# taylorlu/voicepuppet

Hardware: AMD Instinct MI355X
Metric: PixReferNet G+D step frames/sec @256x256 bs=32 (higher is better)
Workload: dtype bf16; 1 GPU; PixReferNet G+D training step (G + 3xD + VGG16-conv3_3 perceptual + TF-Adam x2), 256x256, ngf=ndf=64, global batch 32 = 32 per GPU; global_batch=32, per_gpu_batch=32, parallelism=dp1

## Files before the change

voicepuppet_amd/csrc/conv_args.h:

```cpp
#pragma once
#include <stddef.h>
#include <stdint.h>

namespace vp {

struct TapTable {
  int8_t dh[16];
  int8_t dw[16];
};

struct PixSrc {
  const void* ptr[2];
  int C[2];
  const float* aff_a[2];
  const float* aff_b[2];
  int act;
  int group_n;
};

enum ConvKernel {
  CK_IGEMM = 0,
  CK_PATCH,
  CK_PATCH2,
  CK_SMALLP,
  CK_S2C64,
  CK_CIN8,
  CK_COUT8,
  CK_DCOUT8,
  CK_COUT4,
  CK_C64,
  CK_PATCH3,
  CK_PATCH4,
  CK_DC256,
  CK_DC64,
};
struct IgemmArgs {
  PixSrc x;
  int N, Hin, Win;
  int Cin, log2Cin;
  int cin_mask;
  int cin_real;
  int Hg, Wg;
  int sh, sw;
  int ntaps, nclass;
  TapTable taps[4];
  const void* Wp;
  int Kpad, CoutPad;
  int wp_rows;
  void* Y;
  int y_f32;
  int Cout, ldY;
  int Hof, Wof, os;
  int o0h[4], o0w[4];
  const float* bias;
  int out_act;
  const void* ref;
  const float* ref_a;
  const float* ref_b;
  int ref_act, ref_group_n, accumulate;
  int split_c;
  void* Y2;
  const void* ref2;
  int accumulate2;
  int y2_f32;
  int splitk;
  float* partial;
  int vec_epi;
  int fastk;
  int rowperm;
  int xcd_remap;
  double* bn_part;
  int bn_tpg, bn_nchunk;
  const void* bst_y;
  const void* bst_y2;
  double* bn_part2;
  double* colsum_part;
  const void* zeros;
  int kern, p_kw, p_dhf, p_dhs, p_dwf, p_dws;
  void* xa_lrelu;
  void* xa_relu;
  void* pool_out;
  int pool_only;
  unsigned char* pool_code;
  int pool_src;
  unsigned* sp_cnt;
  unsigned short sp_mask[4];
  int sp_npt, sp_lcpt;
};

struct WgradArgs {
  PixSrc g;
  int Gc, log2Gc;
  int gc_mask;
  int Hgin, Wgin;
  PixSrc d;
  int Dc;
  int N, Hb, Wb;
  int s, ntaps;
  TapTable taps;
  int Mpad, Dpad;
  int splitk;
  float* partial;
  float* dW;
  int Greal, Dreal, accumulate;
  const void* zeros;
  int lw, lh;
  int fastw;
  int xcd_remap;
  int fast_tr;
};

struct Cout1Args {
  const void* dy;
  int ld_dy;
  const float* w;
  const void* ref;
  int ref_act;
  const void* y;
  double* part;
  void* dx;
  int N, H, W, C, Ho, Wo, ks, pad;
  int groups, rows;
  float* slabs;
  float* dW;
  int pix_per_group, tiles_per_group;
};

}
```

voicepuppet_amd/csrc/conv_ops.h:

```cpp
#pragma once
#include <stdlib.h>
#include <string.h>

#include "launch.h"

namespace vp {

struct ConvGeomX : ConvGeom {
  int CoutT;
};

inline ConvGeomX make_geom(int kind, int ks, int stride, int pad, int N, int Hin, int Win, int Cin, int Cin_real, int Cout) {
  ConvGeomX g;
  g.kind = kind; g.ks = ks; g.stride = stride; g.pad = pad;
  g.N = N; g.Hin = Hin; g.Win = Win;
  if (kind == 0) { g.Hout = (Hin + 2 * pad - ks) / stride + 1; g.Wout = (Win + 2 * pad - ks) / stride + 1; }
  else { g.Hout = 2 * Hin; g.Wout = 2 * Win; }
  g.Cin = Cin; g.Cin_real = Cin_real; g.Cout = Cout;
  g.CoutT = Cout < 8 ? 8 : Cout;
  return g;
}

inline int kc_elems(int is_bf16) { return is_bf16 ? 32 : 16; }

inline int& wgrad_cost_knob(int i) { static int v[3] = {80, 15, 150}; return v[i]; }
inline int& plan_misc_knob(int i) { static int v[4] = {384, 8, 4, 512}; return v[i]; }
inline int& igemm_small_grid_knob() { static int v = 128; return v; }
inline int& thin_blocks_knob(int i) { static int v[4] = {1024, 512, 512, 512}; return v[i]; }

inline int pick_igemm_cfg(int rows, int P, int Kpad = 0) {
  if (P >= 96) {
    if (rows % 128 == 0 && igemm_small_grid_knob() > 0 && (long long)((P + 127) / 128) * (rows / 128) <= igemm_small_grid_knob()) return IG_64x128;
    if (rows % 256 == 0 && P >= 256 * 256 && Kpad >= 4096) return IG_256x256;
    if (rows % 128 == 0 && P >= 256 * 512) return IG_128x256;
    if (rows % 128 == 0) return IG_128x128;
    if (rows % 64 == 0) return IG_64x128;
    if (rows <= 16) return IG_16x128;
    return rows > 64 ? IG_128x128 : IG_64x128;
  }
  if (rows <= 64) return IG_64x32;
  return P > 16 ? IG_128x32 : IG_128x16;
}

constexpr int IGEMM_SPLITK_TARGET_DEFAULT = 64;
inline int& igemm_splitk_target_knob() { static int v = IGEMM_SPLITK_TARGET_DEFAULT; return v; }
inline int pick_igemm_splitk(int blocks, int nchunk) {
  const int target = igemm_splitk_target_knob();
  const int cap = plan_misc_knob(1);
  const int minchunk = plan_misc_knob(2);
  if (blocks >= 256 || blocks >= target) return 1;
  int s = (target + blocks - 1) / blocks;
  if (s > nchunk / minchunk) s = nchunk / minchunk;
  if (s > cap) s = cap;
  return s < 1 ? 1 : s;
}

inline void set_single_src(PixSrc& x, const void* p, int C, const float* a, const float* b, int act, int group_n) {
  x.ptr[0] = p; x.ptr[1] = nullptr; x.C[0] = C; x.C[1] = 0;
  x.aff_a[0] = a; x.aff_b[0] = b; x.aff_a[1] = nullptr; x.aff_b[1] = nullptr;
  x.act = act; x.group_n = group_n > 0 ? group_n : (1 << 30);
}

struct LaunchForm {
  bool bias = false, ref = false, xa_lrelu = false, xa_relu = false, x_affine = false;
  bool stats = false;
  int x_act = 0, ref_act = 0;
};

struct IgemmPlan {
  IgemmArgs a;
  int cfg;
  LaunchForm form;
  PackDesc pack;
  size_t pack_elems;
  size_t partial_bytes;
};

struct IgemmPin { int cfg, splitk; };

inline void finish_igemm(IgemmPlan& p, int rows, int is_bf16, const IgemmPin* pin = nullptr) {
  IgemmArgs& a = p.a;
  const int P = a.N * a.Hg * a.Wg;
  a.Kpad = round_up(a.ntaps * a.Cin, kc_elems(is_bf16));
  p.cfg = pick_igemm_cfg(rows, P, a.Kpad);
  if (!is_bf16 && a.ntaps == 1 && p.cfg == IG_128x128) {
    const long long b128 = (long long)((P + 127) / 128) * (rows / 128), b64 = 2 * b128;
    if (((b64 + 255) / 256) * 64 < ((b128 + 255) / 256) * 128) p.cfg = IG_64x128;
  }
  if (pin) p.cfg = pin->cfg;
  int bc, bp;
  igemm_tile(p.cfg, &bc, &bp);
  a.CoutPad = round_up(rows, bc);
  if (a.ntaps == 1) { a.log2Cin = 30; a.cin_mask = 0x3fffffff; }
  else { a.log2Cin = ilog2(a.Cin); a.cin_mask = a.Cin - 1; }
  const int blocks = ((P + bp - 1) / bp) * (a.CoutPad / bc) * a.nclass;
  a.splitk = pin ? pin->splitk : pick_igemm_splitk(blocks, a.Kpad / kc_elems(is_bf16));
  p.partial_bytes = a.splitk > 1 ? (size_t)a.nclass * a.splitk * P * a.CoutPad * sizeof(float) : 0;
  {
    const bool tc4 = p.cfg == IG_128x128 || p.cfg == IG_64x128 || p.cfg == IG_128x256 || p.cfg == IG_256x256;
    a.rowperm = (tc4 && rows % 64 == 0) ? 1 : 0;
    p.pack.perm = a.rowperm;
  }
  a.wp_rows = round_up(rows, 128);
  p.pack.rows_pad = a.wp_rows;
  p.pack.Kpad = a.Kpad;
  p.pack.kc = kc_elems(is_bf16);
  p.pack_elems = (size_t)a.nclass * a.wp_rows * a.Kpad;
}

inline int& patch_tiles_knob() { static int v = 7; return v; }
inline int& patch_small_knob() { static int v = 3; return v; }
inline int& patch_longk_knob() { static int v = 1; return v; }
inline int& patch3_knob() { static int v = 1; return v; }
inline int& wgrad_big_knob() { static int v = 1; return v; }
inline int& patch4_knob() { static int v = 1; return v; }
inline int& c64_knob() { static int v = 1; return v; }
inline int& pool_bwd_fused_knob() { static int v = 1; return v; }
inline int& cout1_knob() { static int v = 256; return v; }
inline int& wgrad1_rows_knob() { static int v = 512; return v; }
inline int& dc64_knob() { static int v = 1; return v; }
inline int& s2c64_knob() { static int v = 512; return v; }
inline int& s2c64_pair_knob() { static int v = 1; return v; }
constexpr int PATCH_MIN_BLOCKS_DEFAULT = 192;
inline int& patch_minblk_knob() { static int v = PATCH_MIN_BLOCKS_DEFAULT; return v; }

inline void patch_tile_hw(int bp, int* th, int* tw) { *th = bp == 128 ? 8 : 16; *tw = bp == 512 ? 32 : 16; }
inline int patch_tile_pixels(int bc) {
  const int k = patch_small_knob();
  if (bc == 256) return (k & 2) ? 128 : 256;
  return (k & 1) ? 256 : 512;
}

inline int patch_tile_rows(int rows, int on) {
  if ((on & 1) && rows % 256 == 0) return 256;
  if ((on & 2) && rows % 128 == 0) return 128;
  if ((on & 4) && rows % 64 == 0) return 64;
  return 0;
}

inline bool plan_patch_eligible(const IgemmPlan& p, int rows, int is_bf16, bool single_src, bool any_grid = false) {
  const int on = patch_tiles_knob();
  const int minblk = any_grid ? 0 : patch_minblk_knob();
  const IgemmArgs& a = p.a;
  const int kc = kc_elems(is_bf16);
  if (!on || !single_src || a.nclass != 1 || a.sh != 1 || a.sw != 1 || a.os != 1 || a.ntaps < 9 || a.Cin % kc || a.Cin < kc) return false;
  if (rows % 64 || a.Cout % 8 || a.ldY % 8 || a.Hg < 16 || a.Wg < 16 || a.Hof != a.Hg || a.Wof != a.Wg) return false;
  const bool p4 = patch4_knob() && is_bf16 && a.ntaps == 16 && rows % 128 == 0;
  if (!p4 && patch_longk_knob() && rows >= 512 && rows % 256 == 0 && a.ntaps * a.Cin >= 4096 && (long long)a.N * a.Hg * a.Wg >= 256 * 256) return false;
  const int bc = p4 ? 128 : patch_tile_rows(rows, on);
  if (!bc) return false;
  int th, tw;
  patch_tile_hw(p4 ? 256 : patch_tile_pixels(bc), &th, &tw);
  const long long blocks = (long long)a.N * ((a.Hg + th - 1) / th) * ((a.Wg + tw - 1) / tw) * (rows / bc);
  const long long p4min = (long long)a.ntaps * a.Cin >= 8192 ? 256 : 512;
  if (p4 && !any_grid && patch_minblk_knob() > 1) {
    if (blocks < p4min) return false;
  } else if (blocks < minblk) return false;
  if ((size_t)a.N * a.Hin * a.Win * a.Cin * (is_bf16 ? 2 : 4) >= 0x70000000ull) return false;
  int ks = 0;
  while (ks * ks < a.ntaps) ++ks;
  if (ks * ks != a.ntaps) return false;
  const int sh = a.taps[0].dh[ks] - a.taps[0].dh[0], sw = a.taps[0].dw[1] - a.taps[0].dw[0];
  if ((sh != 1 && sh != -1) || (sw != 1 && sw != -1)) return false;
  for (int t = 0; t < a.ntaps; ++t)
    if (a.taps[0].dh[t] != a.taps[0].dh[0] + (t / ks) * sh || a.taps[0].dw[t] != a.taps[0].dw[0] + (t % ks) * sw) return false;
  return true;
}
inline void plan_make_patch(IgemmPlan& p, int rows, int is_bf16) {
  IgemmArgs& a = p.a;
  const bool p4 = patch4_knob() && is_bf16 && a.ntaps == 16 && rows % 128 == 0;
  const int bc = p4 ? 128 : patch_tile_rows(rows, patch_tiles_knob());
  int ks = 0;
  while (ks * ks < a.ntaps) ++ks;
  a.kern = CK_PATCH; a.p_kw = ks;
  a.p_dhf = a.taps[0].dh[0]; a.p_dwf = a.taps[0].dw[0];
  a.p_dhs = a.taps[0].dh[ks] - a.taps[0].dh[0]; a.p_dws = a.taps[0].dw[1] - a.taps[0].dw[0];
  const int bp = p4 ? 256 : patch_tile_pixels(bc);
  p.cfg = bc == 256 ? (bp == 128 ? PATCH_256x128 : PATCH_256x256) : (bc == 128 ? (bp == 256 ? PATCH_128x256 : PATCH_128x512) : (bp == 256 ? PATCH_64x256 : PATCH_64x512));
  a.CoutPad = round_up(rows, bc);
  a.splitk = 1;
  p.partial_bytes = 0;
  a.rowperm = 1;
  p.pack.perm = 1;
  p.pack.kswap = 1;
}

inline int& patch_xcd_knob() { static int v = 0; return v; }
inline int& patch2_knob() { static int v = 1; return v; }
inline bool plan_patch2_eligible(const IgemmPlan& p, int rows, int is_bf16, int c0, int c1) {
  const IgemmArgs& a = p.a;
  const int kc = kc_elems(is_bf16);
  if (!patch2_knob() || a.nclass != 4 || a.ntaps != 4 || a.os != 2 || a.sh != 1 || a.sw != 1) return false;
  if (c0 + c1 != a.Cin || c0 % (2 * kc) || c1 % (2 * kc) || c0 < 2 * kc) return false;
  if (rows % 64 || rows > 128 || a.Cout % 8 || a.ldY % 8 || a.Hg < 16 || a.Wg < 16 || a.Hof != 2 * a.Hg || a.Wof != 2 * a.Wg) return false;
  const long long blocks = (long long)a.N * ((a.Hg + 15) / 16) * ((a.Wg + 15) / 16) * 4;
  if (blocks < patch_minblk_knob()) return false;
  const size_t cmax = c0 > c1 ? c0 : c1;
  if ((size_t)a.N * a.Hin * a.Win * cmax * (is_bf16 ? 2 : 4) >= 0x70000000ull) return false;
  for (int cls = 0; cls < 4; ++cls)
    for (int t = 0; t < 4; ++t)
      if (a.taps[cls].dh[t] != a.taps[cls].dh[3] + 1 - (t >> 1) || a.taps[cls].dw[t] != a.taps[cls].dw[3] + 1 - (t & 1)) return false;
  return true;
}
inline void plan_make_patch2(IgemmPlan& p, int rows, int is_bf16) {
  IgemmArgs& a = p.a;
  const int bc = rows % 128 == 0 ? 128 : 64;
  a.kern = CK_PATCH2; a.p_kw = 2;
  p.cfg = bc == 128 ? PATCH_128x256 : PATCH_64x256;
  a.CoutPad = round_up(rows, bc);
  a.splitk = 1;
  p.partial_bytes = 0;
  a.rowperm = 1;
  p.pack.perm = 1;
  p.pack.kswap = 1;
}

inline int& smallp_knob() { static int v = 256; return v; }
inline bool plan_smallp_eligible(const IgemmPlan& p, int rows, int is_bf16, int c0, int c1) {
  const IgemmArgs& a = p.a;
  const int kc = kc_elems(is_bf16);
  const long long Pc = (long long)a.N * a.Hg * a.Wg;
  if (smallp_knob() <= 0 || Pc > smallp_knob() || a.ntaps > 16 || a.nclass > 4) return false;
  if (rows % 32 || a.Cout != rows || a.ldY % 8) return false;
  if (a.Cin < kc || (a.Cin & (a.Cin - 1)) || c0 + c1 != a.Cin || c0 % kc || c1 % kc) return false;
  if ((long long)a.N * a.Hin * a.Win * (c0 > c1 ? c0 : c1) >= (1ll << 30)) return false;
  return true;
}
inline int smallp_counters(const IgemmArgs& a) {
  const int PT = a.sp_npt * 16;
  const int Pc = a.N * a.Hg * a.Wg;
  return (a.CoutPad / 32) * a.nclass * ((Pc + PT - 1) / PT) + a.CoutPad / 32;
}
inline void plan_make_smallp(IgemmPlan& p, int rows, int is_bf16) {
  IgemmArgs& a = p.a;
  const int kc = kc_elems(is_bf16);
  const int Pc = a.N * a.Hg * a.Wg;
  a.kern = CK_SMALLP;
  a.sp_npt = Pc <= 16 ? 1 : (Pc <= 32 ? 2 : 4);
  p.cfg = a.sp_npt == 1 ? SMALLP_32x16 : (a.sp_npt == 2 ? SMALLP_32x32 : SMALLP_32x64);
  a.sp_lcpt = ilog2(a.Cin / kc);
  a.CoutPad = round_up(rows, 32);
  a.rowperm = 0; p.pack.perm = 0; p.pack.kswap = 0;
  int minchunks = 1 << 30;
  for (int cls = 0; cls < a.nclass; ++cls) {
    unsigned m = 0;
    for (int t = 0; t < a.ntaps; ++t) {
      bool okh = false, okw = false;
      for (int q = 0; q < a.Hg && !okh; ++q) { const int ih = q * a.sh + a.taps[cls].dh[t]; okh = ih >= 0 && ih < a.Hin; }
      for (int r = 0; r < a.Wg && !okw; ++r) { const int iw = r * a.sw + a.taps[cls].dw[t]; okw = iw >= 0 && iw < a.Win; }
      if (okh && okw) m |= 1u << t;
    }
    a.sp_mask[cls] = (unsigned short)m;
    const int chunks = __builtin_popcount(m) * (a.Cin / kc);
    if (chunks < minchunks) minchunks = chunks;
  }
  const int PT = a.sp_npt * 16;
  const int tiles = (a.CoutPad / 32) * a.nclass * ((Pc + PT - 1) / PT);
  const int target = plan_misc_knob(0);
  int s = (target + tiles - 1) / tiles;
  if (s > minchunks / 8) s = minchunks / 8;
  if (s > 64) s = 64;
  if (s < 1) s = 1;
  a.splitk = s;
  p.partial_bytes = s > 1 ? (size_t)s * tiles * PT * 32 * sizeof(float) : 0;
}

inline bool plan_s2c64_eligible(const IgemmPlan& p, int rows, int is_bf16, int c0, int c1) {
  const IgemmArgs& a = p.a;
  if (s2c64_knob() <= 0 || !is_bf16 || a.nclass != 1 || a.ntaps != 16 || a.os != 1 || a.sh != 2 || a.sw != 2) return false;
  if ((rows != 128 && rows != 256) || a.Cout != rows || a.ldY != 128 || a.Cin != 64 || c0 != 64 || c1 != 0 || a.Kpad != 1024) return false;
  if (a.Hg % 4 || a.Wg % 16 || a.Hin != 2 * a.Hg || a.Win != 2 * a.Wg || a.Hof != a.Hg || a.Wof != a.Wg) return false;
  for (int t = 0; t < 16; ++t)
    if (a.taps[0].dh[t] != (t >> 2) - 1 || a.taps[0].dw[t] != (t & 3) - 1) return false;
  if (a.N * (a.Hg / 4) * (a.Wg / 16) < s2c64_knob()) return false;
  return (size_t)a.N * a.Hin * a.Win * 64 * 2 < 0x70000000ull;
}
inline void plan_make_s2c64(IgemmPlan& p) {
  IgemmArgs& a = p.a;
  a.kern = CK_S2C64;
  p.cfg = IG_128x128;
  a.CoutPad = a.Cout; a.wp_rows = a.Cout; p.pack.rows_pad = a.Cout;
  p.pack_elems = (size_t)a.wp_rows * a.Kpad;
  a.splitk = 1; p.partial_bytes = 0;
  a.rowperm = 1; p.pack.perm = 1; p.pack.kswap = 0;
}

inline IgemmArgs launch_view(const IgemmPlan& p, const LaunchForm& f) {
  static char set[16] = {};
  IgemmArgs v = p.a;
  v.Y = set; v.zeros = set;
  if (v.split_c) v.Y2 = set;
  if (f.bias) v.bias = (const float*)set;
  if (f.ref) { v.ref = set; v.ref_act = f.ref_act; if (v.split_c) v.ref2 = set; }
  if (f.xa_lrelu) v.xa_lrelu = set;
  if (f.xa_relu) v.xa_relu = set;
  if (f.x_affine) v.x.aff_a[0] = (const float*)set;
  v.x.act = f.x_act;
  if (f.stats) v.bn_part = (double*)set;
  return v;
}

enum { FAM_SMALLP = 1, FAM_PATCH = 2, FAM_PATCH2 = 4, FAM_S2C64 = 8, FAM_ALL = 15 };

inline void plan_kernel(IgemmPlan& p, int rows, int is_bf16, int c0, int c1, unsigned fams, const LaunchForm& f, bool any_grid = false) {
  if ((fams & FAM_SMALLP) && plan_smallp_eligible(p, rows, is_bf16, c0, c1)) plan_make_smallp(p, rows, is_bf16);
  else if ((fams & FAM_PATCH) && plan_patch_eligible(p, rows, is_bf16, c1 == 0 && c0 == p.a.Cin, any_grid)) plan_make_patch(p, rows, is_bf16);
  else if ((fams & FAM_PATCH2) && plan_patch2_eligible(p, rows, is_bf16, c0, c1)) plan_make_patch2(p, rows, is_bf16);
  else if ((fams & FAM_S2C64) && plan_s2c64_eligible(p, rows, is_bf16, c0, c1)) plan_make_s2c64(p);
  p.form = f;
  p.a.x.C[0] = c0; p.a.x.C[1] = c1;
  p.a.kern = pick_conv_kernel(launch_view(p, f), is_bf16);
}

inline IgemmPlan plan_fwd(const ConvGeomX& g, size_t w_off, int is_bf16, const IgemmPin* pin = nullptr) {
  IgemmPlan p;
  memset(&p, 0, sizeof(p));
  IgemmArgs& a = p.a;
  a.N = g.N; a.Hin = g.Hin; a.Win = g.Win; a.Cin = g.Cin; a.cin_real = g.Cin_real;
  a.Cout = g.Cout; a.ldY = g.Cout; a.Hof = g.Hout; a.Wof = g.Wout;
  a.ref_group_n = 1 << 30;
  PackDesc& d = p.pack;
  d.src_off = w_off; d.rows_real = g.Cout; d.C = g.Cin; d.C_real = g.Cin_real;
  if (g.kind == 0) {
    a.Hg = g.Hout; a.Wg = g.Wout; a.sh = a.sw = g.stride; a.os = 1;
    a.ntaps = g.ks * g.ks; a.nclass = 1;
    for (int t = 0; t < a.ntaps; ++t) {
      a.taps[0].dh[t] = (int8_t)(t / g.ks - g.pad); a.taps[0].dw[t] = (int8_t)(t % g.ks - g.pad);
      d.kh[0][t] = (int8_t)(t / g.ks); d.kw[0][t] = (int8_t)(t % g.ks);
    }
    d.s_kh = g.ks * g.Cin_real * g.Cout; d.s_kw = g.Cin_real * g.Cout; d.s_ch = g.Cout; d.s_row = 1;
  } else {
    a.Hg = g.Hin; a.Wg = g.Win; a.sh = a.sw = 1; a.os = 2;
    a.ntaps = 4; a.nclass = 4;
    for (int cls = 0; cls < 4; ++cls) {
      const int ph = cls >> 1, pw = cls & 1;
      a.o0h[cls] = ph; a.o0w[cls] = pw;
      for (int t = 0; t < 4; ++t) {
        const int ta = t >> 1, tb = t & 1;
        a.taps[cls].dh[t] = (int8_t)(ph - ta); a.taps[cls].dw[t] = (int8_t)(pw - tb);
        d.kh[cls][t] = (int8_t)((1 - ph) + 2 * ta); d.kw[cls][t] = (int8_t)((1 - pw) + 2 * tb);
      }
    }
    d.s_kh = 4 * g.Cout * g.Cin_real; d.s_kw = g.Cout * g.Cin_real; d.s_row = g.Cin_real; d.s_ch = 1;
  }
  d.nclass = a.nclass; d.ntaps = a.ntaps;
  finish_igemm(p, g.Cout, is_bf16, pin);
  return p;
}

inline IgemmPlan plan_bwd_data(const ConvGeomX& g, size_t w_off, int row0, int rows, int rows_real, int ldX, int is_bf16) {
  IgemmPlan p;
  memset(&p, 0, sizeof(p));
  IgemmArgs& a = p.a;
  a.N = g.N; a.Hin = g.Hout; a.Win = g.Wout; a.Cin = g.CoutT; a.cin_real = g.Cout;
  a.Cout = rows; a.ldY = ldX; a.Hof = g.Hin; a.Wof = g.Win;
  a.ref_group_n = 1 << 30;
  PackDesc& d = p.pack;
  d.rows_real = rows_real; d.C = g.CoutT; d.C_real = g.Cout;
  if (g.kind == 0) {
    d.s_kh = g.ks * g.Cin_real * g.Cout; d.s_kw = g.Cin_real * g.Cout; d.s_row = g.Cout; d.s_ch = 1;
    if (g.stride == 1) {
      a.Hg = g.Hin; a.Wg = g.Win; a.sh = a.sw = 1; a.os = 1;
      a.ntaps = g.ks * g.ks; a.nclass = 1;
      for (int t = 0; t < a.ntaps; ++t) {
        const int kh = t / g.ks, kw = t % g.ks;
        a.taps[0].dh[t] = (int8_t)(g.pad - kh); a.taps[0].dw[t] = (int8_t)(g.pad - kw);
        d.kh[0][t] = (int8_t)kh; d.kw[0][t] = (int8_t)kw;
      }
    } else {
      a.Hg = g.Hout; a.Wg = g.Wout; a.sh = a.sw = 1; a.os = 2;
      a.ntaps = 4; a.nclass = 4;
      for (int cls = 0; cls < 4; ++cls) {
        const int ph = cls >> 1, pw = cls & 1;
        a.o0h[cls] = ph; a.o0w[cls] = pw;
        for (int t = 0; t < 4; ++t) {
          const int ta = t >> 1, tb = t & 1;
          a.taps[cls].dh[t] = (int8_t)(ph - ta); a.taps[cls].dw[t] = (int8_t)(pw - tb);
          d.kh[cls][t] = (int8_t)((1 - ph) + 2 * ta); d.kw[cls][t] = (int8_t)((1 - pw) + 2 * tb);
        }
      }
    }
  } else {
    d.s_kh = 4 * g.Cout * g.Cin_real; d.s_kw = g.Cout * g.Cin_real; d.s_row = 1; d.s_ch = g.Cin_real;
    a.Hg = g.Hin; a.Wg = g.Win; a.sh = a.sw = 2; a.os = 1;
    a.ntaps = 16; a.nclass = 1;
    for (int t = 0; t < 16; ++t) {
      a.taps[0].dh[t] = (int8_t)(t / 4 - 1); a.taps[0].dw[t] = (int8_t)(t % 4 - 1);
      d.kh[0][t] = (int8_t)(t / 4); d.kw[0][t] = (int8_t)(t % 4);
    }
  }
  d.src_off = w_off + (size_t)row0 * d.s_row;
  d.nclass = a.nclass; d.ntaps = a.ntaps;
  finish_igemm(p, rows, is_bf16);
  return p;
}

struct WgradPlan {
  WgradArgs a;
  int cfg;
  size_t partial_bytes;
};

inline int& wgrad_tr_knob() { static int v = 3; return v; }

inline WgradPlan plan_wgrad(const ConvGeomX& g, int is_bf16, bool plain_operands = true) {
  WgradPlan p;
  memset(&p, 0, sizeof(p));
  WgradArgs& a = p.a;
  a.N = g.N;
  a.ntaps = g.ks * g.ks;
  for (int t = 0; t < a.ntaps; ++t) { a.taps.dh[t] = (int8_t)(t / g.ks - g.pad); a.taps.dw[t] = (int8_t)(t % g.ks - g.pad); }
  if (g.kind == 0) {
    a.Gc = g.Cin; a.Greal = g.Cin_real; a.Hgin = g.Hin; a.Wgin = g.Win;
    a.Dc = g.CoutT; a.Dreal = g.Cout;
    a.Hb = g.Hout; a.Wb = g.Wout; a.s = g.stride;
  } else {
    a.Gc = g.CoutT; a.Greal = g.Cout; a.Hgin = g.Hout; a.Wgin = g.Wout;
    a.Dc = g.Cin; a.Dreal = g.Cin_real;
    a.Hb = g.Hin; a.Wb = g.Win; a.s = 2;
  }
  a.log2Gc = ilog2(a.Gc);
  a.gc_mask = a.Gc - 1;
  if (a.ntaps == 1) { a.log2Gc = 30; a.gc_mask = 0x3fffffff; }
  p.cfg = (a.Dc % 128 == 0) ? WG_128x128 : (a.Dc % 64 == 0 ? WG_128x64 : WG_128x16);
  a.lw = ilog2(a.Wb); a.lh = ilog2(a.Hb);
  const bool tr = is_bf16 && plain_operands && (wgrad_tr_knob() & 1) && (a.ntaps * a.Gc) % 256 == 0 && a.Dc % 128 == 0 &&
                  (((long long)a.N << (a.lw + a.lh)) % 32) == 0;
  if (tr) p.cfg = WG_TR_256x128;
  const bool tr_thin = !tr && is_bf16 && plain_operands && (wgrad_tr_knob() & 2) && (a.ntaps * a.Gc) % 128 == 0 && a.Dc % 8 == 0 && a.Dc <= 128 &&
                       (((long long)a.N << (a.lw + a.lh)) % 32) == 0 && a.lw + a.lh >= 5;
  if (tr_thin) p.cfg = WG_TR_128x128;
  int bm, bn;
  wgrad_tile(p.cfg, &bm, &bn);
  a.Mpad = round_up(a.ntaps * a.Gc, bm);
  a.Dpad = round_up(a.Dc, bn);
  const int kiter = (tr || tr_thin) ? 32 : kc_elems(is_bf16) * (is_bf16 ? 2 : 1);
  a.fastw = (!tr && !tr_thin && (1 << a.lw) >= (is_bf16 ? 8 : 4) && (1 << a.lw) <= kiter) ? 1 : 0;
  const int P = (a.fastw || tr || tr_thin) ? (a.N << (a.lw + a.lh)) : a.N * a.Hb * a.Wb;
  const int nchunk = (P + kiter - 1) / kiter;
  const int tiles = (a.Mpad / bm) * (a.Dpad / bn);
  int s = 1;
  const double wg_fixed = wgrad_cost_knob(0) * 0.1, wg_slab = wgrad_cost_knob(1) * 0.01 + wgrad_cost_knob(2) * 0.001 * tiles;
  {
    const int smax = nchunk / 4 < 1 ? 1 : (nchunk / 4 > 512 ? 512 : nchunk / 4);
    double best = 1e30;
    for (int c = 1; c <= smax; ++c) {
      const int rounds = (tiles * c + plan_misc_knob(3) - 1) / plan_misc_knob(3);
      const double cost = rounds * ((double)nchunk / c + wg_fixed) + wg_slab * c;
      if (cost < best - 1e-9) { best = cost; s = c; }
    }
  }
  if ((tr || tr_thin) && s >= 8 && (s & 7)) {
    const int smax = nchunk / 4 < 1 ? 1 : (nchunk / 4 > 512 ? 512 : nchunk / 4);
    auto cost = [&](int c) { return ((tiles * c + plan_misc_knob(3) - 1) / plan_misc_knob(3)) * ((double)nchunk / c + wg_fixed) + wg_slab * c; };
    const int lo = s & ~7, hi = lo + 8;
    s = (hi <= smax && cost(hi) <= cost(lo)) ? hi : lo;
  }
  a.splitk = s;
  p.partial_bytes = (size_t)s * a.Mpad * a.Dpad * sizeof(float);
  return p;
}

}
```

voicepuppet_amd/csrc/conv_prof.h:

```cpp
#pragma once
#include <hip/hip_runtime.h>

#include <string>

namespace vp {

void profile_enable(int on);
void profile_tag(const char* tag);
size_t profile_collect(char* out, size_t cap);

extern const char* g_prof_family;

struct ProfRec { hipEvent_t e0, e1; std::string name; double flops, bytes; };

struct ProfScope {
  bool on;
  ProfRec r;
  hipStream_t st;
  std::string kind;
  int bf, bc, bp;
  ProfScope(const char* kind_, int is_bf16, int bc_, int bp_, double flops, double bytes, hipStream_t s);
  ~ProfScope();
};

}
```

voicepuppet_amd/csrc/conv_prof.hip:

```cpp
#include "conv_prof.h"

#include <stdio.h>
#include <string.h>

#include <vector>

namespace vp {

static bool g_prof_on = false;
static std::vector<ProfRec> g_prof;
static std::vector<hipEvent_t> g_ev_pool;

static hipEvent_t prof_event() {
  hipEvent_t e;
  if (!g_ev_pool.empty()) { e = g_ev_pool.back(); g_ev_pool.pop_back(); return e; }
  hipEventCreate(&e);
  return e;
}

static std::string g_prof_tag;
static bool g_prof_detail = false;
void profile_enable(int on) { g_prof_on = on != 0; g_prof_detail = on > 1; }
void profile_tag(const char* tag) { if (g_prof_on && g_prof_detail) g_prof_tag = tag ? tag : ""; }

const char* g_prof_family = nullptr;

ProfScope::ProfScope(const char* kind_, int is_bf16, int bc_, int bp_, double flops, double bytes, hipStream_t s) : on(g_prof_on), st(s), kind(kind_), bf(is_bf16), bc(bc_), bp(bp_) {
  if (!on) return;
  g_prof_family = nullptr;
  r.flops = flops; r.bytes = bytes;
  r.e0 = prof_event(); r.e1 = prof_event();
  hipEventRecord(r.e0, st);
}
ProfScope::~ProfScope() {
  if (!on) return;
  hipEventRecord(r.e1, st);
  char buf[96];
  if ((kind == "igemm" || kind == "wgrad") && g_prof_family) snprintf(buf, sizeof(buf), "%s_%s_%s_%dx%d", kind.c_str(), g_prof_family, bf ? "bf16" : "f32", bc, bp);
  else snprintf(buf, sizeof(buf), "%s_%s_%dx%d", kind.c_str(), bf ? "bf16" : "f32", bc, bp);
  r.name = buf;
  if (g_prof_detail && !g_prof_tag.empty()) r.name = g_prof_tag + " " + r.name;
  g_prof.push_back(r);
}

size_t profile_collect(char* out, size_t cap) {
  struct Agg { std::string name; int calls; double ms, flops, bytes; };
  static std::string cache = "[]";
  if (g_prof.empty()) {
    if (out && cap > 0) { strncpy(out, cache.c_str(), cap - 1); out[cap - 1] = 0; }
    return cache.size() + 1;
  }
  std::vector<Agg> agg;
  for (ProfRec& r : g_prof) {
    float ms = 0.f;
    hipEventSynchronize(r.e1);
    hipEventElapsedTime(&ms, r.e0, r.e1);
    g_ev_pool.push_back(r.e0); g_ev_pool.push_back(r.e1);
    Agg* a = nullptr;
    for (Agg& x : agg) if (x.name == r.name) a = &x;
    if (!a) { agg.push_back({r.name, 0, 0, 0, 0}); a = &agg.back(); }
    a->calls++; a->ms += ms; a->flops += r.flops; a->bytes += r.bytes;
  }
  g_prof.clear();
  std::string js = "[";
  for (size_t i = 0; i < agg.size(); ++i) {
    char buf[256];
    snprintf(buf, sizeof(buf), "%s{\"name\":\"%s\",\"calls\":%d,\"ms\":%.6f,\"flops\":%.6e,\"bytes\":%.6e}", i ? "," : "",
             agg[i].name.c_str(), agg[i].calls, agg[i].ms, agg[i].flops, agg[i].bytes);
    js += buf;
  }
  js += "]";
  cache = js;
  if (out && cap > 0) { strncpy(out, js.c_str(), cap - 1); out[cap - 1] = 0; }
  return js.size() + 1;
}

}
```

voicepuppet_amd/csrc/conv_s2c64.hip:

```cpp
#include "conv_ops.h"
#include "igemm_device.h"
#include "launch.h"
#include "patch_device.h"

namespace vp {

namespace {
constexpr int TH = 4, TW = 16;
constexpr int PRW = 17;
constexpr int PHR = 2 * TH + 2;
constexpr int NPATCH = PHR * 2 * PRW;
constexpr int NROUND = 22;
constexpr int PBUFB = NROUND * 16 * 64;
constexpr int NCH = 2;
constexpr int BUFB = NCH * PBUFB;
constexpr int STGB = TH * TW * 256;
constexpr int NW = 8;
constexpr int JP = (NROUND + NW - 1) / NW;
}

__device__ __forceinline__ unsigned s2_pk_max_i16(unsigned x, unsigned y) {
  unsigned r;
  asm("v_pk_max_i16 %0, %1, %2" : "=v"(r) : "v"(x), "v"(y));
  return r;
}
__device__ __forceinline__ unsigned s2_pk_min_u16(unsigned x, unsigned y) {
  unsigned r;
  asm("v_pk_min_u16 %0, %1, %2" : "=v"(r) : "v"(x), "v"(y));
  return r;
}
__device__ __forceinline__ unsigned s2_pk_mul_lo_u16(unsigned x, unsigned y) {
  unsigned r;
  asm("v_pk_mul_lo_u16 %0, %1, %2" : "=v"(r) : "v"(x), "v"(y));
  return r;
}

template <bool STATS, bool PAIR>
__global__ __launch_bounds__(NW * 64, 1) void conv_s2c64_kernel(const IgemmArgs a, const int ntiles) {
  static_assert(!(STATS && PAIR), "statistics belong to the forward layers");
  extern __shared__ __attribute__((aligned(16))) char smem[];
  const int tid = threadIdx.x, lane = tid & 63;
  const int wave = __builtin_amdgcn_readfirstlane(tid >> 6);
  const int fi = lane & 15, fg = lane >> 4;

  const int G = gridDim.x;
  int vb = blockIdx.x;
  if ((G & 7) == 0) vb = (vb & 7) * (G >> 3) + (vb >> 3);
  const int half = PAIR ? (vb & 1) : 0, row0 = 128 * half;
  const int bt = PAIR ? (vb >> 1) : vb, GT = PAIR ? (G >> 1) : G;

  uint4 W[16][NCH];
  {
    const bf16* wp = reinterpret_cast<const bf16*>(a.Wp);
#pragma unroll
    for (int t = 0; t < 16; ++t)
#pragma unroll
      for (int c = 0; c < NCH; ++c)
        W[t][c] = *reinterpret_cast<const uint4*>(wp + ((size_t)(t * NCH + c) * a.wp_rows + row0 + 16 * wave + fi) * 32 + fg * 8);
  }
  const int c0 = 64 * (wave >> 2) + 32 * ((wave >> 1) & 1) + 8 * fg + 4 * (wave & 1);
  f32x4 bia = (f32x4){0.f, 0.f, 0.f, 0.f};
  if (a.bias) bia = (f32x4){a.bias[c0], a.bias[c0 + 1], a.bias[c0 + 2], a.bias[c0 + 3]};

  int tb0[2];
#pragma unroll
  for (int s = 0; s < 2; ++s) {
    const int px = fi + s;
    tb0[s] = (px << 6) + (((fg ^ (px >> 1)) & 3) << 4);
  }
  int ppy[JP], ppx[JP], prel[JP];
#pragma unroll
  for (int j = 0; j < JP; ++j) {
    const int pp = (wave + NW * j) * 16 + (lane >> 2);
    const int run = pp / PRW, idx = pp - run * PRW;
    ppy[j] = pp < NPATCH ? (run >> 1) : 1 << 20;
    ppx[j] = 2 * idx + (run & 1);
    prel[j] = pp < NPATCH ? (ppy[j] * a.Win + ppx[j]) * 128 + (((lane & 3) ^ ((idx >> 1) & 3)) * 8) * (int)sizeof(bf16) : 0;
  }
  const bool last_round = wave + NW * (JP - 1) < NROUND;

  __amdgpu_buffer_rsrc_t rsX = make_rsrc(a.x.ptr[0], (unsigned)((size_t)a.N * a.Hin * a.Win * 64 * sizeof(bf16)));
  const int tiles_x = a.Wg / TW, tpi = tiles_x * (a.Hg / TH);
  bf16* Yp = reinterpret_cast<bf16*>(half ? a.Y2 : a.Y);
  const bf16* refp = reinterpret_cast<const bf16*>(half ? a.ref2 : a.ref);
  const bool accum = PAIR && (half ? a.accumulate2 : a.accumulate);
  constexpr int NST = TH * TW * 256 / 1024 / NW;

  auto issue_patch = [&](int t, int buf) {
    const int n = t / tpi, rem = t - n * tpi;
    const int y0 = 2 * (rem / tiles_x) * TH - 1, x0 = 2 * (rem % tiles_x) * TW - 1;
    const int base = ((n * a.Hin + y0) * a.Win + x0) * 128;
#pragma unroll
    for (int j = 0; j < JP; ++j) {
      if (j == JP - 1 && !last_round) break;
      const int ih = y0 + ppy[j], iw = x0 + ppx[j];
      const bool ok = (unsigned)ih < (unsigned)a.Hin && (unsigned)iw < (unsigned)a.Win;
      const unsigned vo = ok ? (unsigned)(base + prel[j]) : DMA_OOB;
      uint4* l0 = reinterpret_cast<uint4*>(smem + buf * BUFB) + (wave + NW * j) * 64;
#pragma unroll
      for (int c = 0; c < NCH; ++c) dma16_buf(rsX, vo, (unsigned)(c * 64), l0 + c * (PBUFB / 16));
    }
  };

  float ssum[4] = {0.f, 0.f, 0.f, 0.f}, ssq[4] = {0.f, 0.f, 0.f, 0.f};
  int cur_grp = -1;
  unsigned done_mask = 0;
  const int ngroups = STATS ? (ntiles + a.bn_tpg - 1) / a.bn_tpg : 0;
  auto flush = [&](int grp) {
    float s[4], q[4];
#pragma unroll
    for (int e = 0; e < 4; ++e) {
      s[e] = ssum[e]; q[e] = ssq[e];
#pragma unroll
      for (int m = 1; m < 16; m <<= 1) { s[e] += __shfl_xor(s[e], m); q[e] += __shfl_xor(q[e], m); }
      ssum[e] = 0.f; ssq[e] = 0.f;
    }
    if (fi == 0) {
      double* row = a.bn_part + ((size_t)(grp * a.bn_nchunk + blockIdx.x) * 2) * a.Cout + c0;
#pragma unroll
      for (int e = 0; e < 4; ++e) { row[e] = (double)s[e]; row[a.Cout + e] = (double)q[e]; }
    }
    done_mask |= 1u << grp;
  };

  if (bt < ntiles) issue_patch(bt, 0);
#pragma unroll
  for (int t = 0; t < 16; ++t)
#pragma unroll
    for (int c = 0; c < NCH; ++c) asm volatile("" : "+v"(W[t][c].x), "+v"(W[t][c].y), "+v"(W[t][c].z), "+v"(W[t][c].w));
  int it = 0;
  for (int t = bt; t < ntiles; t += GT, ++it) {
    const int buf = it & 1;
    if (it == 0) wait_vm<0>();
    else wait_vm<NST>();
    __builtin_amdgcn_s_barrier();
    asm volatile("" ::: "memory");
    uint2 rz[PAIR ? TH : 1], ry[PAIR ? TH : 1];
    if constexpr (PAIR) {
      const int n = t / tpi, rem = t - n * tpi;
      const size_t o00 = ((size_t)(n * a.Hof + (rem / tiles_x) * TH) * a.Wof + (rem % tiles_x) * TW + fi) * 128 + c0;
#pragma unroll
      for (int r = 0; r < TH; ++r) rz[r] = *reinterpret_cast<const uint2*>(refp + o00 + (size_t)r * a.Wof * 128);
      if (accum) {
#pragma unroll
        for (int r = 0; r < TH; ++r) ry[r] = *reinterpret_cast<const uint2*>(Yp + o00 + (size_t)r * a.Wof * 128);
      }
    }
    if (t + GT < ntiles) issue_patch(t + GT, buf ^ 1);
    if constexpr (STATS) {
      const int grp = t / a.bn_tpg;
      if (grp != cur_grp) {
        if (cur_grp >= 0) flush(cur_grp);
        cur_grp = grp;
      }
    }
    int tb[2];
#pragma unroll
    for (int s = 0; s < 2; ++s) tb[s] = tb0[s] + buf * BUFB;

    f32x4 acc[TH];
#pragma unroll
    for (int r = 0; r < TH; ++r) acc[r] = bia;
    constexpr int LA = 2, NS = LA + 1, NSTEP = NCH * 4 * PHR;
    u32x4 rb[NS];
    auto rd = [&](auto sc) {
      constexpr int S = decltype(sc)::value, c = S / (4 * PHR), kw = (S / PHR) % 4, R = S % PHR;
      rb[S % NS] = lds_rd128<c * PBUFB + (R * 2 + (kw & 1)) * PRW * 64>(tb[kw >> 1]);
    };
    static_steps([&](auto sc) { rd(sc); }, std::make_integer_sequence<int, LA>{});
    static_steps([&](auto sc) {
      constexpr int S = decltype(sc)::value, c = S / (4 * PHR), kw = (S / PHR) % 4, R = S % PHR;
      if constexpr (S + LA < NSTEP) rd(std::integral_constant<int, S + LA>{});
      constexpr int AHEAD = (NSTEP - 1 - S < LA ? NSTEP - 1 - S : LA);
      asm volatile("s_waitcnt lgkmcnt(%0)" ::"n"(AHEAD) : "memory");
      asm volatile("" : "+v"(rb[S % NS]));
      const uint4 fb = make_uint4(rb[S % NS].x, rb[S % NS].y, rb[S % NS].z, rb[S % NS].w);
      static_steps([&](auto ri) {
        constexpr int r = (R >> 1) - decltype(ri)::value;
        if constexpr (r >= 0 && r < TH) {
          constexpr int kh = R - 2 * r;
          acc[r] = mma16<bf16>(W[4 * kh + kw][c], fb, acc[r]);
        }
      }, std::make_integer_sequence<int, 2>{});
      __builtin_amdgcn_sched_barrier(0);
    }, std::make_integer_sequence<int, NSTEP>{});

    char* stg = smem + 2 * BUFB;
    const int wslot = ((((c0 >> 3) ^ fi) & 15) << 4) + ((c0 & 4) << 1);
#pragma unroll
    for (int r = 0; r < TH; ++r) {
      uint2 pk;
      if constexpr (PAIR) {
        if (accum) {
          const float m0 = __uint_as_float(rz[r].x << 16) > 0.f ? 1.f : 0.f, m1 = __uint_as_float(rz[r].x & 0xffff0000u) > 0.f ? 1.f : 0.f;
          const float m2 = __uint_as_float(rz[r].y << 16) > 0.f ? 1.f : 0.f, m3 = __uint_as_float(rz[r].y & 0xffff0000u) > 0.f ? 1.f : 0.f;
          acc[r][0] = fmaf(acc[r][0], m0, __uint_as_float(ry[r].x << 16)); acc[r][1] = fmaf(acc[r][1], m1, __uint_as_float(ry[r].x & 0xffff0000u));
          acc[r][2] = fmaf(acc[r][2], m2, __uint_as_float(ry[r].y << 16)); acc[r][3] = fmaf(acc[r][3], m3, __uint_as_float(ry[r].y & 0xffff0000u));
        }
      }
      pk.x = Elem<bf16>::pack2(acc[r][0], acc[r][1]);
      pk.y = Elem<bf16>::pack2(acc[r][2], acc[r][3]);
      if constexpr (PAIR) {
        if (!accum) {
          pk.x = s2_pk_mul_lo_u16(pk.x, s2_pk_min_u16(s2_pk_max_i16(rz[r].x, 0u), 0x00010001u));
          pk.y = s2_pk_mul_lo_u16(pk.y, s2_pk_min_u16(s2_pk_max_i16(rz[r].y, 0u), 0x00010001u));
        }
      }
      if constexpr (STATS) {
        const float v0 = __uint_as_float(pk.x << 16), v1 = __uint_as_float(pk.x & 0xffff0000u);
        const float v2 = __uint_as_float(pk.y << 16), v3 = __uint_as_float(pk.y & 0xffff0000u);
        ssum[0] += v0; ssum[1] += v1; ssum[2] += v2; ssum[3] += v3;
        ssq[0] = fmaf(v0, v0, ssq[0]); ssq[1] = fmaf(v1, v1, ssq[1]); ssq[2] = fmaf(v2, v2, ssq[2]); ssq[3] = fmaf(v3, v3, ssq[3]);
      }
      *reinterpret_cast<uint2*>(stg + (r * TW + fi) * 256 + wslot) = pk;
    }
    asm volatile("s_waitcnt lgkmcnt(0)" ::: "memory");
    __builtin_amdgcn_s_barrier();
    asm volatile("" ::: "memory");
    {
      const int n = t / tpi, rem = t - n * tpi;
      const int q0 = (rem / tiles_x) * TH, r0 = (rem % tiles_x) * TW;
      const int row = wave >> 1;
#pragma unroll
      for (int j = 0; j < NST; ++j) {
        const int px = 8 * (wave & 1) + 4 * j + (lane >> 4), ps = lane & 15;
        const uint4 o = *reinterpret_cast<const uint4*>(stg + (row * TW + px) * 256 + (ps << 4));
        unsigned* yp = reinterpret_cast<unsigned*>(Yp + ((size_t)(n * a.Hof + q0 + row) * a.Wof + r0 + px) * 128 + ((ps ^ px) & 15) * 8);
        __builtin_nontemporal_store(o.x, yp); __builtin_nontemporal_store(o.y, yp + 1);
        __builtin_nontemporal_store(o.z, yp + 2); __builtin_nontemporal_store(o.w, yp + 3);
      }
    }
  }
  if constexpr (STATS) {
    if (cur_grp >= 0) flush(cur_grp);
    for (int g = 0; g < ngroups; ++g) {
      if (done_mask & (1u << g)) continue;
      if (fi == 0) {
        double* row = a.bn_part + ((size_t)(g * a.bn_nchunk + blockIdx.x) * 2) * a.Cout + c0;
#pragma unroll
        for (int e = 0; e < 4; ++e) { row[e] = 0.0; row[a.Cout + e] = 0.0; }
      }
    }
  }
}

int conv_s2c64_grid(const IgemmArgs& a) {
  const int ntiles = a.N * (a.Hg / TH) * (a.Wg / TW);
  return ntiles < 256 ? ntiles : 256;
}
int conv_s2c64_tiles_per_image(const IgemmArgs& a) { return (a.Hg / TH) * (a.Wg / TW); }

bool conv_s2c64_eligible(const IgemmArgs& a, int is_bf16) {
  if (!is_bf16 || a.kern != CK_S2C64 || a.ldY != 128 || a.Cin != 64 || a.x.C[0] != 64 || a.x.C[1] != 0 || !a.rowperm || a.splitk != 1) return false;
  if (a.Hg % TH || a.Wg % TW || a.Hin != 2 * a.Hg || a.Win != 2 * a.Wg) return false;
  if (a.out_act != ACT_NONE || a.y_f32 || a.pool_out || a.x.aff_a[0] || a.x.act != ACT_NONE || a.ref_a) return false;
  if (a.split_c) {
    return a.split_c == 128 && a.Cout == 256 && a.wp_rows == 256 && a.Y2 && a.ref && a.ref2 && a.ref_act == ACT_RELU && !a.y2_f32 && !a.bias && !a.bn_part;
  }
  return a.Cout == 128 && a.wp_rows == 128 && !a.ref && !a.accumulate;
}

hipError_t launch_conv_s2c64(const IgemmArgs& a, hipStream_t st) {
  const int ntiles = a.N * (a.Hg / TH) * (a.Wg / TW);
  const int pair = a.split_c ? 1 : 0;
  int grid = conv_s2c64_grid(a);
  if (pair) grid = 2 * ntiles < 512 ? 2 * ntiles : 512;
  if (a.bn_part && (pair || a.bn_nchunk != grid || a.bn_tpg <= 0 || (ntiles + a.bn_tpg - 1) / a.bn_tpg > 32)) return hipErrorInvalidValue;
  const int ki = pair ? 2 : (a.bn_part ? 1 : 0);
  void (*kerns[3])(const IgemmArgs, const int) = {conv_s2c64_kernel<false, false>, conv_s2c64_kernel<true, false>, conv_s2c64_kernel<false, true>};
  void (*kern)(const IgemmArgs, const int) = kerns[ki];
  const int smem = 2 * BUFB + STGB;
  static bool attr_done[3] = {false, false, false};
  if (!attr_done[ki]) { (void)hipFuncSetAttribute((const void*)kern, hipFuncAttributeMaxDynamicSharedMemorySize, smem); attr_done[ki] = true; }
  hipLaunchKernelGGL(kern, dim3(grid), dim3(NW * 64), smem, st, a, ntiles);
  return hipGetLastError();
}

}
```

voicepuppet_amd/csrc/ops_api.hip:

```cpp
#include <string.h>

#include <string>

#include "conv_ops.h"
#include "errors.h"
#include "audio_args.h"
#include "launch.h"
#include "vp_common.h"
#include "workspace.h"

using namespace vp;

namespace {

bool conv_desc_ok(const vp_conv_desc* d) {
  if (!d || d->n < 1 || d->h < 1 || d->w < 1) return false;
  if (d->cin < 8 || (d->cin & (d->cin - 1))) return false;
  if (d->kind == 1 && (d->ksize != 4 || d->stride != 2 || d->pad != 1)) return false;
  if (d->kind != 0 && d->kind != 1) return false;
  if (d->ksize < 1 || d->ksize > 4 || d->stride < 1 || d->stride > 2) return false;
  if (d->kind == 0 && d->stride == 2 && (d->ksize != 4 || d->pad != 1 || (d->h & 1) || (d->w & 1))) return false;
  return d->dtype == VP_F32 || d->dtype == VP_BF16;
}

ConvGeomX geom_of(const vp_conv_desc* d) {
  return make_geom(d->kind, d->ksize, d->stride, d->pad, d->n, d->h, d->w, d->cin, d->cin, d->cout);
}

const void* zero_page(char* ws, size_t used, hipStream_t st) {
  char* z = ws + align256(used);
  (void)hipMemsetAsync(z, 0, 256, st);
  return z;
}

}

extern "C" {

int vp_pixrefer_pack_frames(const unsigned char* example_frames, const unsigned char* current_frames, const int* crops,
                            int n, int img_size, float* inputs, float* fg_inputs, float* targets, float* masks, void* stream) {
  if (!example_frames || !current_frames || !crops || !inputs || !fg_inputs || !targets || !masks || n < 1 || img_size < 2) {
    set_err("vp_pixrefer_pack_frames: bad argument");
    return VP_ERR_ARG;
  }
  FramePackArgs a;
  a.ex = example_frames; a.cur = current_frames; a.crops = crops;
  a.inputs = inputs; a.fg_inputs = fg_inputs; a.targets = targets; a.masks = masks;
  a.N = n; a.S = img_size;
  VP_HIP_CHECK(launch_frame_pack(a, (hipStream_t)stream));
  return VP_OK;
}

extern "C" void vp_phase_marks_enable(int on);

enum TuneRule {
  TUNE_PLAIN,
  TUNE_POSITIVE,
  TUNE_NEG_RESETS,
  TUNE_0_TO_4,
};
struct TuneRow { const char* key; int* knob; TuneRule rule; int dflt; };

int vp_tune(const char* key, int value) {
  if (!key) return VP_ERR_ARG;
  static const TuneRow rows[] = {
      {"patch_tiles", &patch_tiles_knob(), TUNE_PLAIN},
      {"patch_min_blocks", &patch_minblk_knob(), TUNE_NEG_RESETS, PATCH_MIN_BLOCKS_DEFAULT},
      {"patch_small_tiles", &patch_small_knob(), TUNE_PLAIN},
      {"patch_long_k_on_256", &patch_longk_knob(), TUNE_PLAIN},
      {"wgrad_tr", &wgrad_tr_knob(), TUNE_PLAIN},
      {"patch3", &patch3_knob(), TUNE_PLAIN},
      {"c64", &c64_knob(), TUNE_PLAIN},
      {"dc64", &dc64_knob(), TUNE_PLAIN},
      {"pool_bwd_fused", &pool_bwd_fused_knob(), TUNE_0_TO_4, 1},
      {"cout1_wgrad_rows", &wgrad1_rows_knob(), TUNE_POSITIVE},
      {"cout1_bwd", &cout1_knob(), TUNE_NEG_RESETS, 256},
      {"s2c64", &s2c64_knob(), TUNE_PLAIN},
      {"wgrad_big", &wgrad_big_knob(), TUNE_PLAIN},
      {"patch4", &patch4_knob(), TUNE_PLAIN},
      {"s2c64_pair", &s2c64_pair_knob(), TUNE_PLAIN},
      {"bfm_dwproj", &bfm_dwproj_knob(), TUNE_PLAIN},
      {"patch2", &patch2_knob(), TUNE_PLAIN},
      {"patch_xcd", &patch_xcd_knob(), TUNE_PLAIN},
      {"smallp_max_pixels", &smallp_knob(), TUNE_PLAIN},
      {"igemm_splitk_target", &igemm_splitk_target_knob(), TUNE_NEG_RESETS, IGEMM_SPLITK_TARGET_DEFAULT},
      {"wgrad_fixed_x10", &wgrad_cost_knob(0), TUNE_PLAIN},
      {"wgrad_slab_x100", &wgrad_cost_knob(1), TUNE_PLAIN},
      {"wgrad_slab_tile_x1000", &wgrad_cost_knob(2), TUNE_NEG_RESETS, 150},
      {"smallp_split_target", &plan_misc_knob(0), TUNE_PLAIN},
      {"igemm_splitk_cap", &plan_misc_knob(1), TUNE_PLAIN},
      {"igemm_splitk_minchunk", &plan_misc_knob(2), TUNE_PLAIN},
      {"wgrad_resident_blocks", &plan_misc_knob(3), TUNE_PLAIN},
      {"igemm_small_grid", &igemm_small_grid_knob(), TUNE_PLAIN},
      {"thin_blocks_cout8", &thin_blocks_knob(0), TUNE_POSITIVE},
      {"thin_blocks_dcout8", &thin_blocks_knob(1), TUNE_POSITIVE},
      {"thin_blocks_cout4", &thin_blocks_knob(2), TUNE_POSITIVE},
      {"thin_blocks_cin8", &thin_blocks_knob(3), TUNE_POSITIVE},
  };
  if (!strcmp(key, "phase_marks")) { vp_phase_marks_enable(value); return VP_OK; }
  for (const TuneRow& r : rows) {
    if (strcmp(key, r.key)) continue;
    if (r.rule == TUNE_POSITIVE && value <= 0) break;
    const bool reset = (r.rule == TUNE_NEG_RESETS && value < 0) || (r.rule == TUNE_0_TO_4 && (value < 0 || value > 4));
    *r.knob = reset ? r.dflt : value;
    return VP_OK;
  }
  set_err("vp_tune: unknown key %s", key);
  return VP_ERR_ARG;
}

static unsigned* smallp_counter_page(char* ws, size_t used, const IgemmArgs& a, hipStream_t st) {
  unsigned* c = (unsigned*)(ws + align256(used) + 256);
  (void)hipMemsetAsync(c, 0, (size_t)smallp_counters(a) * sizeof(unsigned), st);
  return c;
}

size_t vp_conv_workspace_bytes(const vp_conv_desc* d) {
  if (!conv_desc_ok(d)) return 0;
  const int bf = d->dtype == VP_BF16, es = bf ? 2 : 4;
  const ConvGeomX g = geom_of(d);
  size_t best = 0;
  {
    IgemmPlan p = plan_fwd(g, 0, bf);
    best = align256(p.pack_elems * es) + p.partial_bytes;
    plan_kernel(p, g.Cout, bf, d->cin, 0, FAM_SMALLP, LaunchForm{});
    if (p.a.kern == CK_SMALLP) {
      const size_t b = align256(p.pack_elems * es) + align256(p.partial_bytes) + 512 + (size_t)smallp_counters(p.a) * sizeof(unsigned);
      if (b > best) best = b;
    }
  }
  if ((d->cout & (d->cout - 1)) == 0 && d->cout >= 8) {
    IgemmPlan p = plan_bwd_data(g, 0, 0, d->cin, d->cin, d->cin, bf);
    size_t b = align256(p.pack_elems * es) + p.partial_bytes;
    if (b > best) best = b;
    plan_kernel(p, d->cin, bf, d->cout, 0, FAM_SMALLP, LaunchForm{});
    if (p.a.kern == CK_SMALLP) {
      b = align256(p.pack_elems * es) + align256(p.partial_bytes) + 512 + (size_t)smallp_counters(p.a) * sizeof(unsigned);
      if (b > best) best = b;
    }
    for (int plain = 0; plain < 2; ++plain) {
      WgradPlan w = plan_wgrad(g, bf, plain != 0);
      if (w.partial_bytes + 512 > best) best = w.partial_bytes + 512;
    }
  }
  return best + 1024;
}

int vp_conv_fwd(const vp_conv_desc* d, const void* x, const float* in_scale, const float* in_shift,
                const float* w, const float* bias, void* y, void* workspace, void* stream) {
  if (!conv_desc_ok(d) || !x || !w || !y || !workspace) { set_err("vp_conv_fwd: bad argument"); return VP_ERR_ARG; }
  const int bf = d->dtype == VP_BF16, es = bf ? 2 : 4;
  hipStream_t st = (hipStream_t)stream;
  const ConvGeomX g = geom_of(d);
  IgemmPlan p = plan_fwd(g, 0, bf);
  p.a.out_act = d->out_act;
  LaunchForm f;
  f.bias = bias != nullptr; f.x_affine = in_scale != nullptr; f.x_act = d->in_act;
  const bool plain = d->in_act == ACT_NONE && !in_scale;
  plan_kernel(p, g.Cout, bf, d->cin, 0, plain ? (FAM_SMALLP | FAM_PATCH | FAM_PATCH2 | (d->out_act == ACT_NONE ? FAM_S2C64 : 0)) : 0, f);
  char* ws = (char*)workspace;
  VP_HIP_CHECK(launch_pack_weights_one(p.pack, w, ws, bf, st));
  IgemmArgs a = p.a;
  set_single_src(a.x, x, d->cin, in_scale, in_shift, d->in_act, 0);
  a.Wp = ws;
  a.partial = (float*)(ws + align256(p.pack_elems * es));
  a.Y = y; a.bias = bias;
  a.zeros = zero_page(ws, align256(p.pack_elems * es) + p.partial_bytes, st);
  if (a.kern == CK_SMALLP) a.sp_cnt = smallp_counter_page(ws, align256(p.pack_elems * es) + p.partial_bytes, a, st);
  VP_HIP_CHECK(launch_igemm(a, bf, p.cfg, st));
  return VP_OK;
}

int vp_conv_bwd_data(const vp_conv_desc* d, const void* dy, const float* w, void* dx, void* workspace, void* stream) {
  if (!conv_desc_ok(d) || !dy || !w || !dx || !workspace) { set_err("vp_conv_bwd_data: bad argument"); return VP_ERR_ARG; }
  if (d->cout < 8 || (d->cout & (d->cout - 1))) { set_err("vp_conv_bwd_data: cout must be a power of two >= 8"); return VP_ERR_ARG; }
  const int bf = d->dtype == VP_BF16, es = bf ? 2 : 4;
  hipStream_t st = (hipStream_t)stream;
  const ConvGeomX g = geom_of(d);
  IgemmPlan p = plan_bwd_data(g, 0, 0, d->cin, d->cin, d->cin, bf);
  plan_kernel(p, d->cin, bf, d->cout, 0, FAM_SMALLP | FAM_PATCH | FAM_PATCH2, LaunchForm{});
  char* ws = (char*)workspace;
  VP_HIP_CHECK(launch_pack_weights_one(p.pack, w, ws, bf, st));
  IgemmArgs a = p.a;
  set_single_src(a.x, dy, d->cout, nullptr, nullptr, ACT_NONE, 0);
  a.Wp = ws;
  a.partial = (float*)(ws + align256(p.pack_elems * es));
  a.Y = dx;
  a.zeros = zero_page(ws, align256(p.pack_elems * es) + p.partial_bytes, st);
  if (a.kern == CK_SMALLP) a.sp_cnt = smallp_counter_page(ws, align256(p.pack_elems * es) + p.partial_bytes, a, st);
  VP_HIP_CHECK(launch_igemm(a, bf, p.cfg, st));
  return VP_OK;
}

static bool pooled_desc_ok(const vp_conv_desc* d) {
  return conv_desc_ok(d) && d->kind == 0 && d->ksize == 3 && d->stride == 1 && d->pad == 1 && d->dtype == VP_BF16 && d->cin == d->cout &&
         (d->cin == 64 || d->cin == 128) && d->h % 4 == 0 && d->w % 16 == 0 && d->h >= 16;
}

size_t vp_conv3x3_c64_bwd_data_pooled_workspace_bytes(const vp_conv_desc* d) {
  if (!pooled_desc_ok(d)) return 0;
  return align256(vp_conv_workspace_bytes(d)) + align256((size_t)d->n * d->h * d->w * d->cout * 2) + 256;
}

int vp_conv3x3_c64_bwd_data_pooled(const vp_conv_desc* d, const void* dy_pool, const unsigned char* code, const float* w, const void* ref,
                                   void* dx, void* workspace, int fused, void* stream) {
  if (!pooled_desc_ok(d) || !dy_pool || !code || !w || !ref || !dx || !workspace) { set_err("vp_conv3x3_c64_bwd_data_pooled: bad argument"); return VP_ERR_ARG; }
  hipStream_t st = (hipStream_t)stream;
  const ConvGeomX g = geom_of(d);
  IgemmPlan p = plan_bwd_data(g, 0, 0, d->cin, d->cin, d->cin, 1);
  LaunchForm f;
  f.ref = true; f.ref_act = ACT_RELU;
  plan_kernel(p, d->cin, 1, d->cout, 0, FAM_PATCH, f);
  if (p.a.kern != CK_C64) {
    set_err("vp_conv3x3_c64_bwd_data_pooled: %d x %d x %d x %d is planned on kernel %s, not c64", d->n, d->h, d->w, d->cin, conv_kernel_name(p.a.kern));
    return VP_ERR_ARG;
  }
  char* ws = (char*)workspace;
  VP_HIP_CHECK(launch_pack_weights_one(p.pack, w, ws, 1, st));
  IgemmArgs a = p.a;
  a.Wp = ws;
  a.partial = (float*)(ws + align256(p.pack_elems * 2));
  a.Y = dx;
  a.ref = ref; a.ref_act = ACT_RELU;
  a.zeros = zero_page(ws, align256(p.pack_elems * 2) + p.partial_bytes, st);
  if (fused) {
    set_single_src(a.x, dy_pool, d->cout, nullptr, nullptr, ACT_NONE, 0);
    a.pool_code = const_cast<unsigned char*>(code);
    a.pool_src = 1;
  } else {
    char* full = ws + align256(vp_conv_workspace_bytes(d));
    VP_HIP_CHECK(launch_maxpool_bwd_code(code, dy_pool, full, d->n, d->h, d->w, d->cout, 1, st));
    set_single_src(a.x, full, d->cout, nullptr, nullptr, ACT_NONE, 0);
  }
  VP_HIP_CHECK(launch_igemm(a, 1, p.cfg, st));
  return VP_OK;
}

int vp_conv_bwd_weight(const vp_conv_desc* d, const void* x, const float* in_scale, const float* in_shift,
                       const void* dy, float* dw, void* workspace, void* stream) {
  if (!conv_desc_ok(d) || !x || !dy || !dw || !workspace) { set_err("vp_conv_bwd_weight: bad argument"); return VP_ERR_ARG; }
  if (d->cout < 8 || (d->cout & (d->cout - 1))) { set_err("vp_conv_bwd_weight: cout must be a power of two >= 8"); return VP_ERR_ARG; }
  const int bf = d->dtype == VP_BF16;
  hipStream_t st = (hipStream_t)stream;
  const ConvGeomX g = geom_of(d);
  WgradPlan p = plan_wgrad(g, bf, !in_scale && d->in_act == ACT_NONE);
  WgradArgs a = p.a;
  PixSrc xs, ds;
  set_single_src(xs, x, d->cin, in_scale, in_shift, d->in_act, 0);
  set_single_src(ds, dy, d->cout, nullptr, nullptr, ACT_NONE, 0);
  if (d->kind == 0) { a.g = xs; a.d = ds; } else { a.g = ds; a.d = xs; }
  a.partial = (float*)workspace;
  a.dW = dw;
  a.zeros = zero_page((char*)workspace, p.partial_bytes, st);
  VP_HIP_CHECK(launch_wgrad(a, bf, p.cfg, st));
  return VP_OK;
}

size_t vp_bn_workspace_bytes(int pixels, int c, int dtype) {
  if (pixels < 1 || c < 8) return 0;
  const int nch = bn_nchunk(pixels, c, 1, dtype == VP_BF16);
  return (size_t)nch * 2 * c * sizeof(double) + 4 * (size_t)c * sizeof(float) + 1024;
}

static bool bn_ok(int pixels, int c, int dtype) {
  const int e = dtype == VP_BF16 ? 8 : 4;
  return pixels >= 1 && c >= e && c % e == 0 && 256 % (c / e) == 0 && (dtype == VP_F32 || dtype == VP_BF16);
}

int vp_bn_stats(const void* y, int pixels, int c, int dtype, const float* gamma, const float* beta, float eps,
                float* scale, float* shift, float* mean, float* rstd, void* workspace, void* stream) {
  if (!bn_ok(pixels, c, dtype) || !y || !gamma || !beta || !scale || !shift || !mean || !rstd || !workspace) {
    set_err("vp_bn_stats: bad argument");
    return VP_ERR_ARG;
  }
  BnArgs b;
  memset(&b, 0, sizeof(b));
  b.y = y; b.C = c; b.G = 1; b.Pg = pixels;
  b.nchunk = bn_nchunk(pixels, c, 1, dtype == VP_BF16);
  b.partial = (double*)workspace;
  b.gamma = gamma; b.beta = beta; b.aff_a = scale; b.aff_b = shift; b.mu = mean; b.rstd = rstd; b.eps = eps;
  VP_HIP_CHECK(launch_bn_stats(b, dtype == VP_BF16, (hipStream_t)stream));
  return VP_OK;
}

int vp_bn_bwd(const void* y, const void* dz, void* dy, int pixels, int c, int dtype, const float* gamma,
              const float* mean, const float* rstd, float* dgamma, float* dbeta, void* workspace, void* stream) {
  if (!bn_ok(pixels, c, dtype) || !y || !dz || !dy || !gamma || !mean || !rstd || !dgamma || !dbeta || !workspace) {
    set_err("vp_bn_bwd: bad argument");
    return VP_ERR_ARG;
  }
  BnArgs b;
  memset(&b, 0, sizeof(b));
  b.y = y; b.dz = dz; b.dy = dy; b.C = c; b.G = 1; b.Pg = pixels;
  b.nchunk = bn_nchunk(pixels, c, 1, dtype == VP_BF16);
  b.partial = (double*)workspace;
  float* f = (float*)((char*)workspace + (size_t)b.nchunk * 2 * c * sizeof(double));
  b.c1 = f; b.c2 = f + c;
  b.gamma = gamma; b.mu = const_cast<float*>(mean); b.rstd = const_cast<float*>(rstd);
  b.dgamma = dgamma; b.dbeta = dbeta;
  VP_HIP_CHECK(launch_bn_bwd(b, dtype == VP_BF16, (hipStream_t)stream));
  return VP_OK;
}


int vp_maxpool2x2_fwd(const void* x, void* y, int n, int h, int w, int c, int dtype, void* stream) {
  const int e = dtype == VP_BF16 ? 8 : 4;
  if (!x || !y || n < 1 || h < 2 || w < 2 || (h & 1) || (w & 1) || c < e || c % e) { set_err("vp_maxpool2x2_fwd: bad argument"); return VP_ERR_ARG; }
  VP_HIP_CHECK(launch_maxpool_fwd(x, y, n, h, w, c, dtype == VP_BF16, (hipStream_t)stream));
  return VP_OK;
}

int vp_maxpool2x2_bwd(const void* x, const void* dy, void* dx, int n, int h, int w, int c, int dtype, void* stream) {
  const int e = dtype == VP_BF16 ? 8 : 4;
  if (!x || !dy || !dx || n < 1 || h < 2 || w < 2 || (h & 1) || (w & 1) || c < e || c % e) { set_err("vp_maxpool2x2_bwd: bad argument"); return VP_ERR_ARG; }
  VP_HIP_CHECK(launch_maxpool_bwd(x, dy, dx, n, h, w, c, dtype == VP_BF16, (hipStream_t)stream));
  return VP_OK;
}

int vp_maxpool2x2_bwd_code(const void* code, const void* dy, void* dx, int n, int h, int w, int c, int dtype, void* stream) {
  const int e = dtype == VP_BF16 ? 8 : 4;
  if (!code || !dy || !dx || n < 1 || h < 2 || w < 2 || (h & 1) || (w & 1) || c < e || c % e) { set_err("vp_maxpool2x2_bwd_code: bad argument"); return VP_ERR_ARG; }
  VP_HIP_CHECK(launch_maxpool_bwd_code(code, dy, dx, n, h, w, c, dtype == VP_BF16, (hipStream_t)stream));
  return VP_OK;
}

int vp_composite_fwd(const float* gen_out4, const float* targets, float* out4, float* outputs, float* outputs_fg, int n, int hw,
                     void* stream) {
  if (!gen_out4 || !targets || !out4 || !outputs || !outputs_fg || n < 1 || hw < 1) { set_err("vp_composite_fwd: bad argument"); return VP_ERR_ARG; }
  CompositeArgs ca;
  memset(&ca, 0, sizeof(ca));
  ca.y4 = gen_out4; ca.targets = targets; ca.o4 = out4; ca.outputs = outputs; ca.outputs_fg = outputs_fg; ca.N = n; ca.HW = hw; ca.train = 0;
  VP_HIP_CHECK(launch_composite_fwd(ca, 0, (hipStream_t)stream));
  return VP_OK;
}

int vp_gan_loss(const float* logits, void* seed_d, void* seed_g, float* predict, float* losses, int m, float gan_weight, int dtype,
                void* stream) {
  if (!logits || !seed_d || !seed_g || !predict || !losses || m < 1) { set_err("vp_gan_loss: bad argument"); return VP_ERR_ARG; }
  GanLossArgs ga;
  memset(&ga, 0, sizeof(ga));
  ga.logits = logits; ga.dl_d = seed_d; ga.dl_g = seed_g; ga.predict = predict; ga.losses = losses; ga.M = m; ga.gan_weight = gan_weight;
  VP_HIP_CHECK(launch_gan_loss(ga, dtype == VP_BF16, (hipStream_t)stream));
  return VP_OK;
}

int vp_dwconv7x3_bn_act(const float* x, const float* w, const float* bias, float* y, int b, int h, int wd, int c, void* stream) {
  if (!x || !w || !bias || !y || b < 1 || h < 1 || wd < 1 || c < 4 || (c & 3)) { set_err("vp_dwconv7x3_bn_act: bad argument"); return VP_ERR_ARG; }
  VP_HIP_CHECK(launch_dwconv7x3(x, w, bias, y, 0, b, h, wd, c, (hipStream_t)stream));
  return VP_OK;
}

int vp_dwconv7x3_bn_act_t(const void* x, const float* w, const float* bias, void* y, int dtype, int b, int h, int wd, int c, void* stream) {
  if (!x || !w || !bias || !y || b < 1 || h < 1 || wd < 1 || c < 4 || (c & 3) || (dtype != VP_F32 && dtype != VP_BF16)) {
    set_err("vp_dwconv7x3_bn_act_t: bad argument"); return VP_ERR_ARG;
  }
  VP_HIP_CHECK(launch_dwconv7x3(x, w, bias, y, dtype == VP_BF16, b, h, wd, c, (hipStream_t)stream));
  return VP_OK;
}

int vp_conv_first_fwd(const float* x, const float* w, const float* bias, float* y, int b, int h, int w_in, int cout, void* stream) {
  if (!x || !w || !bias || !y || b < 1 || h < 1 || w_in < 1 || cout < 1) { set_err("vp_conv_first_fwd: bad argument"); return VP_ERR_ARG; }
  int pt, ho, pl, wo;
  same_pad(h, 9, 1, &pt, &ho);
  same_pad(w_in, 5, 2, &pl, &wo);
  VP_HIP_CHECK(launch_conv_first(x, w, bias, y, 0, b, h, w_in, wo, cout, pt, pl, (hipStream_t)stream));
  return VP_OK;
}

static IgemmPlan dwproj_pack_plan(int pixels, int ce, int cout) {
  IgemmPlan p = plan_fwd(make_geom(0, 1, 1, 0, 1, pixels, 1, ce, ce, cout), 0, 0);
  p.pack.s_ch = cout;
  p.pack.dst_off = 0;
  p.pack.perm = 0; p.a.rowperm = 0;
  return p;
}

size_t vp_dwproj_workspace_bytes(int ce, int cout) {
  if (ce < 16 || ce % 16 || cout < 1) return 0;
  return align256((size_t)22 * ce * sizeof(float)) + align256(dwproj_pack_plan(1, ce, cout).pack_elems * sizeof(float)) + 256;
}

int vp_dwproj_fwd(const float* ex, const float* w_dw, const float* b_dw, const float* w_proj, const float* b_proj, float* y, int add, int b, int h,
                  int w, int ce, int cout, void* workspace, void* stream) {
  if (!ex || !w_dw || !b_dw || !w_proj || !b_proj || !y || !workspace || b < 1 || h < 1 || w < 1) { set_err("vp_dwproj_fwd: bad argument"); return VP_ERR_ARG; }
  if (!dwproj_eligible(w, ce, cout)) {
    set_err("vp_dwproj_fwd: no kernel for mel width %d, %d expanded and %d output channels (dwproj_eligible)", w, ce, cout);
    return VP_ERR_ARG;
  }
  const size_t ex_bytes = (size_t)b * h * w * ce * sizeof(float);
  if (ex_bytes >= 0xF0000000ull) {
    set_err("vp_dwproj_fwd: the expanded tensor is %zu bytes, the kernel's 32-bit lane offsets stop below 0xF0000000 (%llu)", ex_bytes, 0xF0000000ull);
    return VP_ERR_ARG;
  }
  hipStream_t st = (hipStream_t)stream;
  float* wdw22 = (float*)workspace;
  float* packed = (float*)((char*)workspace + align256((size_t)22 * ce * sizeof(float)));
  VP_HIP_CHECK(hipMemcpyAsync(wdw22, w_dw, (size_t)21 * ce * sizeof(float), hipMemcpyDeviceToDevice, st));
  VP_HIP_CHECK(hipMemcpyAsync(wdw22 + (size_t)21 * ce, b_dw, (size_t)ce * sizeof(float), hipMemcpyDeviceToDevice, st));
  const IgemmPlan p = dwproj_pack_plan(b * h * w, ce, cout);
  VP_HIP_CHECK(launch_pack_weights_one(p.pack, w_proj, packed, 0, st));
  VP_HIP_CHECK(launch_dwproj(ex, wdw22, packed, p.a.wp_rows, b_proj, y, add ? 1 : 0, b, h, w, ce, cout, st));
  return VP_OK;
}

int vp_maxpool_hw(const float* x, float* y, int b, int h, int w, int c, int kh, int kw, int sh, int sw, void* stream) {
  if (!x || !y || b < 1 || h < 1 || w < 1 || c < 4 || (c & 3) || kh < 1 || kw < 1 || sh < 1 || sw < 1) { set_err("vp_maxpool_hw: bad argument"); return VP_ERR_ARG; }
  const int ho = (h + sh - 1) / sh, wo = (w + sw - 1) / sw;
  const int ph = (ho - 1) * sh + kh - h, pw = (wo - 1) * sw + kw - w;
  const int pt = ph > 0 ? ph / 2 : 0, pl = pw > 0 ? pw / 2 : 0;
  VP_HIP_CHECK(launch_maxpool_same(x, y, 0, 0, b, h, w, c, kh, kw, sh, sw, pt, pl, ho, wo, (hipStream_t)stream));
  return VP_OK;
}

int vp_gru_seq(const float* xg, const float* xc, const float* whg, const float* whc, const int* seq_len, float* out, int b, int t,
               void* stream) {
  if (!xg || !xc || !whg || !whc || !seq_len || !out || b < 1 || t < 1) { set_err("vp_gru_seq: bad argument"); return VP_ERR_ARG; }
  VP_HIP_CHECK(launch_gru_seq(xg, xc, whg, whc, seq_len, out, b, t, (hipStream_t)stream));
  return VP_OK;
}

int vp_gru_seq_state(const float* xg, const float* xc, const float* whg, const float* whc, float* hstate, float* out, int b, int t, int t0,
                     int n, void* stream) {
  if (!xg || !xc || !whg || !whc || !hstate || !out || b < 1 || t < 1 || t0 < 0 || n < 0 || t0 + n > t) {
    set_err("vp_gru_seq_state: bad argument"); return VP_ERR_ARG;
  }
  if (n == 0) return VP_OK;
  VP_HIP_CHECK(launch_gru_state(xg, xc, whg, whc, hstate, out, b, t, t0, n, (hipStream_t)stream));
  return VP_OK;
}

}

extern "C" __attribute__((target("sse4.2"))) unsigned vp_crc32c(const void* data, size_t n, unsigned crc) {
  const unsigned char* p = (const unsigned char*)data;
  unsigned long long c = (unsigned long long)(crc ^ 0xFFFFFFFFu);
  while (n && ((size_t)p & 7)) { c = __builtin_ia32_crc32qi((unsigned)c, *p++); --n; }
  while (n >= 8) { c = __builtin_ia32_crc32di(c, *(const unsigned long long*)p); p += 8; n -= 8; }
  while (n) { c = __builtin_ia32_crc32qi((unsigned)c, *p++); --n; }
  return (unsigned)c ^ 0xFFFFFFFFu;
}
```

voicepuppet_amd/csrc/plan_pixrefer.hip:

```cpp
#include <math.h>
#include <stdio.h>
#include <string.h>

#include <mutex>
#include <string>
#include <utility>
#include <vector>

#include "conv_ops.h"
#include "conv_prof.h"
#include "errors.h"
#include "launch.h"
#include "smallp_args.h"
#include "vp_common.h"
#include "workspace.h"

namespace vp {

thread_local char g_err[512] = "";
void set_err(const char* fmt, ...) {
  va_list ap;
  va_start(ap, fmt);
  vsnprintf(g_err, sizeof(g_err), fmt, ap);
  va_end(ap);
}

struct BnBuf {
  float *a, *b, *mu, *rstd, *c1, *c2, *c1g, *c2g;
  double *pb, *pbg;
};

struct Tens {
  std::string name;
  void* y = nullptr;
  void* dz = nullptr;
  int N = 0, H = 0, W = 0, C = 0;
  bool is_f32 = false;
  bool has_bn = false;
  bool is_input = false;
  int pool = -1, pool_src = -1;
  bool dz_written = false;
  void* dz2 = nullptr;
  bool dz2_written = false;
  void* xa[3] = {nullptr, nullptr, nullptr};
  bool need_act[3] = {false, false, false};
  BnBuf bn{};
  int producer = -1;
  int n_bwd_consumers = 0;
  int dz_writes = 0;
  bool bn_bwd_done = false;
  bool hi = false;
  void* dz32 = nullptr;
  double* cs_part = nullptr;
  int cs_chunks = 0;
  int pb_cap = 0, pbg_cap = 0;
  int bst_chunks = 0, bst_chunks_g = 0;
  size_t elems() const { return (size_t)N * H * W * C; }
};

struct Layer {
  std::string scope;
  ConvGeomX g;
  int src[2] = {-1, -1};
  int nsrc = 1;
  int in_act = ACT_NONE;
  int out_act = ACT_NONE;
  int out = -1;
  bool has_bn = false;
  bool fg = false;
  int pool = -1, pool_t = -1;
  size_t w_off = 0, b_off = 0, gamma_off = 0, beta_off = 0;
  size_t pk_fwd = 0, pk_bwd[2] = {0, 0}, pk_bwd_alt[2] = {0, 0};
  bool need_bwd[2] = {false, false};
  IgemmPlan fwd, bwd[2], bwd_alt[2];
  IgemmPlan bwd_pair;
  size_t pk_bwd_pair = 0;
  bool has_pair = false;
  IgemmPlan fwd_half;
  size_t pk_fwd_half = 0;
  bool has_fwd_half = false;
  WgradPlan wg;
  size_t desc0 = 0, desc1 = 0;
  bool tapgemm = false;
  bool fwd_stats = false;
  float* tap_S = nullptr;
  void* tap_dyS = nullptr;
  unsigned* sp_cnt_fwd = nullptr;
  unsigned* sp_cnt_bwd[2] = {nullptr, nullptr};
  unsigned* sp_cnt_pair = nullptr;
};

struct ParamInfo { std::string name; size_t off; int ndim; int64_t shape[4]; };

struct Net {
  std::vector<Tens> t;
  std::vector<Layer> l;
  std::vector<ParamInfo> manifest;
  size_t nparams = 0;
  int batch = 0, groups = 1;
  int i_md5 = -1, i_me2 = -1;
  float* params = nullptr;
  float* grads = nullptr;
  char* packed = nullptr;
  size_t packed_elems = 0;
  std::vector<PackDesc> descs;
  PackDesc* d_descs = nullptr;
  unsigned* sp_cnt = nullptr;
  size_t sp_cnt_n = 0;
};

struct Lane { hipStream_t s; char* scratch; double* bn_partial; };
enum { LANE_CALLER = 0, LANE_SIDE = 1, LANE_BRANCH = 2, LANE_BRANCH2 = 3 };

struct Sub { int sample0, nb; bool alt, gpass; };

}

using namespace vp;

struct vp_pixrefer {
  vp_pixrefer_desc d;
  int bf16, es;
  Net G, D, V;
  void *gin, *gfg, *din, *vin;
  float *y4, *o4, *outputs, *outputs_fg, *logits, *predict, *losses;
  void *dl_d, *dl_g, *d_din, *d_vin, *dy4, *df3;
  void *vpool1, *vpool2, *d_vpool1, *d_vpool2;
  unsigned char* vpool_code[2];
  bool pool_codes_written;
  bool pool_fuse_ok[2];
  bool pool_bwd_fused;
  bool pool_dz_stale[2];
  double *comp_partial, *perc_partial;
  Lane lane[4];
  hipEvent_t ev_b2join;
  bool use_b2;
  hipEvent_t ev_fork, ev_join, ev_bfork, ev_bjoin;
  hipEvent_t ev_upd_b, ev_upd_m;
  bool overlap, forked;
  int bst_count;
  int bst_on;
  int vgg_fork_layer;
  bool store_first_raw;
  bool ov_on;
  int dfork_point;
  bool dsplit_on;
  hipEvent_t mark[64];
  int nmark;
  bool marks_made;
  int dfork_pending;
  void* zeros;
  size_t scratch_bytes;
  int n_comp, n_perc;
  struct { bool active, d_done; float *m_g, *v_g, *m_d, *v_d; float lr_t_g, lr_t_d, beta1, beta2, eps; } upd;
  int upd_mask;
  bool params_dirty;
  bool vgg_dirty;
  const float *in_targets, *in_masks;
};

namespace vp {

static int add_tensor(Net& n, const std::string& name, int N, int H, int W, int C, bool has_bn, bool is_input) {
  Tens t;
  t.name = name; t.N = N; t.H = H; t.W = W; t.C = C; t.has_bn = has_bn; t.is_input = is_input;
  n.t.push_back(t);
  return (int)n.t.size() - 1;
}

static void add_param(Net& n, const std::string& name, std::initializer_list<int64_t> shape, size_t* off_out) {
  ParamInfo p;
  p.name = name; p.off = n.nparams; p.ndim = (int)shape.size();
  size_t cnt = 1;
  int i = 0;
  for (auto s : shape) { p.shape[i++] = s; cnt *= (size_t)s; }
  for (; i < 4; ++i) p.shape[i] = 1;
  *off_out = n.nparams;
  n.nparams += cnt;
  n.manifest.push_back(p);
}

static int add_layer(Net& n, const std::string& prefix, const std::string& scope, int kind, int ks, int stride, int pad,
                     std::initializer_list<int> srcs, int cin_real, int cout, bool has_bn, int in_act, int out_act,
                     const char* wname, const char* bname) {
  Layer L;
  L.scope = scope;
  L.nsrc = 0;
  int cin = 0;
  for (int s : srcs) {
    L.src[L.nsrc++] = s; cin += n.t[s].C;
    if (in_act != ACT_NONE) n.t[s].need_act[in_act] = true;
  }
  const Tens& t0 = n.t[L.src[0]];
  L.g = make_geom(kind, ks, stride, pad, n.batch, t0.H, t0.W, cin, cin_real, cout);
  L.in_act = in_act; L.out_act = out_act; L.has_bn = has_bn;
  const std::string base = prefix + scope + "/";
  if (kind == 0) add_param(n, base + wname, {ks, ks, cin_real, cout}, &L.w_off);
  else add_param(n, base + wname, {4, 4, cout, cin_real}, &L.w_off);
  add_param(n, base + bname, {cout}, &L.b_off);
  if (has_bn) {
    add_param(n, base + "batch_normalization/gamma", {cout}, &L.gamma_off);
    add_param(n, base + "batch_normalization/beta", {cout}, &L.beta_off);
  }
  L.out = add_tensor(n, scope, n.batch, L.g.Hout, L.g.Wout, L.g.CoutT, has_bn, false);
  n.t[L.out].producer = (int)n.l.size();
  n.l.push_back(L);
  return L.out;
}

static void build_generator(Net& n, int N, int H, int ngf, int groups = 1) {
  n.batch = N; n.groups = groups;
  const int tin = add_tensor(n, "inputs", N, H, H, 8, false, true);
  const int tfg = add_tensor(n, "fg_inputs", N, H, H, 8, false, true);
  const char* CK = "conv2d/kernel"; const char* CB = "conv2d/bias";
  const char* DK = "conv2d_transpose/kernel"; const char* DB = "conv2d_transpose/bias";
  const std::string P = "generator/";
  int e1 = add_layer(n, P, "encoder_1", 0, 4, 2, 1, {tin}, 6, ngf, false, ACT_NONE, ACT_NONE, CK, CB);
  int e2 = add_layer(n, P, "encoder_2", 0, 4, 2, 1, {e1}, ngf, ngf * 2, true, ACT_LRELU, ACT_NONE, CK, CB);
  int e3 = add_layer(n, P, "encoder_3", 0, 4, 2, 1, {e2}, ngf * 2, ngf * 2, true, ACT_LRELU, ACT_NONE, CK, CB);
  int e4 = add_layer(n, P, "encoder_4", 0, 4, 2, 1, {e3}, ngf * 2, ngf * 4, true, ACT_LRELU, ACT_NONE, CK, CB);
  int f1 = add_layer(n, P, "encoder_fg_1", 0, 4, 2, 1, {tfg}, 3, ngf, false, ACT_NONE, ACT_NONE, CK, CB);
  int f2 = add_layer(n, P, "encoder_fg_2", 0, 4, 2, 1, {f1}, ngf, ngf * 2, true, ACT_LRELU, ACT_NONE, CK, CB);
  int f3 = add_layer(n, P, "encoder_fg_3", 0, 4, 2, 1, {f2}, ngf * 2, ngf * 2, true, ACT_LRELU, ACT_NONE, CK, CB);
  int f4 = add_layer(n, P, "encoder_fg_4", 0, 4, 2, 1, {f3}, ngf * 2, ngf * 4, true, ACT_LRELU, ACT_NONE, CK, CB);
  int m2 = add_layer(n, P, "merged_encoder_2", 0, 4, 2, 1, {e4, f4}, ngf * 8, ngf * 4, true, ACT_LRELU, ACT_NONE, CK, CB);
  int m3 = add_layer(n, P, "merged_encoder_3", 0, 4, 2, 1, {m2}, ngf * 4, ngf * 8, true, ACT_LRELU, ACT_NONE, CK, CB);
  int m4 = add_layer(n, P, "merged_encoder_4", 0, 4, 2, 1, {m3}, ngf * 8, ngf * 8, true, ACT_LRELU, ACT_NONE, CK, CB);
  int m5 = add_layer(n, P, "merged_encoder_5", 0, 4, 2, 1, {m4}, ngf * 8, ngf * 8, true, ACT_LRELU, ACT_NONE, CK, CB);
  int d5 = add_layer(n, P, "merged_decoder_5", 1, 4, 2, 1, {m5}, ngf * 8, ngf * 8, true, ACT_RELU, ACT_NONE, DK, DB);
  int d4 = add_layer(n, P, "merged_decoder_4", 1, 4, 2, 1, {d5, m4}, ngf * 16, ngf * 8, true, ACT_RELU, ACT_NONE, DK, DB);
  int d3 = add_layer(n, P, "merged_decoder_3", 1, 4, 2, 1, {d4, m3}, ngf * 16, ngf * 4, true, ACT_RELU, ACT_NONE, DK, DB);
  int d2 = add_layer(n, P, "merged_decoder_2", 1, 4, 2, 1, {d3, m2}, ngf * 8, ngf * 4, true, ACT_RELU, ACT_NONE, DK, DB);
  int c4 = add_layer(n, P, "merged2_decoder_4", 1, 4, 2, 1, {d2, e4}, ngf * 8, ngf * 2, true, ACT_RELU, ACT_NONE, DK, DB);
  int c3 = add_layer(n, P, "merged2_decoder_3", 1, 4, 2, 1, {c4, e3}, ngf * 4, ngf * 2, true, ACT_RELU, ACT_NONE, DK, DB);
  int c2 = add_layer(n, P, "merged2_decoder_2", 1, 4, 2, 1, {c3, e2}, ngf * 4, ngf, true, ACT_RELU, ACT_NONE, DK, DB);
  int d1 = add_layer(n, P, "decoder_1", 1, 4, 2, 1, {c2, e1}, ngf * 2, 4, false, ACT_RELU, ACT_NONE, DK, DB);
  n.t[d1].is_f32 = true;
  for (int f : {f1, f2, f3, f4}) n.l[n.t[f].producer].fg = true;
  n.i_me2 = n.t[m2].producer; n.i_md5 = n.t[d5].producer;
}

static void build_discriminator(Net& n, int N, int H, int ndf) {
  n.batch = 3 * N; n.groups = 3;
  const int tin = add_tensor(n, "d_inputs", 3 * N, H, H, 8, false, true);
  const char* CK = "conv2d/kernel"; const char* CB = "conv2d/bias";
  const std::string P = "discriminator/";
  int l1 = add_layer(n, P, "layer_1", 0, 4, 2, 1, {tin}, 6, ndf, false, ACT_NONE, ACT_NONE, CK, CB);
  int l2 = add_layer(n, P, "layer_2", 0, 4, 2, 1, {l1}, ndf, ndf * 2, true, ACT_LRELU, ACT_NONE, CK, CB);
  int l3 = add_layer(n, P, "layer_3", 0, 4, 2, 1, {l2}, ndf * 2, ndf * 4, true, ACT_LRELU, ACT_NONE, CK, CB);
  int l4 = add_layer(n, P, "layer_4", 0, 4, 1, 1, {l3}, ndf * 4, ndf * 8, true, ACT_LRELU, ACT_NONE, CK, CB);
  int l5 = add_layer(n, P, "layer_5", 0, 4, 1, 1, {l4}, ndf * 8, 1, false, ACT_LRELU, ACT_NONE, CK, CB);
  n.t[l5].is_f32 = true;
}

static void build_vgg(Net& n, int N, int H) {
  n.batch = 2 * N; n.groups = 1;
  const int tin = add_tensor(n, "v_inputs", 2 * N, H, H, 8, false, true);
  const std::string P = "vgg_16/";
  auto add_pool = [&](int k, int conv) {
    const Tens tc = n.t[conv];
    const int p = add_tensor(n, k ? "pool2" : "pool1", tc.N, tc.H / 2, tc.W / 2, tc.C, false, false);
    n.t[p].pool = k; n.t[p].pool_src = conv;
    n.l[tc.producer].pool = k; n.l[tc.producer].pool_t = p;
    return p;
  };
  int c11 = add_layer(n, P, "conv1/conv1_1", 0, 3, 1, 1, {tin}, 3, 64, false, ACT_NONE, ACT_RELU, "weights", "biases");
  int c12 = add_layer(n, P, "conv1/conv1_2", 0, 3, 1, 1, {c11}, 64, 64, false, ACT_NONE, ACT_RELU, "weights", "biases");
  const int p1 = add_pool(0, c12);
  int c21 = add_layer(n, P, "conv2/conv2_1", 0, 3, 1, 1, {p1}, 64, 128, false, ACT_NONE, ACT_RELU, "weights", "biases");
  int c22 = add_layer(n, P, "conv2/conv2_2", 0, 3, 1, 1, {c21}, 128, 128, false, ACT_NONE, ACT_RELU, "weights", "biases");
  const int p2 = add_pool(1, c22);
  int c31 = add_layer(n, P, "conv3/conv3_1", 0, 3, 1, 1, {p2}, 128, 256, false, ACT_NONE, ACT_RELU, "weights", "biases");
  int c32 = add_layer(n, P, "conv3/conv3_2", 0, 3, 1, 1, {c31}, 256, 256, false, ACT_NONE, ACT_RELU, "weights", "biases");
  add_layer(n, P, "conv3/conv3_3", 0, 3, 1, 1, {c32}, 256, 256, false, ACT_NONE, ACT_RELU, "weights", "biases");
}

static int epi_stat_chunks(const IgemmPlan& p, int batch, int groups);
static bool first_layer_shape(int bf16, const Net& n, const Layer& L) {
  if (!bf16 || L.has_bn || L.tapgemm || L.out_act != ACT_NONE) return false;
  const Tens& to = n.t[L.out];
  return to.need_act[ACT_LRELU] && !to.is_f32;
}
constexpr int BST_MAX_CHUNKS = 8192;

static void plan_net(Net& n, int bf16, bool training, bool want_wgrad, int alt_batch, size_t* scratch_max, bool fwd_halves = false) {
  size_t pk = 0;
  auto take = [&](IgemmPlan& p) {
    p.pack.dst_off = pk;
    pk += (p.pack_elems + 63) & ~(size_t)63;
    n.descs.push_back(p.pack);
    if (p.partial_bytes > *scratch_max) *scratch_max = p.partial_bytes;
  };
  for (Layer& L : n.l) {
    L.desc0 = n.descs.size();
    Tens& to = n.t[L.out];
    const int c0 = n.t[L.src[0]].C, c1 = L.nsrc > 1 ? n.t[L.src[1]].C : 0;
    L.tapgemm = training && L.g.kind == 0 && L.g.stride == 1 && L.g.ks == 4 && L.g.Cout == 1 && L.nsrc == 1 && !L.has_bn &&
                L.g.Cin == L.g.Cin_real;
    if (L.tapgemm) {
      ConvGeomX g1 = make_geom(0, 1, 1, 0, L.g.N, L.g.Hin, L.g.Win, L.g.Cin, L.g.Cin, 16);
      L.fwd = plan_fwd(g1, L.w_off, bf16);
      L.fwd.pack.s_row = L.g.Cin; L.fwd.pack.s_ch = 1; L.fwd.pack.s_kh = 0; L.fwd.pack.s_kw = 0;
      L.fwd.a.y_f32 = 1;
      plan_kernel(L.fwd, 16, bf16, L.g.Cin, 0, 0, LaunchForm{});
    } else {
      L.fwd = plan_fwd(L.g, L.w_off, bf16);
      L.fwd.a.ldY = to.is_f32 ? L.g.Cout : to.C; L.fwd.a.y_f32 = to.is_f32 ? 1 : 0; L.fwd.a.out_act = L.out_act;
      LaunchForm f;
      f.bias = !L.has_bn;
      if (first_layer_shape(bf16, n, L)) { f.xa_lrelu = true; f.xa_relu = to.need_act[ACT_RELU]; }
      const unsigned fams = (n.groups == 1 && alt_batch == 0 ? FAM_SMALLP : 0) | FAM_PATCH | FAM_PATCH2 |
                            (L.has_bn && L.out_act == ACT_NONE ? FAM_S2C64 : 0);
      plan_kernel(L.fwd, L.g.Cout, bf16, c0, c1, fams, f);
      const IgemmArgs& a = L.fwd.a;
      const bool own_rows = (a.kern == CK_DC256 && n.groups == 1) || a.kern == CK_S2C64;
      const int chunks = epi_stat_chunks(L.fwd, n.batch, n.groups);
      if (L.has_bn && !own_rows && chunks > 0 && L.g.Cout % 8 == 0 && a.ldY % 8 == 0 && !a.y_f32 &&
          (size_t)n.groups * chunks * 2 * to.C <= (size_t)1024 * 2 * 512) {
        L.fwd_stats = L.fwd.form.stats = true;
        L.fwd.a.kern = pick_conv_kernel(launch_view(L.fwd, L.fwd.form), bf16);
      }
    }
    take(L.fwd);
    L.pk_fwd = L.fwd.pack.dst_off;
    if (fwd_halves && alt_batch > 0 && !L.tapgemm && !L.has_bn) {
      ConvGeomX g2 = L.g;
      g2.N = alt_batch;
      L.fwd_half = plan_fwd(g2, L.w_off, bf16);
      L.fwd_half.a.ldY = to.C; L.fwd_half.a.out_act = L.out_act;
      LaunchForm f;
      f.bias = true;
      plan_kernel(L.fwd_half, g2.Cout, bf16, c0, c1, conv_staging(L.fwd.a.kern) == CK_PATCH ? FAM_PATCH : 0, f, true);
      const PackDesc &pa = L.fwd.pack, &pb = L.fwd_half.pack;
      if (L.fwd_half.a.splitk == 1) {
        if (pa.kswap != pb.kswap || pa.perm != pb.perm || pa.kc != pb.kc || pa.Kpad != pb.Kpad || pa.rows_pad != pb.rows_pad) {
          take(L.fwd_half);
          L.pk_fwd_half = L.fwd_half.pack.dst_off;
        } else {
          L.pk_fwd_half = L.pk_fwd;
        }
        L.has_fwd_half = true;
      }
    }
    if (!training) continue;
    int row0 = 0;
    for (int s = 0; s < L.nsrc; ++s) {
      const Tens& ts = n.t[L.src[s]];
      const int rows = ts.C;
      int rows_real = rows;
      if (ts.is_input) rows_real = L.g.Cin_real;
      L.need_bwd[s] = !ts.is_input || (n.groups == 3) || (n.l[0].g.ks == 3);
      if (L.need_bwd[s]) {
        LaunchForm f;
        f.ref_act = L.in_act != ACT_NONE ? L.in_act : (ts.producer >= 0 && n.l[ts.producer].out_act == ACT_RELU ? ACT_RELU : ACT_NONE);
        f.ref = !ts.is_input && f.ref_act != ACT_NONE;
        L.bwd[s] = plan_bwd_data(L.g, L.w_off, row0, rows, rows_real, ts.C, bf16);
        if (alt_batch > 0) {
          ConvGeomX g2 = L.g;
          g2.N = alt_batch;
          L.bwd_alt[s] = plan_bwd_data(g2, L.w_off, row0, rows, rows_real, ts.C, bf16);
          if (L.bwd_alt[s].a.rowperm != L.bwd[s].a.rowperm) {
            L.bwd[s].a.rowperm = L.bwd_alt[s].a.rowperm = 0;
            L.bwd[s].pack.perm = L.bwd_alt[s].pack.perm = 0;
          }
        }
        plan_kernel(L.bwd[s], rows, bf16, L.g.CoutT, 0, (n.groups == 1 && alt_batch == 0 && !ts.is_input ? FAM_SMALLP : 0) | FAM_PATCH | FAM_PATCH2, f);
        if (alt_batch > 0) plan_kernel(L.bwd_alt[s], rows, bf16, L.g.CoutT, 0, FAM_PATCH | FAM_PATCH2, f);
        take(L.bwd[s]);
        L.pk_bwd[s] = L.pk_bwd_alt[s] = L.bwd[s].pack.dst_off;
        if (alt_batch > 0) {
          const PackDesc &pa = L.bwd[s].pack, &pb = L.bwd_alt[s].pack;
          if (pa.kswap != pb.kswap || pa.perm != pb.perm || pa.kc != pb.kc || pa.Kpad != pb.Kpad) {
            take(L.bwd_alt[s]);
            L.pk_bwd_alt[s] = L.bwd_alt[s].pack.dst_off;
          } else {
            L.bwd_alt[s].pack.dst_off = L.pk_bwd[s];
            if (L.bwd_alt[s].partial_bytes > *scratch_max) *scratch_max = L.bwd_alt[s].partial_bytes;
          }
        }
      }
      row0 += rows;
    }
    {
      const int s0 = conv_staging(L.bwd[0].a.kern);
      if (L.nsrc == 2 && n.groups == 1 && alt_batch == 0 && L.need_bwd[0] && L.need_bwd[1] && c0 == c1 && !n.t[L.src[0]].is_input &&
          !n.t[L.src[1]].is_input && s0 == conv_staging(L.bwd[1].a.kern) && (s0 == CK_IGEMM || s0 == CK_SMALLP) &&
          L.g.Cin_real == c0 + c1 && c0 % 32 == 0) {
        L.bwd_pair = plan_bwd_data(L.g, L.w_off, 0, c0 + c1, c0 + c1, c0, bf16);
        L.bwd_pair.a.split_c = c0;
        LaunchForm f;
        f.ref = true; f.ref_act = L.in_act;
        const unsigned fams = s0 == CK_SMALLP ? FAM_SMALLP : (s2c64_pair_knob() && L.in_act == ACT_RELU ? FAM_S2C64 : 0);
        plan_kernel(L.bwd_pair, c0 + c1, bf16, L.g.CoutT, 0, fams, f);
        if (s0 != CK_SMALLP || L.bwd_pair.a.kern == CK_SMALLP) {
          take(L.bwd_pair);
          L.pk_bwd_pair = L.bwd_pair.pack.dst_off;
          L.has_pair = true;
        }
      }
    }
    if (want_wgrad) {
      if (L.tapgemm) {
        ConvGeomX gw = make_geom(0, 1, 1, 0, L.g.N, L.g.Hin, L.g.Win, 16, 16, L.g.Cin);
        L.wg = plan_wgrad(gw, bf16);
      } else {
        L.wg = plan_wgrad(L.g, bf16);
      }
      if (L.wg.partial_bytes > *scratch_max) *scratch_max = L.wg.partial_bytes;
    }
  }
  n.packed_elems = pk;
  {
    for (Tens& t : n.t) t.hi = bf16 && t.has_bn && n.groups == 1 && alt_batch == 0 && t.producer >= 0 && n.l[t.producer].fwd.a.kern == CK_SMALLP;
    if (training)
      for (Layer& L : n.l)
        for (int s = 0; s < L.nsrc; ++s)
          if (L.need_bwd[s] && L.bwd[s].a.kern != CK_SMALLP) n.t[L.src[s]].hi = false;
    for (Layer& L : n.l)
      for (int s = 0; s < L.nsrc; ++s)
        if (L.in_act == ACT_NONE) n.t[L.src[s]].hi = false;
  }
  for (Tens& t : n.t) t.pb_cap = t.pbg_cap = 0;
  if (training)
    for (Layer& L : n.l) {
      auto cap = [&](Tens& t, const IgemmPlan& p, int batch, int groups, int& c) {
        if (!t.has_bn || t.hi) return;
        const int k = epi_stat_chunks(p, batch, groups);
        if (k > 0 && k <= BST_MAX_CHUNKS && k > c) c = k;
      };
      for (int s = 0; s < L.nsrc; ++s) {
        if (!L.need_bwd[s]) continue;
        Tens& ts = n.t[L.src[s]];
        cap(ts, L.bwd[s], n.batch, n.groups, ts.pb_cap);
        if (alt_batch > 0) cap(ts, L.bwd_alt[s], alt_batch, 1, ts.pbg_cap);
        if (L.has_pair) cap(ts, L.bwd_pair, n.batch, n.groups, ts.pb_cap);
        if (L.tapgemm && bf16 && ts.has_bn && !ts.hi && L.g.ks == 4 && L.g.stride == 1 && L.g.Cin == 512) {
          if (ts.pb_cap < 256) ts.pb_cap = 256;
          if (alt_batch > 0 && ts.pbg_cap < 256) ts.pbg_cap = 256;
        }
      }
    }
  for (size_t i = 0; i < n.l.size(); ++i) n.l[i].desc1 = i + 1 < n.l.size() ? n.l[i + 1].desc0 : n.descs.size();
  for (Tens& t : n.t) t.n_bwd_consumers = 0;
  n.sp_cnt_n = 0;
  for (Layer& L : n.l) {
    if (L.fwd.a.kern == CK_SMALLP) n.sp_cnt_n += smallp_counters(L.fwd.a);
    for (int s = 0; s < L.nsrc && training; ++s) {
      if (!L.need_bwd[s]) continue;
      n.t[L.src[s]].n_bwd_consumers++;
      if (L.bwd[s].a.kern == CK_SMALLP) n.sp_cnt_n += smallp_counters(L.bwd[s].a);
    }
    if (training && L.has_pair && L.bwd_pair.a.kern == CK_SMALLP) n.sp_cnt_n += smallp_counters(L.bwd_pair.a);
  }
}

static void carve_net(Net& n, Arena& ar, int es, bool training) {
  for (Tens& t : n.t) {
    if (t.name == "decoder_1" || t.name == "layer_5") {
      continue;
    }
    if (!t.is_input) t.y = ar.alloc(t.elems() * (t.hi ? sizeof(float) : (size_t)es));
    for (int k = 1; k < 3; ++k) if (t.need_act[k]) t.xa[k] = ar.alloc(t.elems() * es);
    if (t.has_bn) {
      const size_t gc = (size_t)n.groups * t.C * sizeof(float);
      t.bn.a = (float*)ar.alloc(gc); t.bn.b = (float*)ar.alloc(gc);
      t.bn.mu = (float*)ar.alloc(gc); t.bn.rstd = (float*)ar.alloc(gc);
      t.bn.c1 = (float*)ar.alloc(gc); t.bn.c2 = (float*)ar.alloc(gc);
      t.bn.c1g = (float*)ar.alloc(gc); t.bn.c2g = (float*)ar.alloc(gc);
      t.bn.pb = (training && t.pb_cap) ? (double*)ar.alloc((size_t)n.groups * t.pb_cap * 2 * t.C * sizeof(double)) : nullptr;
      t.bn.pbg = (training && t.pbg_cap) ? (double*)ar.alloc((size_t)t.pbg_cap * 2 * t.C * sizeof(double)) : nullptr;
    }
  }
  for (Layer& L : n.l) {
    if (!L.tapgemm) continue;
    const size_t q = (size_t)L.g.N * L.g.Hin * L.g.Win * 16;
    L.tap_S = (float*)ar.alloc(q * sizeof(float));
    L.tap_dyS = ar.alloc(q * es);
  }
  n.packed = (char*)ar.alloc(n.packed_elems * es);
  n.d_descs = (PackDesc*)ar.alloc(n.descs.size() * sizeof(PackDesc));
  n.sp_cnt = (unsigned*)ar.alloc((n.sp_cnt_n + 1) * sizeof(unsigned));
  {
    unsigned* c = n.sp_cnt;
    for (Layer& L : n.l) {
      if (L.fwd.a.kern == CK_SMALLP) { L.sp_cnt_fwd = c; c += c ? smallp_counters(L.fwd.a) : 0; }
      for (int s = 0; s < L.nsrc && training; ++s)
        if (L.need_bwd[s] && L.bwd[s].a.kern == CK_SMALLP) { L.sp_cnt_bwd[s] = c; c += c ? smallp_counters(L.bwd[s].a) : 0; }
      if (training && L.has_pair && L.bwd_pair.a.kern == CK_SMALLP) { L.sp_cnt_pair = c; c += c ? smallp_counters(L.bwd_pair.a) : 0; }
    }
  }
}

static size_t carve_all(vp_pixrefer* h, char* base, size_t cap, std::vector<std::pair<size_t, size_t>>* track = nullptr) {
  Arena ar(base);
  ar.track = track;
  const vp_pixrefer_desc& d = h->d;
  const int N = d.batch, H = d.height, es = h->es;
  const size_t px = (size_t)N * H * H;
  h->gin = ar.alloc(px * 8 * es);
  h->gfg = ar.alloc(px * 8 * es);
  h->y4 = (float*)ar.alloc(px * 4 * sizeof(float));
  h->o4 = (float*)ar.alloc(px * 4 * sizeof(float));
  h->outputs = (float*)ar.alloc(px * 3 * sizeof(float));
  h->outputs_fg = (float*)ar.alloc(px * 3 * sizeof(float));
  h->losses = (float*)ar.alloc(8 * sizeof(float));
  h->G.t[0].y = h->gin; h->G.t[1].y = h->gfg;
  carve_net(h->G, ar, es, d.training);
  if (d.training) {
    const int hd = H / 8 - 2;
    const size_t M = (size_t)N * hd * hd;
    h->din = ar.alloc(3 * px * 8 * es);
    h->vin = ar.alloc(2 * px * 8 * es);
    h->logits = (float*)ar.alloc(3 * M * sizeof(float));
    h->predict = (float*)ar.alloc(2 * M * sizeof(float));
    h->dl_d = ar.alloc(3 * M * 8 * es);
    h->dl_g = ar.alloc(M * 8 * es);
    h->d_din = ar.alloc(px * 8 * es);
    h->d_vin = ar.alloc(px * 8 * es);
    h->dy4 = ar.alloc(px * 8 * es);
    h->D.t[0].y = h->din; h->V.t[0].y = h->vin;
    carve_net(h->D, ar, es, true);
    carve_net(h->V, ar, es, true);
    for (Tens& t : h->G.t) if (!t.is_input && !t.is_f32) { t.dz = ar.alloc(t.elems() * es); if (t.hi) t.dz32 = ar.alloc(t.elems() * sizeof(float)); }
    for (Tens& t : h->D.t) if (!t.is_input && !t.is_f32) { t.dz = ar.alloc(t.elems() * es); t.dz2 = ar.alloc(t.elems() / 3 * es); }
    for (Net* n : {&h->G, &h->D})
      for (Tens& t : n->t) if (h->bf16 && !t.is_input && !t.has_bn && t.C == 64) t.cs_part = (double*)ar.alloc((size_t)512 * 2 * 64 * sizeof(double));
    for (Tens& t : h->V.t) if (!t.is_input) t.dz = ar.alloc(t.elems() / 2 * es);
    for (const Tens& t : h->V.t) if (t.pool >= 0) h->vpool_code[t.pool] = (unsigned char*)ar.alloc(t.elems() / 2);
    h->n_comp = composite_nblocks(N, H * H);
    h->n_perc = perceptual_nblocks((size_t)N * (H / 4) * (H / 4) * 256, h->bf16);
    h->comp_partial = (double*)ar.alloc((size_t)h->n_comp * 2 * sizeof(double));
    h->perc_partial = (double*)ar.alloc((size_t)h->n_perc * sizeof(double));
  }
  h->zeros = ar.alloc(256);
  for (int k = 0; k < (d.training ? 4 : 1); ++k) {
    h->lane[k].bn_partial = (double*)ar.alloc((size_t)1024 * 2 * 512 * sizeof(double));
    h->lane[k].scratch = (char*)ar.alloc(h->scratch_bytes);
  }
  return ar.total();
}

static IgemmArgs pool_fused_view(const IgemmPlan& p) {
  static unsigned char set[16] = {};
  IgemmArgs v = launch_view(p, p.form);
  v.pool_code = set;
  v.pool_src = 1;
  return v;
}

static void init_handle(vp_pixrefer* h, const vp_pixrefer_desc* d) {
  h->d = *d;
  h->bf16 = d->dtype == VP_BF16;
  h->es = h->bf16 ? 2 : 4;
  build_generator(h->G, d->batch, d->height, d->ngf, (!d->training && d->per_sample_bn) ? d->batch : 1);
  size_t smax = 0;
  plan_net(h->G, h->bf16, d->training, d->training, 0, &smax);
  if (d->training) {
    build_discriminator(h->D, d->batch, d->height, d->ndf);
    plan_net(h->D, h->bf16, true, true, d->batch, &smax);
    build_vgg(h->V, d->batch, d->height);
    for (Layer& L : h->V.l) L.g.N = 2 * d->batch;
    plan_net(h->V, h->bf16, true, false, d->batch, &smax, true);
    for (const Layer& L : h->V.l) {
      if (L.pool < 0) continue;
      const int k = L.pool, knob = pool_bwd_fused_knob();
      const IgemmArgs& ba = L.bwd_alt[0].a;
      const bool big = !k || (long long)ba.N * (ba.Hg / 4) * (ba.Wg / 16) >= 4096;
      h->pool_fuse_ok[k] = ((knob == 1 && big) || knob == 2 + k || knob == 4) && h->bf16 && conv_kernel_ok(pool_fused_view(L.bwd_alt[0]), h->bf16);
    }
  }
  h->scratch_bytes = smax + 256;
  h->params_dirty = true;
  h->vgg_dirty = true;
}

static bool valid_desc(const vp_pixrefer_desc* d) {
  if (!d) { set_err("pixrefer descriptor: null"); return false; }
  if (d->batch < 1 || d->height < 256 || d->height % 256 != 0) { set_err("pixrefer descriptor: batch %d / height %d (height must be a multiple of 256)", d->batch, d->height); return false; }
  if (d->ngf < 8 || (d->ngf & (d->ngf - 1)) || d->ndf < 8 || (d->ndf & (d->ndf - 1))) { set_err("pixrefer descriptor: ngf %d / ndf %d must be powers of two >= 8", d->ngf, d->ndf); return false; }
  if (d->ngf > 64 || d->ndf > 64) { set_err("pixrefer descriptor: ngf %d / ndf %d > 64 exceed the batch-norm workspace (512 channels)", d->ngf, d->ndf); return false; }
  if (!d->training && d->per_sample_bn && d->batch > 1024) { set_err("pixrefer descriptor: per-sample batch-norm supports at most 1024 frames per call (got %d)", d->batch); return false; }
  if (d->dtype != VP_F32 && d->dtype != VP_BF16) { set_err("pixrefer descriptor: dtype %d", d->dtype); return false; }
  if ((d->streams != 0 && d->streams != 1 && d->streams != 3 && d->streams != 4) || d->d_backward_fork < 0 || d->d_backward_fork > 3 || d->d_beside_vgg < 0 ||
      d->d_beside_vgg > 2) {
    set_err("pixrefer descriptor: schedule fields streams %d / d_backward_fork %d / d_beside_vgg %d", d->streams, d->d_backward_fork, d->d_beside_vgg);
    return false;
  }
  return true;
}

static char* at_sample(const Tens& t, const void* base, int sample0, int es) {
  return (char*)base + (size_t)sample0 * t.H * t.W * t.C * es;
}

static void fill_src(const Net& n, const Layer& L, PixSrc& x, int group_n, int sample0, int es) {
  for (int s = 0; s < 2; ++s) {
    x.ptr[s] = nullptr; x.C[s] = 0; x.aff_a[s] = nullptr; x.aff_b[s] = nullptr;
  }
  for (int s = 0; s < L.nsrc; ++s) {
    const Tens& t = n.t[L.src[s]];
    x.ptr[s] = at_sample(t, (L.in_act != ACT_NONE) ? t.xa[L.in_act] : t.y, sample0, es);
    x.C[s] = t.C;
  }
  x.act = ACT_NONE;
  x.group_n = group_n;
}

static Lane caller_lane(const vp_pixrefer* h, void* stream) {
  return Lane{(hipStream_t)stream, h->lane[LANE_CALLER].scratch, h->lane[LANE_CALLER].bn_partial};
}

static int after(hipEvent_t ev, hipStream_t from, hipStream_t to) {
  VP_HIP_CHECK(hipEventRecord(ev, from));
  VP_HIP_CHECK(hipStreamWaitEvent(to, ev, 0));
  return VP_OK;
}

static int run_pack(vp_pixrefer* h, Net& n, hipStream_t st) {
  if (n.descs.empty()) return VP_OK;
  VP_HIP_CHECK(launch_pack_weights(n.d_descs, (int)n.descs.size(), n.params, n.packed, h->bf16, st));
  return VP_OK;
}

static int run_bn_stats(vp_pixrefer* h, Net& n, Layer& L, int fused_chunks, const Lane& ln) {
  hipStream_t st = ln.s;
  Tens& t = n.t[L.out];
  BnArgs b;
  memset(&b, 0, sizeof(b));
  b.y = t.y; b.C = t.C; b.G = n.groups; b.Pg = (n.batch / n.groups) * t.H * t.W;
  b.nchunk = bn_nchunk(b.Pg, b.C, b.G, h->bf16);
  b.partial = ln.bn_partial;
  b.gamma = n.params + L.gamma_off; b.beta = n.params + L.beta_off;
  b.aff_a = t.bn.a; b.aff_b = t.bn.b; b.mu = t.bn.mu; b.rstd = t.bn.rstd;
  b.eps = 1e-5f;
  if (fused_chunks > 0) { b.nchunk = fused_chunks; VP_HIP_CHECK(launch_bn_finalize(b, st)); return VP_OK; }
  if (bn_small(b)) {
    VP_HIP_CHECK(launch_bn_small_fwd(b, t.xa[ACT_LRELU], t.xa[ACT_RELU], h->bf16, st));
    return 1;
  }
  VP_HIP_CHECK(launch_bn_stats(b, h->bf16, st));
  return VP_OK;
}

static bool plan_can_pool(const IgemmPlan& p) {
  if (conv_staging(p.a.kern) != CK_PATCH || (p.a.Hg & 1) || (p.a.Wg & 1)) return false;
  int bc, bp;
  igemm_tile(p.cfg, &bc, &bp);
  int th, tw;
  patch_tile_hw(bp, &th, &tw);
  return tw == 16 && th % 2 == 0;
}

static int epi_stat_chunks(const IgemmPlan& p, int batch, int groups) {
  const IgemmArgs& a = p.a;
  const int fam = conv_staging(a.kern);
  if (a.splitk != 1 || fam == CK_SMALLP || fam == CK_S2C64 || batch % groups) return 0;
  int bc, bp;
  igemm_tile(p.cfg, &bc, &bp);
  const int pg = (batch / groups) * a.Hg * a.Wg;
  if (!(fam || groups == 1 || pg % bp == 0)) return 0;
  int pth = 16, ptw = 16;
  patch_tile_hw(bp, &pth, &ptw);
  const int tpg = fam ? (batch / groups) * ((a.Hg + pth - 1) / pth) * ((a.Wg + ptw - 1) / ptw) : (pg + bp - 1) / bp;
  return a.nclass * tpg;
}

static int run_layer_fwd_half(vp_pixrefer* h, Net& n, Layer& L, int half, const Lane& ln, void* pool_out = nullptr, bool pool_only = false,
                              unsigned char* pool_code = nullptr) {
  IgemmArgs a = L.fwd_half.a;
  a.pool_out = pool_out;
  a.pool_only = pool_out && pool_only ? 1 : 0;
  a.pool_code = a.pool_only ? pool_code : nullptr;
  const int nb = a.N;
  fill_src(n, L, a.x, nb, half * nb, h->es);
  a.Wp = n.packed + L.pk_fwd_half * h->es;
  Tens& to = n.t[L.out];
  a.Y = at_sample(to, to.y, half * nb, h->es);
  a.bias = n.params + L.b_off;
  a.partial = nullptr;
  a.zeros = h->zeros;
  profile_tag((L.scope + (half ? ":fwd1" : ":fwd0")).c_str());
  VP_HIP_CHECK(launch_igemm(a, h->bf16, L.fwd_half.cfg, ln.s));
  return VP_OK;
}

static bool first_layer_acts_fused(const vp_pixrefer* h, const Net& n, const Layer& L) {
  return first_layer_shape(h->bf16, n, L) && L.fwd.a.kern == CK_CIN8;
}

static SmallPArgs smallp_args(const IgemmArgs& a, unsigned* cnt, const Lane& ln) {
  SmallPArgs sp;
  memset(&sp, 0, sizeof(sp));
  sp.g = a;
  sp.g.sp_cnt = cnt;
  for (int c = 0; c < 4; ++c) sp.tap_mask[c] = a.sp_mask[c];
  sp.slab = a.partial; sp.cnt = cnt; sp.part = ln.bn_partial;
  return sp;
}

static void smallp_bn_bwd(SmallPArgs& sp, Net& n, Tens& t) {
  const Layer& Lp = n.l[t.producer];
  sp.mode = SP_BWD_BN;
  if (t.hi) { sp.hi = 1; sp.dy_out = t.dz; }
  sp.bn_y = t.y; sp.bn_mu = t.bn.mu; sp.bn_rstd = t.bn.rstd; sp.bn_gamma = n.params + Lp.gamma_off;
  sp.c1 = t.bn.c1; sp.c2 = t.bn.c2;
  sp.dgamma = n.grads + Lp.gamma_off; sp.dbeta = n.grads + Lp.beta_off; sp.dbias_zero = n.grads + Lp.b_off;
  t.bn_bwd_done = true;
}

static int run_layer_fwd(vp_pixrefer* h, Net& n, Layer& L, const Lane& ln, void* pool_out = nullptr) {
  hipStream_t st = ln.s;
  IgemmArgs a = L.fwd.a;
  a.pool_out = pool_out;
  fill_src(n, L, a.x, n.batch / n.groups, 0, h->es);
  a.Wp = n.packed + L.pk_fwd * h->es;
  Tens& to = n.t[L.out];
  a.Y = L.tapgemm ? L.tap_S : to.y;
  a.bias = L.has_bn || L.tapgemm ? nullptr : n.params + L.b_off;
  a.partial = (float*)ln.scratch;
  a.zeros = h->zeros;
  if (a.kern == CK_SMALLP) {
    SmallPArgs sp = smallp_args(a, L.sp_cnt_fwd, ln);
    sp.mode = L.has_bn ? SP_FWD_BN : SP_PLAIN;
    sp.hi = to.hi ? 1 : 0;
    if (L.has_bn) {
      sp.gamma = n.params + L.gamma_off; sp.beta = n.params + L.beta_off;
      sp.aff_a = to.bn.a; sp.aff_b = to.bn.b; sp.mu = to.bn.mu; sp.rstd = to.bn.rstd;
      sp.out_lrelu = to.need_act[ACT_LRELU] ? to.xa[ACT_LRELU] : nullptr;
      sp.out_relu = to.need_act[ACT_RELU] ? to.xa[ACT_RELU] : nullptr;
      sp.eps = 1e-5f;
    }
    profile_tag((L.scope + ":fwd").c_str());
    VP_HIP_CHECK(launch_smallp(sp, h->bf16, st));
    if (!L.has_bn && (to.need_act[ACT_LRELU] || to.need_act[ACT_RELU]))
      VP_HIP_CHECK(launch_act_apply(to.y, nullptr, nullptr, to.C, (n.batch / n.groups) * to.H * to.W, (size_t)to.N * to.H * to.W,
                                    to.xa[ACT_LRELU], to.xa[ACT_RELU], h->bf16, st));
    return VP_OK;
  }
  bool fused_stats = false;
  int stat_chunks = 0;
  if (L.has_bn && a.kern == CK_DC256 && n.groups == 1) {
    stat_chunks = 2 * conv_dc256_grid(a);
    a.bn_part = ln.bn_partial; a.bn_tpg = 1 << 30; a.bn_nchunk = stat_chunks;
    fused_stats = true;
  } else if (L.has_bn && a.kern == CK_S2C64) {
    const int grid = conv_s2c64_grid(a);
    if ((size_t)n.groups * grid * 2 * to.C <= (size_t)1024 * 2 * 512 && n.groups <= 32) {
      stat_chunks = grid;
      a.bn_part = ln.bn_partial; a.bn_tpg = (n.batch / n.groups) * conv_s2c64_tiles_per_image(a); a.bn_nchunk = grid;
      fused_stats = true;
    }
  } else if (L.fwd_stats) {
    stat_chunks = epi_stat_chunks(L.fwd, n.batch, n.groups);
    a.bn_part = ln.bn_partial; a.bn_tpg = stat_chunks / a.nclass; a.bn_nchunk = stat_chunks;
    fused_stats = true;
  }
  bool acts_fused = false;
  if (first_layer_acts_fused(h, n, L)) {
    a.xa_lrelu = to.need_act[ACT_LRELU] ? to.xa[ACT_LRELU] : nullptr;
    a.xa_relu = to.need_act[ACT_RELU] ? to.xa[ACT_RELU] : nullptr;
    if (!h->store_first_raw) a.Y = nullptr;
    acts_fused = true;
  }
  profile_tag((L.scope + ":fwd").c_str());
  VP_HIP_CHECK(launch_igemm(a, h->bf16, L.fwd.cfg, st));
  if (L.tapgemm) {
    TapArgs ta;
    memset(&ta, 0, sizeof(ta));
    ta.S = L.tap_S; ta.bias = n.params + L.b_off; ta.y = (float*)to.y;
    ta.N = L.g.N; ta.Hin = L.g.Hin; ta.Win = L.g.Win; ta.Hout = L.g.Hout; ta.Wout = L.g.Wout; ta.ks = L.g.ks; ta.pad = L.g.pad;
    VP_HIP_CHECK(launch_tap_gather(ta, st));
  }
  bool acts_done = acts_fused;
  if (L.has_bn) {
    const int rc = run_bn_stats(h, n, L, fused_stats ? stat_chunks : 0, ln);
    if (rc < 0) return rc;
    acts_done = rc == 1;
  }
  if (!acts_done && (to.need_act[ACT_LRELU] || to.need_act[ACT_RELU])) {
    VP_HIP_CHECK(launch_act_apply(to.y, L.has_bn ? to.bn.a : nullptr, L.has_bn ? to.bn.b : nullptr, to.C,
                                  (n.batch / n.groups) * to.H * to.W, (size_t)to.N * to.H * to.W,
                                  to.xa[ACT_LRELU], to.xa[ACT_RELU], h->bf16, st));
  }
  return VP_OK;
}

static int run_layer_wgrad(vp_pixrefer* h, Net& n, Layer& L, const void* dy, const Sub& sub, const Lane& ln) {
  hipStream_t st = ln.s;
  const int es = h->es, sample0 = sub.sample0, nb = sub.nb;
  WgradArgs w = L.wg.a;
  PixSrc xs;
  fill_src(n, L, xs, n.batch / n.groups, sample0, es);
  PixSrc ds;
  set_single_src(ds, dy, L.g.CoutT, nullptr, nullptr, ACT_NONE, 0);
  if (L.g.kind == 0) { w.g = xs; w.d = ds; } else { w.g = ds; w.d = xs; }
  bool own_wgrad = false;
  if (L.tapgemm && h->bf16 && cout1_knob() > 0 && L.nsrc == 1 && !n.t[L.src[0]].is_input && !n.t[L.src[0]].hi && n.t[L.src[0]].xa[L.in_act] &&
      L.g.ks == 4 && L.g.stride == 1) {
    Tens& tx = n.t[L.src[0]];
    Cout1Args c;
    memset(&c, 0, sizeof(c));
    c.dy = dy; c.ld_dy = L.g.CoutT;
    c.ref = at_sample(tx, tx.xa[L.in_act], sample0, es);
    c.N = nb; c.H = tx.H; c.W = tx.W; c.C = tx.C; c.Ho = L.g.Hout; c.Wo = L.g.Wout; c.ks = L.g.ks; c.pad = L.g.pad;
    c.slabs = (float*)ln.scratch; c.dW = n.grads + L.w_off;
    const long long px = (long long)nb * tx.H * tx.W;
    const size_t cap = h->scratch_bytes / ((size_t)16 * 512 * sizeof(float));
    c.rows = (int)(px / 96 < wgrad1_rows_knob() ? px / 96 : wgrad1_rows_knob());
    if ((size_t)c.rows > cap) c.rows = (int)cap;
    if (c.rows >= 1 && L.g.Cin == 512 && conv_cout1_wgrad_eligible(c)) {
      profile_tag((L.scope + ":wgrad").c_str());
      VP_HIP_CHECK(launch_conv_cout1_wgrad(c, st));
      own_wgrad = true;
    }
  }
  if (L.tapgemm && !own_wgrad) {
    TapArgs ta;
    memset(&ta, 0, sizeof(ta));
    ta.dy = dy; ta.dyS = L.tap_dyS; ta.ld_dy = L.g.CoutT;
    ta.N = nb; ta.Hin = L.g.Hin; ta.Win = L.g.Win; ta.Hout = L.g.Hout; ta.Wout = L.g.Wout; ta.ks = L.g.ks; ta.pad = L.g.pad;
    VP_HIP_CHECK(launch_tap_spread(ta, h->bf16, st));
    set_single_src(w.g, L.tap_dyS, 16, nullptr, nullptr, ACT_NONE, 0);
    w.d = xs;
  }
  w.partial = (float*)ln.scratch;
  w.dW = n.grads + L.w_off;
  w.accumulate = 0;
  w.zeros = h->zeros;
  if (!own_wgrad) {
    profile_tag((L.scope + ":wgrad").c_str());
    VP_HIP_CHECK(launch_wgrad(w, h->bf16, L.wg.cfg, st));
  }
  float* db = n.grads + L.b_off;
  if (L.has_bn) {
  } else {
    BnArgs b;
    memset(&b, 0, sizeof(b));
    b.y = dy; b.C = L.g.CoutT; b.G = 1; b.Pg = nb * L.g.Hout * L.g.Wout;
    b.nchunk = bn_nchunk(b.Pg, b.C, 1, h->bf16);
    b.partial = ln.bn_partial;
    Tens& to = n.t[L.out];
    if (to.cs_chunks > 0 && dy == to.dz) {
      b.partial = to.cs_part; b.nchunk = to.cs_chunks;
      to.cs_chunks = 0;
      VP_HIP_CHECK(launch_colsum_tail(b, L.g.Cout, db, 0, st));
    } else {
      VP_HIP_CHECK(launch_colsum(b, L.g.Cout, db, 0, h->bf16, st));
    }
  }
  return VP_OK;
}

static void try_bst(vp_pixrefer* h, const Net& n, const Layer& L, const Sub& sub, IgemmArgs& a, const IgemmPlan& p, Tens& ts, int which, bool last) {
  const bool gpass = sub.gpass;
  if (!h->bst_on || !last || !ts.has_bn || ts.hi || ts.producer < 0 || ts.is_input) return;
  const int groups = (gpass || sub.alt) ? 1 : n.groups;
  if ((sub.nb / groups) * ts.H * ts.W <= 2048) return;
  if (a.y_f32 || a.ldY % 8 || a.Cout % 8 || a.ldY != ts.C) return;
  if (h->bst_on < 2 && (a.split_c || conv_staging(a.kern) == CK_PATCH || (L.tapgemm && gpass))) return;
  if (a.kern != CK_IGEMM && a.kern != CK_PATCH4 && !(a.kern == CK_PATCH2 && a.x.C[1] == 0)) return;
  const int chunks = epi_stat_chunks(p, sub.nb, groups);
  if (chunks <= 0 || chunks > (gpass ? ts.pbg_cap : ts.pb_cap)) return;
  double* part = gpass ? ts.bn.pbg : ts.bn.pb;
  const void* y = at_sample(ts, ts.y, sub.sample0, h->es);
  if (which == 0) { a.bn_part = part; a.bst_y = y; }
  else { a.bn_part2 = part; a.bst_y2 = y; }
  a.bn_tpg = chunks / a.nclass; a.bn_nchunk = chunks;
  (gpass ? ts.bst_chunks_g : ts.bst_chunks) = chunks;
  h->bst_count++;
}

static int run_layer_dgrad(vp_pixrefer* h, Net& n, Layer& L, const void* dy, const Sub& sub, const Lane& ln) {
  hipStream_t st = ln.s;
  const int es = h->es, sample0 = sub.sample0, nb = sub.nb;
  const bool alt = sub.alt, gpass = sub.gpass;
  const int group_n = n.batch / n.groups;
  const bool pair_sp = L.has_pair && L.bwd_pair.a.kern == CK_SMALLP;
  const bool pair_sp_ok = pair_sp && n.t[L.src[0]].has_bn && n.t[L.src[0]].dz_writes + 1 == n.t[L.src[0]].n_bwd_consumers &&
                          n.t[L.src[1]].dz_writes + 1 < n.t[L.src[1]].n_bwd_consumers;
  if (L.has_pair && !alt && !gpass && (!pair_sp || pair_sp_ok)) {
    Tens &t0 = n.t[L.src[0]], &t1 = n.t[L.src[1]];
    IgemmArgs a = L.bwd_pair.a;
    set_single_src(a.x, dy, L.g.CoutT, nullptr, nullptr, ACT_NONE, 0);
    a.Wp = n.packed + L.pk_bwd_pair * es;
    a.partial = (float*)ln.scratch;
    a.zeros = h->zeros;
    a.Y = t0.dz; a.accumulate = t0.dz_written ? 1 : 0;
    a.Y2 = t1.dz; a.accumulate2 = t1.dz_written ? 1 : 0;
    a.ref = at_sample(t0, t0.xa[L.in_act], sample0, es);
    a.ref2 = at_sample(t1, t1.xa[L.in_act], sample0, es);
    a.ref_act = L.in_act;
    a.ref_group_n = group_n;
    t0.dz_written = t1.dz_written = true;
    t0.dz_writes++; t1.dz_writes++;
    profile_tag((L.scope + ":bwd").c_str());
    if (pair_sp) {
      if (t0.hi) a.Y = t0.dz32;
      if (t1.hi) a.Y2 = t1.dz32;
      a.y2_f32 = t1.hi ? 1 : 0;
      SmallPArgs sp = smallp_args(a, L.sp_cnt_pair, ln);
      smallp_bn_bwd(sp, n, t0);
      VP_HIP_CHECK(launch_smallp(sp, h->bf16, st));
    } else {
      try_bst(h, n, L, sub, a, L.bwd_pair, t0, 0, t0.dz_writes == t0.n_bwd_consumers);
      try_bst(h, n, L, sub, a, L.bwd_pair, t1, 1, t1.dz_writes == t1.n_bwd_consumers);
      VP_HIP_CHECK(launch_igemm(a, h->bf16, L.bwd_pair.cfg, st));
    }
    return VP_OK;
  }
  for (int s = 0; s < L.nsrc; ++s) {
    if (!L.need_bwd[s]) continue;
    Tens& ts = n.t[L.src[s]];
    IgemmArgs a = alt ? L.bwd_alt[s].a : L.bwd[s].a;
    set_single_src(a.x, dy, L.g.CoutT, nullptr, nullptr, ACT_NONE, 0);
    a.Wp = n.packed + (alt ? L.pk_bwd_alt[s] : L.pk_bwd[s]) * es;
    a.partial = (float*)ln.scratch;
    if (ts.is_input) {
      a.Y = (n.groups == 3) ? h->d_din : h->d_vin;
      a.accumulate = 0;
    } else {
      a.Y = gpass ? ts.dz2 : ts.dz;
      if (ts.hi) {
        if (gpass || alt || a.kern != CK_SMALLP) { set_err("%s: float32 few-pixel tensor %s reached by a launch that is not the few-pixel kernel", L.scope.c_str(), ts.name.c_str()); return VP_ERR_STATE; }
        a.Y = ts.dz32; a.y_f32 = 1;
      }
      bool& written = gpass ? ts.dz2_written : ts.dz_written;
      a.accumulate = written ? 1 : 0;
      written = true;
      if (!gpass) {
        ts.dz_writes++;
      }
      a.ref = at_sample(ts, ts.xa[L.in_act], sample0, es);
      a.ref_act = L.in_act;
      a.ref_group_n = group_n;
    }
    a.zeros = h->zeros;
    profile_tag((L.scope + (alt ? ":bwdG" : ":bwd")).c_str());
    if (a.kern == CK_SMALLP && !alt) {
      SmallPArgs sp = smallp_args(a, L.sp_cnt_bwd[s], ln);
      const bool last = !ts.is_input && !gpass && ts.has_bn && ts.producer >= 0 && ts.dz_writes == ts.n_bwd_consumers && n.groups == 1;
      if (ts.hi && !last && ts.dz_writes == ts.n_bwd_consumers) { set_err("%s: float32 tensor %s needs its batch-norm backward in the launch", L.scope.c_str(), ts.name.c_str()); return VP_ERR_STATE; }
      if (last) {
        smallp_bn_bwd(sp, n, ts);
        if (ts.hi) sp.g.y_f32 = 0;
      }
      VP_HIP_CHECK(launch_smallp(sp, h->bf16, st));
      continue;
    }
    if (L.tapgemm && h->bf16 && cout1_knob() > 0 && !ts.is_input && !ts.hi && !a.accumulate && L.in_act == ACT_LRELU && L.g.ks == 4 && L.g.stride == 1) {
      const int groups = (gpass || alt) ? 1 : n.groups;
      Cout1Args c;
      memset(&c, 0, sizeof(c));
      c.dy = dy; c.ld_dy = L.g.CoutT;
      c.w = n.params + L.w_off;
      c.ref = a.ref; c.ref_act = a.ref_act;
      c.dx = a.Y;
      c.N = nb; c.H = ts.H; c.W = ts.W; c.C = ts.C; c.Ho = L.g.Hout; c.Wo = L.g.Wout; c.ks = L.g.ks; c.pad = L.g.pad;
      c.groups = groups;
      const int tiles = nb % groups ? 0 : ((nb / groups) * ts.H * ts.W + 15) >> 4;
      const int cap = gpass ? ts.pbg_cap : ts.pb_cap;
      const bool sums = h->bst_on && ts.has_bn && ts.producer >= 0 && (nb / groups) * ts.H * ts.W > 2048 && cap > 0;
      c.rows = tiles / 8 < cout1_knob() ? tiles / 8 : cout1_knob();
      if (c.rows > 512 / groups) c.rows = 512 / groups;
      if (sums && c.rows > cap) c.rows = cap;
      if ((long long)nb * ts.H * ts.W < 16384 || c.rows < 1) c.rows = 0;
      if (sums) { c.part = gpass ? ts.bn.pbg : ts.bn.pb; c.y = at_sample(ts, ts.y, sample0, es); }
      if (tiles > 0 && c.rows > 0 && conv_cout1_bwd_eligible(c)) {
        if (sums) { (gpass ? ts.bst_chunks_g : ts.bst_chunks) = c.rows; h->bst_count++; }
        VP_HIP_CHECK(launch_conv_cout1_bwd(c, st));
        continue;
      }
    }
    if (h->bst_on && h->bf16 && !ts.is_input && !ts.has_bn && ts.cs_part && !gpass && !alt && ts.producer >= 0 && !n.l[ts.producer].tapgemm &&
        (n.groups != 1 || ts.dz_writes == ts.n_bwd_consumers) && a.kern == CK_DC64) {
      a.colsum_part = ts.cs_part;
      ts.cs_chunks = conv_dc64_grid(a);
    }
    if (!ts.is_input) try_bst(h, n, L, sub, a, alt ? L.bwd_alt[s] : L.bwd[s], ts, 0, (gpass || n.groups != 1) ? true : ts.dz_writes == ts.n_bwd_consumers);
    VP_HIP_CHECK(launch_igemm(a, h->bf16, alt ? L.bwd_alt[s].cfg : L.bwd[s].cfg, st));
  }
  return VP_OK;
}

static int run_layer_bwd(vp_pixrefer* h, Net& n, Layer& L, const void* dy, bool want_dw, const Sub& sub, const Lane& ln) {
  int rc;
  if (want_dw && (rc = run_layer_wgrad(h, n, L, dy, sub, ln))) return rc;
  return run_layer_dgrad(h, n, L, dy, sub, ln);
}

static int run_bn_bwd(vp_pixrefer* h, Net& n, Layer& L, bool want_dw, const Sub& sub, int group0, int ng, const Lane& ln) {
  hipStream_t st = ln.s;
  const bool gpass = sub.gpass;
  Tens& t = n.t[L.out];
  if (!gpass && t.bn_bwd_done) { t.bn_bwd_done = false; return VP_OK; }
  if (t.hi) { set_err("%s: the batch-norm backward of a float32 few-pixel tensor runs inside the few-pixel launch only", L.scope.c_str()); return VP_ERR_STATE; }
  BnArgs b;
  memset(&b, 0, sizeof(b));
  b.y = at_sample(t, t.y, sub.sample0, h->es);
  b.dy = gpass ? t.dz2 : t.dz; b.dz = b.dy;
  b.C = t.C; b.G = ng; b.Pg = (sub.nb / ng) * t.H * t.W;
  b.nchunk = bn_nchunk(b.Pg, b.C, b.G, h->bf16);
  b.partial = ln.bn_partial;
  b.gamma = n.params + L.gamma_off;
  b.mu = t.bn.mu + (size_t)group0 * t.C; b.rstd = t.bn.rstd + (size_t)group0 * t.C;
  b.c1 = gpass ? t.bn.c1g : t.bn.c1; b.c2 = gpass ? t.bn.c2g : t.bn.c2;
  if (want_dw) { b.dgamma = n.grads + L.gamma_off; b.dbeta = n.grads + L.beta_off; b.dbias_zero = n.grads + L.b_off; }
  int& fused = gpass ? t.bst_chunks_g : t.bst_chunks;
  if (fused > 0) {
    b.partial = gpass ? t.bn.pbg : t.bn.pb;
    b.nchunk = fused;
    b.raw = 1;
    fused = 0;
    VP_HIP_CHECK(launch_bn_bwd_tail(b, h->bf16, st));
    return VP_OK;
  }
  if (bn_small(b)) { VP_HIP_CHECK(launch_bn_small_bwd(b, h->bf16, st)); return VP_OK; }
  VP_HIP_CHECK(launch_bn_bwd(b, h->bf16, st));
  return VP_OK;
}

static int vgg_forward(vp_pixrefer* h, int half, const Lane& ln, bool codes) {
  Net& V = h->V;
  const int N = h->d.batch, s0 = half > 0 ? N : 0;
  int rc;
  for (Layer& L : V.l) {
    const bool fuse = L.pool >= 0 && plan_can_pool(half < 0 ? L.fwd : L.fwd_half);
    const Tens& ti = V.t[L.out];
    void* pool_y = L.pool >= 0 ? at_sample(V.t[L.pool_t], V.t[L.pool_t].y, s0, h->es) : nullptr;
    if (half < 0) {
      rc = run_layer_fwd(h, V, L, ln, fuse ? pool_y : nullptr);
    } else {
      const bool code = fuse && codes && half == 1;
      rc = run_layer_fwd_half(h, V, L, half, ln, fuse ? pool_y : nullptr, half == 0 || code, code ? h->vpool_code[L.pool] : nullptr);
    }
    if (rc) return rc;
    if (L.pool >= 0 && !fuse) VP_HIP_CHECK(launch_maxpool_fwd(at_sample(ti, ti.y, s0, h->es), pool_y, half < 0 ? ti.N : N, ti.H, ti.W, ti.C, h->bf16, ln.s));
  }
  return VP_OK;
}

static int discriminator_gpass(vp_pixrefer* h, const Lane& ln) {
  Net& D = h->D;
  const int N = h->d.batch;
  const Sub fake{2 * N, N, true, true};
  int rc;
  for (Tens& t : D.t) { t.dz2_written = false; t.bst_chunks_g = 0; }
  for (int i = (int)D.l.size() - 1; i >= 0; --i) {
    Layer& L = D.l[i];
    if (L.has_bn) if ((rc = run_bn_bwd(h, D, L, false, fake, 2, 1, ln))) return rc;
    const void* dy = (i == (int)D.l.size() - 1) ? h->dl_g : D.t[L.out].dz2;
    if ((rc = run_layer_bwd(h, D, L, dy, false, fake, ln))) return rc;
  }
  return VP_OK;
}

static int vgg_backward(vp_pixrefer* h, const Lane& ln) {
  Net& V = h->V;
  const int N = h->d.batch, bf = h->bf16, es = h->es;
  for (Tens& t : V.t) t.dz_written = false;
  h->pool_bwd_fused = false;
  h->pool_dz_stale[0] = h->pool_dz_stale[1] = false;
  for (int i = (int)V.l.size() - 1; i >= 0; --i) {
    Layer& L = V.l[i];
    Tens& to = V.t[L.out];
    Tens& ti = V.t[L.src[0]];
    IgemmArgs a = L.bwd_alt[0].a;
    set_single_src(a.x, to.dz, L.g.CoutT, nullptr, nullptr, ACT_NONE, 0);
    if (L.pool >= 0 && h->pool_dz_stale[L.pool]) {
      a.x.ptr[0] = V.t[L.pool_t].dz;
      a.pool_code = h->vpool_code[L.pool];
      a.pool_src = 1;
    }
    a.Wp = V.packed + L.pk_bwd_alt[0] * es;
    a.partial = (float*)ln.scratch;
    if (ti.is_input) {
      a.Y = h->d_vin;
    } else {
      a.Y = ti.dz;
      if (ti.pool < 0) {
        a.ref = (const char*)ti.y + ti.elems() / 2 * es;
        a.ref_act = ACT_RELU;
      }
    }
    a.zeros = h->zeros;
    profile_tag((L.scope + ":bwd").c_str());
    VP_HIP_CHECK(launch_igemm(a, bf, L.bwd_alt[0].cfg, ln.s));
    if (ti.pool >= 0) {
      Tens& tc = V.t[ti.pool_src];
      const char* xin = (const char*)tc.y + tc.elems() / 2 * es;
      const int k = ti.pool;
      if (h->pool_codes_written && h->pool_fuse_ok[k]) {
        h->pool_dz_stale[k] = true;
        h->pool_bwd_fused = true;
      } else if (h->pool_codes_written) VP_HIP_CHECK(launch_maxpool_bwd_code(h->vpool_code[k], ti.dz, tc.dz, N, tc.H, tc.W, tc.C, bf, ln.s));
      else VP_HIP_CHECK(launch_maxpool_bwd(xin, ti.dz, tc.dz, N, tc.H, tc.W, tc.C, bf, ln.s));
    }
  }
  return VP_OK;
}

}

extern "C" {

static bool g_phase_marks = false;
static bool g_phase_detail = false;
void vp_phase_marks_enable(int on) { g_phase_marks = on != 0; g_phase_detail = on > 1; }
static void phase_mark(vp_pixrefer* h, hipStream_t st, int idx) {
  if (!g_phase_marks || idx >= 64) return;
  if (!h->marks_made) { for (int i = 0; i < 64; ++i) (void)hipEventCreate(&h->mark[i]); h->marks_made = true; }
  (void)hipEventRecord(h->mark[idx], st);
  if (idx + 1 > h->nmark) h->nmark = idx + 1;
}
float vp_pixrefer_mark_ms(vp_pixrefer_t* h, int from, int to) {
  if (!h || !h->marks_made || from < 0 || to < 0 || from >= 64 || to >= 64) return -1.f;
  float t = -1.f;
  if (hipEventSynchronize(h->mark[to]) != hipSuccess || hipEventElapsedTime(&t, h->mark[from], h->mark[to]) != hipSuccess) { (void)hipGetLastError(); return -1.f; }
  return t;
}
int vp_pixrefer_phase_ms(vp_pixrefer_t* h, float* ms, int cap) {
  if (!h || !ms) return 0;
  int n = 0;
  for (int i = 0; i + 1 < (h->nmark < 8 ? h->nmark : 8) && n < cap; ++i) {
    float t = 0.f;
    if (hipEventSynchronize(h->mark[i + 1]) != hipSuccess || hipEventElapsedTime(&t, h->mark[i], h->mark[i + 1]) != hipSuccess) {
      (void)hipGetLastError();
      break;
    }
    ms[n++] = t;
  }
  return n;
}
int vp_version(void) { return 100; }
const char* vp_last_error(void) { return g_err; }

static Net* manifest_net(const vp_pixrefer_desc* d, int which, vp_pixrefer* tmp) {
  if (which == 0) { build_generator(tmp->G, d->batch, d->height, d->ngf); return &tmp->G; }
  if (which == 1) { build_discriminator(tmp->D, d->batch, d->height, d->ndf); return &tmp->D; }
  if (which == 2) { build_vgg(tmp->V, d->batch, d->height); return &tmp->V; }
  return nullptr;
}

size_t vp_pixrefer_param_count(const vp_pixrefer_desc* d, int which) {
  if (!valid_desc(d)) return 0;
  vp_pixrefer tmp{};
  Net* n = manifest_net(d, which, &tmp);
  return n ? n->nparams : 0;
}

int vp_pixrefer_param_info(const vp_pixrefer_desc* d, int which, int index, char* name, int name_cap,
                           size_t* offset, int* ndim, int64_t shape[4]) {
  if (!valid_desc(d)) return VP_ERR_ARG;
  vp_pixrefer tmp{};
  Net* n = manifest_net(d, which, &tmp);
  if (!n || index < 0 || index >= (int)n->manifest.size()) return VP_ERR_ARG;
  const ParamInfo& p = n->manifest[index];
  if (name && name_cap > 0) { strncpy(name, p.name.c_str(), name_cap - 1); name[name_cap - 1] = 0; }
  if (offset) *offset = p.off;
  if (ndim) *ndim = p.ndim;
  if (shape) for (int i = 0; i < 4; ++i) shape[i] = p.shape[i];
  return VP_OK;
}

size_t vp_pixrefer_workspace_bytes(const vp_pixrefer_desc* d) {
  if (!valid_desc(d)) return 0;
  vp_pixrefer* h = new vp_pixrefer{};
  init_handle(h, d);
  const size_t n = carve_all(h, nullptr, 0);
  delete h;
  return n;
}

int vp_pixrefer_validate_plan(const vp_pixrefer_desc* d) {
  if (!valid_desc(d)) return VP_ERR_ARG;
  vp_pixrefer* h = new vp_pixrefer{};
  init_handle(h, d);
  const size_t need = carve_all(h, nullptr, 0);
  std::vector<std::pair<size_t, size_t>> regs;
  char* const base = reinterpret_cast<char*>((uintptr_t)1 << 40);
  carve_all(h, base, need, &regs);
  int rc = VP_OK;
  auto fail = [&](const char* fmt, auto... args) { if (rc == VP_OK) { set_err(fmt, args...); rc = VP_ERR_STATE; } };
  size_t prev_end = 0;
  for (size_t i = 0; i < regs.size(); ++i) {
    if (regs[i].first % 256) fail("region %zu at %zu: not 256-byte aligned", i, regs[i].first);
    if (regs[i].first < prev_end) fail("region %zu at %zu overlaps the previous one (ends %zu)", i, regs[i].first, prev_end);
    prev_end = regs[i].first + regs[i].second;
  }
  if (prev_end + 256 > need + 256 || prev_end > need) fail("carved %zu bytes of a %zu-byte workspace", prev_end, need);
  auto region_of = [&](const void* p, size_t bytes, const char* what) {
    if (!p) { fail("%s: null", what); return; }
    const size_t off = (size_t)((const char*)p - base);
    for (const auto& r : regs)
      if (off >= r.first && off + bytes <= r.first + r.second) return;
    fail("%s: [%zu, +%zu) is not inside a carved region", what, off, bytes);
  };
  const int es = h->es;
  for (Net* n : {&h->G, &h->D, &h->V}) {
    if (n->t.empty()) continue;
    for (const Tens& t : n->t) {
      const std::string nm = t.name;
      if (t.is_f32) continue;
      region_of(t.y, t.elems() * (t.hi ? 4 : es), (nm + ".y").c_str());
      for (int k = 1; k < 3; ++k) if (t.need_act[k]) region_of(t.xa[k], t.elems() * es, (nm + ".xa").c_str());
      if (t.has_bn) {
        const size_t gc = (size_t)n->groups * t.C * sizeof(float);
        for (const float* p : {t.bn.a, t.bn.b, t.bn.mu, t.bn.rstd, t.bn.c1, t.bn.c2, t.bn.c1g, t.bn.c2g}) region_of(p, gc, (nm + ".bn").c_str());
        if (d->training && t.pb_cap) region_of(t.bn.pb, (size_t)n->groups * t.pb_cap * 2 * t.C * sizeof(double), (nm + ".bn.pb").c_str());
        if (d->training && t.pbg_cap) region_of(t.bn.pbg, (size_t)t.pbg_cap * 2 * t.C * sizeof(double), (nm + ".bn.pbg").c_str());
        if ((size_t)n->groups * t.C > (size_t)1024 * 512) fail("%s: %d groups x %d channels exceed the batch-norm partial rows", nm.c_str(), n->groups, t.C);
      }
      if (t.cs_part) region_of(t.cs_part, (size_t)512 * 2 * 64 * sizeof(double), (nm + ".cs_part").c_str());
      if (d->training && !t.is_input) {
        const size_t div = n == &h->V ? 2 : 1;
        region_of(t.dz, t.elems() / div * es, (nm + ".dz").c_str());
        if (t.hi) region_of(t.dz32, t.elems() * 4, (nm + ".dz32").c_str());
        if (n == &h->D) region_of(t.dz2, t.elems() / 3 * es, (nm + ".dz2").c_str());
      }
    }
    region_of(n->packed, n->packed_elems * es, "packed weights");
    region_of(n->d_descs, n->descs.size() * sizeof(PackDesc), "pack descriptors");
    for (const PackDesc& p : n->descs) {
      const size_t pe = (size_t)p.nclass * p.Kpad * p.rows_pad;
      if (p.dst_off + pe > n->packed_elems) fail("pack block [%zu, +%zu) outside the %zu-element packed arena", p.dst_off, pe, n->packed_elems);
      if (p.src_off >= n->nparams) fail("pack source %zu outside the %zu-float parameter arena", p.src_off, n->nparams);
    }
    size_t pend = 0;
    for (const ParamInfo& p : n->manifest) {
      size_t cnt = 1;
      for (int i = 0; i < 4; ++i) cnt *= (size_t)p.shape[i];
      if (p.off != pend) fail("parameter %s at %zu: arena not contiguous (expected %zu)", p.name.c_str(), p.off, pend);
      pend = p.off + cnt;
    }
    if (pend != n->nparams) fail("parameter manifest covers %zu of %zu floats", pend, n->nparams);
    for (const Layer& L : n->l) {
      auto plan_ok = [&](const IgemmPlan& p, const char* what) {
        if (p.partial_bytes > h->scratch_bytes) fail("%s %s: split-K slab %zu > scratch %zu", L.scope.c_str(), what, p.partial_bytes, h->scratch_bytes);
        if (p.a.splitk < 1 || p.a.CoutPad < p.a.Cout) fail("%s %s: splitk %d CoutPad %d", L.scope.c_str(), what, p.a.splitk, p.a.CoutPad);
        if (!conv_kernel_ok(launch_view(p, p.form), h->bf16))
          fail("%s %s: the launch is outside the preconditions of its kernel %s", L.scope.c_str(), what, conv_kernel_name(p.a.kern));
      };
      plan_ok(L.fwd, "fwd");
      if (L.has_fwd_half) plan_ok(L.fwd_half, "fwd_half");
      if (d->training && L.has_pair) plan_ok(L.bwd_pair, "bwd_pair");
      if (d->training)
        for (int s2 = 0; s2 < L.nsrc; ++s2) if (L.need_bwd[s2]) { plan_ok(L.bwd[s2], "bwd"); if (n == &h->D || n == &h->V) plan_ok(L.bwd_alt[s2], "bwd_alt"); }
      if (d->training && n != &h->V && L.wg.partial_bytes > h->scratch_bytes) fail("%s wgrad: slab %zu > scratch %zu", L.scope.c_str(), L.wg.partial_bytes, h->scratch_bytes);
      if (L.tapgemm) { region_of(L.tap_S, (size_t)L.g.N * L.g.Hin * L.g.Win * 16 * 4, "tap_S"); region_of(L.tap_dyS, (size_t)L.g.N * L.g.Hin * L.g.Win * 16 * es, "tap_dyS"); }
    }
  }
  const size_t px = (size_t)d->batch * d->height * d->height;
  region_of(h->gin, px * 8 * es, "gin"); region_of(h->gfg, px * 8 * es, "gfg");
  region_of(h->y4, px * 4 * 4, "y4"); region_of(h->o4, px * 4 * 4, "o4");
  region_of(h->outputs, px * 3 * 4, "outputs"); region_of(h->outputs_fg, px * 3 * 4, "outputs_fg");
  static const char* const lane_scratch[4] = {"scratch", "scratch2", "scratch3", "scratch4"};
  static const char* const lane_bnp[4] = {"bn_partial", "bn_partial2", "bn_partial3", "bn_partial4"};
  for (int k = 0; k < (d->training ? 4 : 1); ++k) {
    region_of(h->lane[k].scratch, h->scratch_bytes, lane_scratch[k]);
    region_of(h->lane[k].bn_partial, (size_t)1024 * 2 * 512 * 8, lane_bnp[k]);
  }
  if (d->training) {
    const int hd = d->height / 8 - 2;
    const size_t M = (size_t)d->batch * hd * hd;
    region_of(h->din, 3 * px * 8 * es, "din"); region_of(h->vin, 2 * px * 8 * es, "vin");
    region_of(h->logits, 3 * M * 4, "logits"); region_of(h->predict, 2 * M * 4, "predict");
    region_of(h->dl_d, 3 * M * 8 * es, "dl_d"); region_of(h->dl_g, M * 8 * es, "dl_g");
    region_of(h->d_din, px * 8 * es, "d_din"); region_of(h->d_vin, px * 8 * es, "d_vin"); region_of(h->dy4, px * 8 * es, "dy4");
    for (const Tens& t : h->V.t) if (t.pool >= 0) region_of(h->vpool_code[t.pool], t.elems() / 2, (t.name + " codes").c_str());
    for (const Layer& L : h->V.l) {
      const int k = L.pool;
      if (k < 0 || !h->pool_fuse_ok[k]) continue;
      const Tens& tp = h->V.t[L.pool_t];
      if (tp.pool != k || tp.pool_src != L.out || tp.H * 2 != h->V.t[L.out].H || tp.C != h->V.t[L.out].C) fail("%s: the tensor behind it is not its 2x2 pool", L.scope.c_str());
      if (L.bwd_alt[0].a.kern != CK_C64 || !conv_kernel_ok(pool_fused_view(L.bwd_alt[0]), h->bf16)) fail("%s bwd_alt: no pooled-source form of kernel %s", L.scope.c_str(), conv_kernel_name(L.bwd_alt[0].a.kern));
      region_of(tp.dz, tp.elems() / 2 * es, (tp.name + ".dz (pooled-source read)").c_str());
      region_of(h->vpool_code[k], tp.elems() / 2, (tp.name + " codes (pooled-source read)").c_str());
    }
  }
  delete h;
  return rc;
}

struct StreamPool {
  int dev = -1;
  hipStream_t side = nullptr, branch = nullptr, branch2 = nullptr;
};
static StreamPool g_pool;
static std::mutex g_pool_mu;

static int pool_streams(bool want_b2, hipStream_t* side, hipStream_t* branch, hipStream_t* branch2) {
  std::lock_guard<std::mutex> lk(g_pool_mu);
  int dev = 0;
  VP_HIP_CHECK(hipGetDevice(&dev));
  if (g_pool.dev >= 0 && g_pool.dev != dev) { set_err("the step executor's streams were created on device %d, this plan is on device %d (one device per process)", g_pool.dev, dev); return VP_ERR_STATE; }
  if (!g_pool.side) {
    int prio_lo = 0, prio_hi = 0;
    (void)hipDeviceGetStreamPriorityRange(&prio_lo, &prio_hi);
    VP_HIP_CHECK(hipStreamCreateWithPriority(&g_pool.side, hipStreamNonBlocking, prio_lo));
    VP_HIP_CHECK(hipStreamCreateWithFlags(&g_pool.branch, hipStreamNonBlocking));
    g_pool.dev = dev;
  }
  if (want_b2 && !g_pool.branch2) VP_HIP_CHECK(hipStreamCreateWithFlags(&g_pool.branch2, hipStreamNonBlocking));
  if (side) *side = g_pool.side;
  if (branch) *branch = g_pool.branch;
  if (branch2) *branch2 = g_pool.branch2;
  return VP_OK;
}

int vp_reserve_streams(void) { return pool_streams(true, nullptr, nullptr, nullptr); }

void* vp_host_stream(void) {
  hipStream_t b2 = nullptr;
  if (pool_streams(true, nullptr, nullptr, &b2)) return nullptr;
  return (void*)b2;
}

int vp_pixrefer_create(const vp_pixrefer_desc* d, void* workspace, size_t workspace_bytes,
                       float* params_g, float* params_d, const float* params_vgg,
                       float* grads_g, float* grads_d, void* stream, vp_pixrefer_t** out) {
  if (!valid_desc(d) || !workspace || !params_g || !out) { set_err("vp_pixrefer_create: bad argument"); return VP_ERR_ARG; }
  if (d->training && (!params_d || !params_vgg || !grads_g || !grads_d)) { set_err("training needs D/VGG params and grad arenas"); return VP_ERR_ARG; }
  vp_pixrefer* h = new vp_pixrefer{};
  init_handle(h, d);
  const size_t need = carve_all(h, nullptr, 0);
  if (workspace_bytes < need) { set_err("workspace too small: %zu < %zu", workspace_bytes, need); delete h; return VP_ERR_WORKSPACE; }
  carve_all(h, (char*)workspace, workspace_bytes);
  h->G.params = params_g; h->G.grads = grads_g;
  h->D.params = params_d; h->D.grads = grads_d;
  h->V.params = const_cast<float*>(params_vgg);
  for (Tens& t : h->G.t) if (t.is_f32) { t.y = h->y4; t.dz = h->dy4; }
  hipStream_t st = (hipStream_t)stream;
  VP_HIP_CHECK(hipMemsetAsync(h->zeros, 0, 256, st));
  if (d->training) for (Tens& t : h->D.t) if (t.is_f32) { t.y = h->logits; t.dz = h->dl_d; }
  for (Net* n : {&h->G, &h->D, &h->V}) {
    if (n->descs.empty()) continue;
    VP_HIP_CHECK(hipMemcpyAsync(n->d_descs, n->descs.data(), n->descs.size() * sizeof(PackDesc), hipMemcpyHostToDevice, st));
    VP_HIP_CHECK(hipMemsetAsync(n->sp_cnt, 0, (n->sp_cnt_n + 1) * sizeof(unsigned), st));
  }
  VP_HIP_CHECK(hipStreamSynchronize(st));
  h->overlap = false; h->forked = false;
  h->bst_on = 1; h->vgg_fork_layer = 3;
  h->ov_on = true; h->store_first_raw = false; h->dfork_point = d->d_backward_fork ? d->d_backward_fork - 1 : 2; h->dsplit_on = d->d_beside_vgg != 1;
  if (d->training && d->streams != 1) {
    { const int rc = pool_streams(false, &h->lane[LANE_SIDE].s, &h->lane[LANE_BRANCH].s, &h->lane[LANE_BRANCH2].s); if (rc) { delete h; return rc; } }
    VP_HIP_CHECK(hipEventCreateWithFlags(&h->ev_fork, hipEventDisableTiming));
    VP_HIP_CHECK(hipEventCreateWithFlags(&h->ev_join, hipEventDisableTiming));
    h->use_b2 = d->streams != 3;
    VP_HIP_CHECK(hipEventCreateWithFlags(&h->ev_b2join, hipEventDisableTiming));
    VP_HIP_CHECK(hipEventCreateWithFlags(&h->ev_bfork, hipEventDisableTiming));
    VP_HIP_CHECK(hipEventCreateWithFlags(&h->ev_bjoin, hipEventDisableTiming));
    VP_HIP_CHECK(hipEventCreateWithFlags(&h->ev_upd_b, hipEventDisableTiming));
    VP_HIP_CHECK(hipEventCreateWithFlags(&h->ev_upd_m, hipEventDisableTiming));
    h->overlap = true;
  }
  *out = h;
  return VP_OK;
}

void vp_pixrefer_destroy(vp_pixrefer_t* h) {
  if (!h) return;
  if (h->marks_made) for (int i = 0; i < 64; ++i) (void)hipEventDestroy(h->mark[i]);
  if (h->overlap) {
    for (int k = LANE_SIDE; k <= LANE_BRANCH2; ++k) if (h->lane[k].s) (void)hipStreamSynchronize(h->lane[k].s);
    for (hipEvent_t ev : {h->ev_fork, h->ev_join, h->ev_bfork, h->ev_bjoin, h->ev_b2join, h->ev_upd_b, h->ev_upd_m}) (void)hipEventDestroy(ev);
  }
  delete h;
}

int vp_pixrefer_params_changed(vp_pixrefer_t* h) {
  if (!h) return VP_ERR_ARG;
  h->params_dirty = true;
  h->vgg_dirty = true;
  h->upd_mask = 0;
  return VP_OK;
}

int vp_pixrefer_optimizer_stepped(vp_pixrefer_t* h) {
  if (!h) return VP_ERR_ARG;
  h->params_dirty = true;
  return VP_OK;
}

static int forward_impl(vp_pixrefer_t* h, const float* inputs, const float* fg_inputs, int fg_c, const float* targets, const float* masks, void* stream);

int vp_pixrefer_forward(vp_pixrefer_t* h, const float* inputs, const float* fg_inputs,
                        const float* targets, const float* masks, void* stream) {
  return forward_impl(h, inputs, fg_inputs, 6, targets, masks, stream);
}

int vp_pixrefer_forward_fg3(vp_pixrefer_t* h, const float* inputs, const float* fg_inputs3, const float* targets, void* stream) {
  if (h && h->d.training) { set_err("vp_pixrefer_forward_fg3: inference plans only (the training graph reads fg_inputs[..., 3:], pixrefer.py:297,321)"); return VP_ERR_STATE; }
  return forward_impl(h, inputs, fg_inputs3, 3, targets, nullptr, stream);
}

size_t vp_pixrefer_desc_size(void) { return sizeof(vp_pixrefer_desc); }

static int forward_impl(vp_pixrefer_t* h, const float* inputs, const float* fg_inputs, int fg_c, const float* targets, const float* masks, void* stream) {
  if (!h || !inputs || !fg_inputs || !targets) { set_err("vp_pixrefer_forward: null argument"); return VP_ERR_ARG; }
  const vp_pixrefer_desc& d = h->d;
  if (d.training && !masks) { set_err("vp_pixrefer_forward: masks required when training"); return VP_ERR_ARG; }
  const Lane me = caller_lane(h, stream);
  const Lane &side = h->lane[LANE_SIDE], &branch = h->lane[LANE_BRANCH];
  hipStream_t st = me.s;
  const int N = d.batch, H = d.height, bf = h->bf16;
  int rc;
  if (h->params_dirty) {
    if ((rc = run_pack(h, h->G, st))) return rc;
    if (d.training) {
      if ((rc = run_pack(h, h->D, st))) return rc;
      if (h->vgg_dirty) { if ((rc = run_pack(h, h->V, st))) return rc; h->vgg_dirty = false; }
    }
    h->params_dirty = false;
  }
  h->in_targets = targets; h->in_masks = masks;
  PackInputsArgs pi;
  memset(&pi, 0, sizeof(pi));
  pi.inputs = inputs; pi.fg_inputs = fg_inputs; pi.gin = h->gin; pi.gfg = h->gfg; pi.din = h->din; pi.vin = h->vin;
  pi.N = N; pi.HW = H * H; pi.train = d.training; pi.fg_c = fg_c;
  phase_mark(h, st, 0);
  VP_HIP_CHECK(launch_pack_inputs(pi, bf, st));

  bool split_vgg = d.training && h->overlap && h->ov_on;
  if (split_vgg) for (Layer& L : h->V.l) split_vgg = split_vgg && L.has_fwd_half;
  bool vgg_real_pending = split_vgg;
  auto vgg_real_half = [&]() -> int {
    vgg_real_pending = false;
    if ((rc = after(h->ev_fork, st, side.s))) return rc;
    if ((rc = vgg_forward(h, 0, side, false))) return rc;
    VP_HIP_CHECK(hipEventRecord(h->ev_join, side.s));
    return VP_OK;
  };
  if (vgg_real_pending && h->vgg_fork_layer <= 0 && (rc = vgg_real_half())) return rc;

  const bool split_enc = d.training && h->overlap && h->ov_on;
  if (split_enc) {
    if ((rc = after(h->ev_bfork, st, branch.s))) return rc;
    for (Layer& L : h->G.l) if (L.fg) if ((rc = run_layer_fwd(h, h->G, L, branch))) return rc;
    VP_HIP_CHECK(hipEventRecord(h->ev_bjoin, branch.s));
  }
  for (int i = 0; i < (int)h->G.l.size(); ++i) {
    Layer& L = h->G.l[i];
    if (split_enc && L.fg) continue;
    if (split_enc && i == h->G.i_me2) VP_HIP_CHECK(hipStreamWaitEvent(st, h->ev_bjoin, 0));
    if (vgg_real_pending && i >= h->vgg_fork_layer && (rc = vgg_real_half())) return rc;
    if (g_phase_detail) phase_mark(h, st, 8 + i);
    if ((rc = run_layer_fwd(h, h->G, L, me))) return rc;
  }

  if (vgg_real_pending && (rc = vgg_real_half())) return rc;
  CompositeArgs ca;
  memset(&ca, 0, sizeof(ca));
  ca.y4 = h->y4; ca.targets = targets; ca.masks = masks; ca.o4 = h->o4; ca.outputs = h->outputs; ca.outputs_fg = h->outputs_fg;
  ca.din = h->din; ca.vin = h->vin; ca.partial = h->comp_partial; ca.N = N; ca.HW = H * H; ca.train = d.training;
  VP_HIP_CHECK(launch_composite_fwd(ca, bf, st));
  phase_mark(h, st, 1);
  if (!d.training) return VP_OK;

  const bool split_d = h->overlap && h->ov_on && h->dsplit_on;
  const Lane& ld = split_d ? branch : me;
  if (split_d && (rc = after(h->ev_bfork, st, branch.s))) return rc;
  for (Layer& L : h->D.l) if ((rc = run_layer_fwd(h, h->D, L, ld))) return rc;
  const int hd = H / 8 - 2;
  GanLossArgs ga;
  memset(&ga, 0, sizeof(ga));
  ga.logits = h->logits; ga.dl_d = h->dl_d; ga.dl_g = h->dl_g; ga.predict = h->predict; ga.losses = h->losses;
  ga.M = N * hd * hd; ga.gan_weight = d.gan_weight;
  VP_HIP_CHECK(launch_gan_loss(ga, bf, ld.s));
  if (split_d) VP_HIP_CHECK(hipEventRecord(h->ev_bjoin, branch.s));

  Net& V = h->V;
  bool codes = split_vgg && bf && !h->store_first_raw && h->vpool_code[0] && h->vpool_code[1];
  for (Layer& L : V.l)
    if (L.pool >= 0) codes = codes && plan_can_pool(L.fwd_half);
  h->pool_codes_written = codes;
  if ((rc = vgg_forward(h, split_vgg ? 1 : -1, me, codes))) return rc;
  if (split_vgg) VP_HIP_CHECK(hipStreamWaitEvent(st, h->ev_join, 0));
  const Tens& f3 = V.t.back();
  PerceptualArgs pa;
  memset(&pa, 0, sizeof(pa));
  pa.f3 = f3.y; pa.df3 = f3.dz; pa.partial = h->perc_partial; pa.half = f3.elems() / 2; pa.l1_weight = d.l1_weight;
  VP_HIP_CHECK(launch_perceptual(pa, bf, st));

  if (split_d) VP_HIP_CHECK(hipStreamWaitEvent(st, h->ev_bjoin, 0));
  LossFinalArgs lf;
  memset(&lf, 0, sizeof(lf));
  lf.comp_partial = h->comp_partial; lf.n_comp = h->n_comp; lf.perc_partial = h->perc_partial; lf.n_perc = h->n_perc;
  lf.n_out = (double)N * H * H * 3; lf.n_feat = (double)pa.half; lf.losses = h->losses;
  lf.l1_weight = d.l1_weight; lf.gan_weight = d.gan_weight;
  VP_HIP_CHECK(launch_loss_final(lf, st));
  phase_mark(h, st, 2);
  return VP_OK;
}

static int backward_d_on(vp_pixrefer_t* h, const Lane& ln);
static int fork_d(vp_pixrefer_t* h, hipStream_t st);

static float adam_lr_t(float lr, float beta1, float beta2, int t) {
  return (float)((double)lr * sqrt(1.0 - pow((double)beta2, t)) / (1.0 - pow((double)beta1, t)));
}

static void bucket_range(const Net& G, int bucket, int* l0, int* l1, size_t* off0, size_t* off1) {
  const int last = (int)G.l.size() - 1;
  *l0 = bucket == 0 ? G.i_md5 : (bucket == 1 ? G.i_me2 : 0);
  *l1 = bucket == 0 ? last : (bucket == 1 ? G.i_md5 - 1 : G.i_me2 - 1);
  *off0 = G.l[*l0].w_off;
  *off1 = *l1 < last ? G.l[*l1 + 1].w_off : G.nparams;
}

static int update_range(vp_pixrefer_t* h, Net& n, float* m, float* v, float lr_t, size_t off0, size_t off1, int l0, int l1, hipStream_t s) {
  if (off1 > off0) {
    AdamArgs a;
    a.p = n.params + off0; a.g = n.grads + off0; a.m = m + off0; a.v = v + off0; a.n = off1 - off0;
    a.lr_t = lr_t; a.beta1 = h->upd.beta1; a.beta2 = h->upd.beta2; a.eps = h->upd.eps;
    VP_HIP_CHECK(launch_adam(a, s));
  }
  const size_t d0 = n.l[l0].desc0, d1 = n.l[l1].desc1;
  if (d1 > d0) VP_HIP_CHECK(launch_pack_weights(n.d_descs + d0, (int)(d1 - d0), n.params, n.packed, h->bf16, s));
  return VP_OK;
}
static int update_d(vp_pixrefer_t* h, hipStream_t s) {
  h->upd.d_done = true;
  return update_range(h, h->D, h->upd.m_d, h->upd.v_d, h->upd.lr_t_d, 0, h->D.nparams, 0, (int)h->D.l.size() - 1, s);
}

int vp_pixrefer_backward(vp_pixrefer_t* h, void* stream) {
  if (!h || !h->d.training) { set_err("vp_pixrefer_backward: needs a training plan"); return VP_ERR_STATE; }
  hipStream_t st = (hipStream_t)stream;
  if (!h->overlap || !h->ov_on) {
    int rc = vp_pixrefer_backward_d(h, stream);
    if (rc) return rc;
    return vp_pixrefer_backward_g(h, stream);
  }
  int rc;
  h->dfork_pending = h->dfork_point;
  if (h->dfork_pending == 0 && (rc = fork_d(h, st))) { h->dfork_pending = 0; return rc; }
  rc = vp_pixrefer_backward_g(h, stream);
  h->dfork_pending = 0;
  if (rc) return rc;
  VP_HIP_CHECK(hipStreamWaitEvent(st, h->ev_join, 0));
  phase_mark(h, st, 7);
  return VP_OK;
}

static int fork_d(vp_pixrefer_t* h, hipStream_t st) {
  const Lane& side = h->lane[LANE_SIDE];
  h->dfork_pending = 0;
  int rc = after(h->ev_fork, st, side.s);
  if (rc) return rc;
  if ((rc = backward_d_on(h, side))) return rc;
  if (h->upd.active && h->dfork_point == 2 && (rc = update_d(h, side.s))) return rc;
  VP_HIP_CHECK(hipEventRecord(h->ev_join, side.s));
  return VP_OK;
}

int vp_pixrefer_backward_update(vp_pixrefer_t* h, float* m_g, float* v_g, float* m_d, float* v_d, int step_t_g, int step_t_d,
                                float lr, float beta1, float beta2, float eps, void* stream) {
  if (!h || !h->d.training) { set_err("vp_pixrefer_backward_update: needs a training plan"); return VP_ERR_STATE; }
  if (!m_g || !v_g || !m_d || !v_d || step_t_g < 1 || step_t_d < 1) { set_err("vp_pixrefer_backward_update: bad argument"); return VP_ERR_ARG; }
  h->upd.active = true; h->upd.d_done = false;
  h->upd.m_g = m_g; h->upd.v_g = v_g; h->upd.m_d = m_d; h->upd.v_d = v_d;
  h->upd.lr_t_g = adam_lr_t(lr, beta1, beta2, step_t_g); h->upd.lr_t_d = adam_lr_t(lr, beta1, beta2, step_t_d); h->upd.beta1 = beta1; h->upd.beta2 = beta2; h->upd.eps = eps;
  int rc = vp_pixrefer_backward(h, stream);
  if (!rc && !h->upd.d_done) rc = update_d(h, (hipStream_t)stream);
  h->upd.active = false;
  if (rc) return rc;
  h->params_dirty = false;
  return VP_OK;
}

int vp_pixrefer_update_bucket(vp_pixrefer_t* h, int which, int bucket, float* m, float* v, int step_t, float lr, float beta1, float beta2,
                              float eps, void* stream) {
  if (!h || !h->d.training || !m || !v || step_t < 1 || which < 0 || which > 1 || bucket < 0 || bucket > (which ? 0 : 2)) {
    set_err("vp_pixrefer_update_bucket: bad argument");
    return VP_ERR_ARG;
  }
  const float lr_t = adam_lr_t(lr, beta1, beta2, step_t);
  h->upd.beta1 = beta1; h->upd.beta2 = beta2; h->upd.eps = eps;
  int rc;
  if (which == 1) {
    rc = update_range(h, h->D, m, v, lr_t, 0, h->D.nparams, 0, (int)h->D.l.size() - 1, (hipStream_t)stream);
    h->upd_mask |= 8;
  } else {
    int l0, l1;
    size_t off0, off1;
    bucket_range(h->G, bucket, &l0, &l1, &off0, &off1);
    rc = update_range(h, h->G, m, v, lr_t, off0, off1, l0, l1, (hipStream_t)stream);
    h->upd_mask |= 1 << bucket;
  }
  if (rc) return rc;
  if (h->upd_mask == 15) { h->upd_mask = 0; h->params_dirty = false; }
  return VP_OK;
}

int vp_pixrefer_backward_d(vp_pixrefer_t* h, void* stream) {
  if (!h || !h->d.training) { set_err("vp_pixrefer_backward_d: needs a training plan"); return VP_ERR_STATE; }
  return backward_d_on(h, caller_lane(h, stream));
}

int vp_pixrefer_backward_d_fork(vp_pixrefer_t* h, void* stream) {
  if (!h || !h->d.training) { set_err("vp_pixrefer_backward_d_fork: needs a training plan"); return VP_ERR_STATE; }
  hipStream_t st = (hipStream_t)stream;
  h->forked = h->overlap && h->ov_on;
  if (!h->forked) return backward_d_on(h, caller_lane(h, stream));
  h->dfork_pending = h->dfork_point;
  if (h->dfork_pending == 0) return fork_d(h, st);
  return VP_OK;
}

void* vp_pixrefer_side_stream(vp_pixrefer_t* h) { return (h && h->overlap) ? (void*)h->lane[LANE_SIDE].s : nullptr; }

int vp_pixrefer_use_streams(vp_pixrefer_t* h, int n) {
  if (!h || (n != 3 && n != 4)) { set_err("vp_pixrefer_use_streams: 3 or 4"); return VP_ERR_ARG; }
  h->use_b2 = (n == 4) && h->overlap;
  return VP_OK;
}

int vp_pixrefer_set_option(vp_pixrefer_t* h, const char* key, int value) {
  if (!h || !key) { set_err("vp_pixrefer_set_option: null argument"); return VP_ERR_ARG; }
  const std::string k(key);
  if (k == "overlap") { h->ov_on = value != 0; return VP_OK; }
  if (k == "d_backward_fork") { h->dfork_point = value < 0 ? 0 : (value > 2 ? 2 : value); return VP_OK; }
  if (k == "d_beside_vgg") { h->dsplit_on = value != 0; return VP_OK; }
  if (k == "store_first_raw") { h->store_first_raw = value != 0; return VP_OK; }
  if (k == "bwd_sums_in_epilogue") { h->bst_on = value < 0 ? 0 : (value > 2 ? 2 : value); return VP_OK; }
  if (k == "vgg_real_fork") { h->vgg_fork_layer = value < 0 ? 0 : value; return VP_OK; }
  set_err("vp_pixrefer_set_option: unknown key %s", key);
  return VP_ERR_ARG;
}

long long vp_pixrefer_counter(vp_pixrefer_t* h, const char* key) {
  if (!h || !key) return -1;
  if (std::string(key) == "bwd_sums_launches") return h->bst_count;
  if (std::string(key) == "pool_codes_written") return h->pool_codes_written ? 1 : 0;
  if (std::string(key) == "pool_bwd_fused") return h->pool_bwd_fused ? 1 : 0;
  return -1;
}

int vp_pixrefer_backward_d_join(vp_pixrefer_t* h, void* stream) {
  if (!h || !h->d.training) { set_err("vp_pixrefer_backward_d_join: needs a training plan"); return VP_ERR_STATE; }
  if (h->forked && h->dfork_pending) {
    const int rc = fork_d(h, (hipStream_t)stream);
    if (rc) return rc;
  }
  if (h->forked) VP_HIP_CHECK(hipStreamWaitEvent((hipStream_t)stream, h->ev_join, 0));
  h->forked = false;
  return VP_OK;
}

static int backward_d_on(vp_pixrefer_t* h, const Lane& ln) {
  const Sub all{0, 3 * h->d.batch, false, false};
  int rc;
  Net& D = h->D;

  for (Tens& t : D.t) { t.dz_written = false; t.bst_chunks = 0; t.cs_chunks = 0; }
  for (int i = (int)D.l.size() - 1; i >= 0; --i) {
    Layer& L = D.l[i];
    Tens& to = D.t[L.out];
    if (L.has_bn) if ((rc = run_bn_bwd(h, D, L, true, all, 0, 3, ln))) return rc;
    const bool save = L.need_bwd[0];
    if (i == 0) L.need_bwd[0] = false;
    rc = run_layer_bwd(h, D, L, to.dz, true, all, ln);
    L.need_bwd[0] = save;
    if (rc) return rc;
  }

  return VP_OK;
}

int vp_pixrefer_backward_g(vp_pixrefer_t* h, void* stream) { return vp_pixrefer_backward_g_stage(h, -1, stream); }

int vp_pixrefer_backward_g_stages(void) { return 3; }

static int backward_g_head(vp_pixrefer_t* h, const Lane& me) {
  const vp_pixrefer_desc& d = h->d;
  hipStream_t st = me.s;
  int rc;
  const bool split_d = h->overlap && h->ov_on && h->dsplit_on;
  const Lane& ld = split_d ? h->lane[LANE_BRANCH] : me;
  if (split_d && (rc = after(h->ev_bfork, st, ld.s))) return rc;
  if ((rc = discriminator_gpass(h, ld))) return rc;
  if (split_d) VP_HIP_CHECK(hipEventRecord(h->ev_bjoin, ld.s));
  if (h->dfork_pending == 1 && (rc = fork_d(h, st))) return rc;
  if ((rc = vgg_backward(h, me))) return rc;
  if (split_d) VP_HIP_CHECK(hipStreamWaitEvent(st, h->ev_bjoin, 0));
  if (h->dfork_pending == 2 && (rc = fork_d(h, st))) return rc;
  CompositeArgs ca;
  memset(&ca, 0, sizeof(ca));
  ca.targets = h->in_targets; ca.masks = h->in_masks; ca.o4 = h->o4; ca.outputs = h->outputs;
  ca.d_din = h->d_din; ca.d_vin = h->d_vin; ca.dy4 = h->dy4; ca.N = d.batch; ca.HW = d.height * d.height; ca.l1_weight = d.l1_weight;
  VP_HIP_CHECK(launch_composite_bwd(ca, h->bf16, st));
  phase_mark(h, st, 3);
  for (Tens& t : h->G.t) { t.dz_written = false; t.dz_writes = 0; t.bn_bwd_done = false; t.bst_chunks = 0; t.cs_chunks = 0; }
  return VP_OK;
}

int vp_pixrefer_backward_g_stage(vp_pixrefer_t* h, int stage, void* stream) {
  if (!h || !h->d.training) { set_err("vp_pixrefer_backward_g: needs a training plan"); return VP_ERR_STATE; }
  if (stage > 2) { set_err("vp_pixrefer_backward_g_stage: stage must be < 3"); return VP_ERR_ARG; }
  const Lane me = caller_lane(h, stream);
  const Lane &side = h->lane[LANE_SIDE], &branch = h->lane[LANE_BRANCH], &b2 = h->lane[LANE_BRANCH2];
  hipStream_t st = me.s;
  const Sub all{0, h->d.batch, false, false};
  int rc;
  Net& G = h->G;
  int l_lo = 0, l_hi = (int)G.l.size() - 1;
  size_t off0, off1;
  if (stage >= 0) bucket_range(G, stage, &l_lo, &l_hi, &off0, &off1);
  if (stage <= 0 && (rc = backward_g_head(h, me))) return rc;
  const bool split_enc = h->overlap && h->ov_on && l_lo == 0;
  const bool wsplit = h->overlap && h->ov_on;
  bool forked = false;
  const Lane* fgl = nullptr;
  for (int i = l_hi; i >= l_lo; --i) {
    Layer& L = G.l[i];
    Tens& to = G.t[L.out];
    const bool fg = split_enc && L.fg;
    if (fg && !fgl) {
      VP_HIP_CHECK(hipEventRecord(h->ev_bfork, st));
      if (h->use_b2 && !b2.s && (rc = pool_streams(true, nullptr, nullptr, &h->lane[LANE_BRANCH2].s))) return rc;
      fgl = h->use_b2 ? &b2 : &branch;
      VP_HIP_CHECK(hipStreamWaitEvent(fgl->s, h->ev_bfork, 0));
      forked = true;
    }
    const Lane& ln = fg ? *fgl : me;
    if (i == G.i_md5 - 1) phase_mark(h, st, 4);
    if (i == G.i_me2 - 1) phase_mark(h, st, 5);
    if (g_phase_detail && !fg) phase_mark(h, st, 32 + i);
    if (L.has_bn) if ((rc = run_bn_bwd(h, G, L, true, all, 0, 1, ln))) return rc;
    if (wsplit && !fg) {
      if ((rc = after(h->ev_bfork, st, branch.s))) return rc;
      forked = true;
      if ((rc = run_layer_wgrad(h, G, L, to.dz, all, branch))) return rc;
      if ((rc = run_layer_dgrad(h, G, L, to.dz, all, me))) return rc;
    } else {
      if ((rc = run_layer_bwd(h, G, L, to.dz, true, all, ln))) return rc;
    }
    const int bucket = i == G.i_md5 ? 0 : (i == G.i_me2 ? 1 : (i == 0 ? 2 : -1));
    if (h->upd.active && bucket >= 0) {
      int l0, l1;
      bucket_range(G, bucket, &l0, &l1, &off0, &off1);
      hipStream_t su = st;
      const bool on_side = wsplit && h->dfork_pending == 0;
      if (on_side) {
        VP_HIP_CHECK(hipEventRecord(h->ev_upd_b, branch.s));
        VP_HIP_CHECK(hipEventRecord(h->ev_upd_m, st));
        VP_HIP_CHECK(hipStreamWaitEvent(side.s, h->ev_upd_b, 0));
        VP_HIP_CHECK(hipStreamWaitEvent(side.s, h->ev_upd_m, 0));
        if (fgl == &b2 && (rc = after(h->ev_b2join, b2.s, side.s))) return rc;
        su = side.s;
      } else if (wsplit) {
        if ((rc = after(h->ev_bfork, st, branch.s))) return rc;
        if (fgl == &b2 && (rc = after(h->ev_b2join, b2.s, branch.s))) return rc;
        su = branch.s; forked = true;
      }
      if ((rc = update_range(h, G, h->upd.m_g, h->upd.v_g, h->upd.lr_t_g, off0, off1, l0, l1, su))) return rc;
      if (on_side) VP_HIP_CHECK(hipEventRecord(h->ev_join, side.s));
    }
  }
  if (forked) {
    if (g_phase_detail && (stage < 0 || stage == 2)) phase_mark(h, st, 60);
    if ((rc = after(h->ev_bjoin, branch.s, st))) return rc;
    if (fgl == &b2 && (rc = after(h->ev_b2join, b2.s, st))) return rc;
  }
  if (stage < 0 || stage == 2) phase_mark(h, st, 6);
  return VP_OK;
}

int vp_profile_enable(int on) { profile_enable(on); return VP_OK; }
size_t vp_profile_collect(char* json, size_t cap) { return profile_collect(json, cap); }

int vp_pixrefer_tensor(vp_pixrefer_t* h, const char* name, void** ptr, int64_t shape[4], int* dtype) {
  if (!h || !name || !ptr) return VP_ERR_ARG;
  const int N = h->d.batch, H = h->d.height;
  auto ret = [&](void* p, int64_t a, int64_t b, int64_t c, int64_t e, int dt) {
    *ptr = p;
    if (shape) { shape[0] = a; shape[1] = b; shape[2] = c; shape[3] = e; }
    if (dtype) *dtype = dt;
    return p ? VP_OK : VP_ERR_STATE;
  };
  const std::string s(name);
  const int cd = h->bf16 ? VP_BF16 : VP_F32;
  if (s == "Outputs_raw") return ret(h->outputs, N, H, H, 3, VP_F32);
  if (s == "Outputs_FG") return ret(h->outputs_fg, N, H, H, 3, VP_F32);
  if (s == "gen_out4") return ret(h->o4, N, H, H, 4, VP_F32);
  if (s == "losses") return ret(h->losses, 8, 1, 1, 1, VP_F32);
  const int hd = H / 8 - 2;
  if (s == "Predict") return ret(h->predict, 2, N, hd, hd, VP_F32);
  if (s == "logits") return ret(h->logits, 3 * N, hd, hd, 1, VP_F32);
  if (s == "d_gen_out4") return ret(h->dy4, N, H, H, 8, cd);
  if (s == "d_din") return ret(h->d_din, N, H, H, 8, cd);
  if (s == "d_vin") return ret(h->d_vin, N, H, H, 8, cd);
  const size_t c = s.find('/');
  if (c == std::string::npos) return VP_ERR_ARG;
  const std::string net = s.substr(0, c);
  std::string rest = s.substr(c + 1);
  Net* n = net == "g" ? &h->G : net == "d" ? &h->D : net == "v" ? &h->V : nullptr;
  if (!n) return VP_ERR_ARG;
  std::string field;
  const size_t k = rest.find(':');
  if (k != std::string::npos) { field = rest.substr(k + 1); rest = rest.substr(0, k); }
  for (Tens& t : n->t) {
    if (t.name != rest) continue;
    if (field.empty() && !h->store_first_raw && t.producer >= 0 && first_layer_acts_fused(h, *n, n->l[t.producer])) {
      set_err("vp_pixrefer_tensor: the raw output of %s is not stored (its kernel writes the consumers' activations); vp_pixrefer_set_option(h, \"store_first_raw\", 1) before the forward pass", s.c_str());
      return VP_ERR_STATE;
    }
    if (field.empty() && n == &h->V && h->pool_codes_written && (t.name == "conv1/conv1_2" || t.name == "conv2/conv2_2")) {
      set_err("vp_pixrefer_tensor: the full-resolution output of %s is not stored (the step keeps its 2x2 max pool and the pool's arg-max codes); vp_pixrefer_set_option(h, \"store_first_raw\", 1) before the forward pass", s.c_str());
      return VP_ERR_STATE;
    }
    if (field.empty()) return ret(t.y, t.N, t.H, t.W, t.is_f32 ? (t.name == "decoder_1" ? 4 : 1) : t.C, (t.is_f32 || t.hi) ? VP_F32 : cd);
    if (field == "dz32") return t.hi ? ret(t.dz32, t.N, t.H, t.W, t.C, VP_F32) : VP_ERR_ARG;
    if (field == "dy" && n == &h->V && (t.name == "conv1/conv1_2" || t.name == "conv2/conv2_2") && h->pool_dz_stale[t.name == "conv2/conv2_2"]) {
      const int k = t.name == "conv2/conv2_2";
      const Tens& tp = n->t[(&t - n->t.data()) + 1];
      VP_HIP_CHECK(hipDeviceSynchronize());
      VP_HIP_CHECK(launch_maxpool_bwd_code(h->vpool_code[k], tp.dz, t.dz, t.N / 2, t.H, t.W, t.C, h->bf16, nullptr));
      VP_HIP_CHECK(hipDeviceSynchronize());
      h->pool_dz_stale[k] = false;
    }
    if (field == "dy") return ret(t.dz, n == &h->V ? t.N / 2 : t.N, t.H, t.W, t.C, cd);
    if (!t.has_bn) return VP_ERR_ARG;
    if (field == "scale") return ret(t.bn.a, n->groups, t.C, 1, 1, VP_F32);
    if (field == "shift") return ret(t.bn.b, n->groups, t.C, 1, 1, VP_F32);
    if (field == "mean") return ret(t.bn.mu, n->groups, t.C, 1, 1, VP_F32);
    if (field == "rstd") return ret(t.bn.rstd, n->groups, t.C, 1, 1, VP_F32);
    return VP_ERR_ARG;
  }
  return VP_ERR_ARG;
}

int vp_pixrefer_fetch(vp_pixrefer_t* h, int what, void* dst, void* stream) {
  if (!h || !dst || what < 0 || what > 3) { set_err("vp_pixrefer_fetch: bad argument"); return VP_ERR_ARG; }
  FetchArgs f;
  memset(&f, 0, sizeof(f));
  f.raw3 = h->outputs; f.fg3 = h->outputs_fg; f.o4 = h->o4; f.dst = dst;
  f.npix = (size_t)h->d.batch * h->d.height * h->d.height;
  f.mode = what;
  if (what == 3 && h->d.training) {
    VP_HIP_CHECK(hipMemcpyAsync(dst, h->outputs_fg, f.npix * 3 * sizeof(float), hipMemcpyDeviceToDevice, (hipStream_t)stream));
    return VP_OK;
  }
  VP_HIP_CHECK(launch_fetch(f, (hipStream_t)stream));
  return VP_OK;
}

int vp_grad_pack_bf16(const float* src, void* dst_bf16, size_t n, void* stream) {
  if (!src || !dst_bf16 || n < 1 || ((uintptr_t)src & 31) || ((uintptr_t)dst_bf16 & 15)) { set_err("vp_grad_pack_bf16: bad argument"); return VP_ERR_ARG; }
  VP_HIP_CHECK(launch_grad_pack_bf16(src, dst_bf16, n, (hipStream_t)stream));
  return VP_OK;
}
int vp_grad_unpack_bf16(const void* src_bf16, float* dst, size_t n, float scale, void* stream) {
  if (!src_bf16 || !dst || n < 1 || ((uintptr_t)dst & 31) || ((uintptr_t)src_bf16 & 15)) { set_err("vp_grad_unpack_bf16: bad argument"); return VP_ERR_ARG; }
  VP_HIP_CHECK(launch_grad_unpack_bf16(src_bf16, dst, n, scale, (hipStream_t)stream));
  return VP_OK;
}

int vp_adam_tf(float* params, const float* grads, float* m, float* v, size_t n, int step_t,
               float lr, float beta1, float beta2, float eps, void* stream) {
  if (!params || !grads || !m || !v || step_t < 1) { set_err("vp_adam_tf: bad argument"); return VP_ERR_ARG; }
  AdamArgs a;
  a.p = params; a.g = grads; a.m = m; a.v = v; a.n = n;
  a.lr_t = adam_lr_t(lr, beta1, beta2, step_t);
  a.beta1 = beta1; a.beta2 = beta2; a.eps = eps;
  VP_HIP_CHECK(launch_adam(a, (hipStream_t)stream));
  return VP_OK;
}

}
```

Baseline: 4504 frames/s.

## Run discriminator forward on real-image groups early on a side stream

Splits the discriminator forward into sub-launches so the two groups that do not depend on the generator output run on a separate stream, overlapped with the generator forward. Only the fake group runs after the composite, and then it joins with the early real-group work. Per-group batch-norm statistics, partial tables and the s2c64 kernel's tile offset (tile0) are adjusted so sub-launches reproduce the full-batch plan. The cost is more launches and extra events, plus possible contention with the generator kernels on the GPU.

```diff
diff --git a/voicepuppet_amd/csrc/conv_args.h b/voicepuppet_amd/csrc/conv_args.h
--- a/voicepuppet_amd/csrc/conv_args.h
+++ b/voicepuppet_amd/csrc/conv_args.h
@@ -86,6 +86,7 @@
   unsigned* sp_cnt;
   unsigned short sp_mask[4];
   int sp_npt, sp_lcpt;
+  int tile0;
 };
 
 struct WgradArgs {
diff --git a/voicepuppet_amd/csrc/conv_ops.h b/voicepuppet_amd/csrc/conv_ops.h
--- a/voicepuppet_amd/csrc/conv_ops.h
+++ b/voicepuppet_amd/csrc/conv_ops.h
@@ -116,6 +116,7 @@
 inline int& patch4_knob() { static int v = 1; return v; }
 inline int& c64_knob() { static int v = 1; return v; }
 inline int& pool_bwd_fused_knob() { static int v = 1; return v; }
+inline int& d_real_early_knob() { static int v = 1; return v; }
 inline int& cout1_knob() { static int v = 256; return v; }
 inline int& wgrad1_rows_knob() { static int v = 512; return v; }
 inline int& dc64_knob() { static int v = 1; return v; }
diff --git a/voicepuppet_amd/csrc/conv_prof.h b/voicepuppet_amd/csrc/conv_prof.h
--- a/voicepuppet_amd/csrc/conv_prof.h
+++ b/voicepuppet_amd/csrc/conv_prof.h
@@ -6,6 +6,7 @@
 namespace vp {
 
 void profile_enable(int on);
+bool profile_enabled();
 void profile_tag(const char* tag);
 size_t profile_collect(char* out, size_t cap);
 
diff --git a/voicepuppet_amd/csrc/conv_prof.hip b/voicepuppet_amd/csrc/conv_prof.hip
--- a/voicepuppet_amd/csrc/conv_prof.hip
+++ b/voicepuppet_amd/csrc/conv_prof.hip
@@ -21,6 +21,7 @@
 static std::string g_prof_tag;
 static bool g_prof_detail = false;
 void profile_enable(int on) { g_prof_on = on != 0; g_prof_detail = on > 1; }
+bool profile_enabled() { return g_prof_on; }
 void profile_tag(const char* tag) { if (g_prof_on && g_prof_detail) g_prof_tag = tag ? tag : ""; }
 
 const char* g_prof_family = nullptr;
diff --git a/voicepuppet_amd/csrc/conv_s2c64.hip b/voicepuppet_amd/csrc/conv_s2c64.hip
--- a/voicepuppet_amd/csrc/conv_s2c64.hip
+++ b/voicepuppet_amd/csrc/conv_s2c64.hip
@@ -123,13 +123,14 @@
     done_mask |= 1u << grp;
   };
 
-  if (bt < ntiles) issue_patch(bt, 0);
+  const int tfirst = (bt + GT - a.tile0 % GT) % GT;
+  if (tfirst < ntiles) issue_patch(tfirst, 0);
 #pragma unroll
   for (int t = 0; t < 16; ++t)
 #pragma unroll
     for (int c = 0; c < NCH; ++c) asm volatile("" : "+v"(W[t][c].x), "+v"(W[t][c].y), "+v"(W[t][c].z), "+v"(W[t][c].w));
   int it = 0;
-  for (int t = bt; t < ntiles; t += GT, ++it) {
+  for (int t = tfirst; t < ntiles; t += GT, ++it) {
     const int buf = it & 1;
     if (it == 0) wait_vm<0>();
     else wait_vm<NST>();
@@ -265,7 +266,9 @@
   const int pair = a.split_c ? 1 : 0;
   int grid = conv_s2c64_grid(a);
   if (pair) grid = 2 * ntiles < 512 ? 2 * ntiles : 512;
-  if (a.bn_part && (pair || a.bn_nchunk != grid || a.bn_tpg <= 0 || (ntiles + a.bn_tpg - 1) / a.bn_tpg > 32)) return hipErrorInvalidValue;
+  if (a.tile0 && (!a.bn_part || a.tile0 < 0 || a.bn_tpg <= 0 || a.tile0 % a.bn_tpg)) return hipErrorInvalidValue;
+  if (a.bn_part && (pair || a.bn_nchunk < grid || a.bn_nchunk > 256 || a.bn_tpg <= 0 || (ntiles + a.bn_tpg - 1) / a.bn_tpg > 32)) return hipErrorInvalidValue;
+  if (a.bn_part) grid = a.bn_nchunk;
   const int ki = pair ? 2 : (a.bn_part ? 1 : 0);
   void (*kerns[3])(const IgemmArgs, const int) = {conv_s2c64_kernel<false, false>, conv_s2c64_kernel<true, false>, conv_s2c64_kernel<false, true>};
   void (*kern)(const IgemmArgs, const int) = kerns[ki];
diff --git a/voicepuppet_amd/csrc/ops_api.hip b/voicepuppet_amd/csrc/ops_api.hip
--- a/voicepuppet_amd/csrc/ops_api.hip
+++ b/voicepuppet_amd/csrc/ops_api.hip
@@ -73,6 +73,7 @@
       {"c64", &c64_knob(), TUNE_PLAIN},
       {"dc64", &dc64_knob(), TUNE_PLAIN},
       {"pool_bwd_fused", &pool_bwd_fused_knob(), TUNE_0_TO_4, 1},
+      {"d_real_early", &d_real_early_knob(), TUNE_0_TO_4, 1},
       {"cout1_wgrad_rows", &wgrad1_rows_knob(), TUNE_POSITIVE},
       {"cout1_bwd", &cout1_knob(), TUNE_NEG_RESETS, 256},
       {"s2c64", &s2c64_knob(), TUNE_PLAIN},
diff --git a/voicepuppet_amd/csrc/plan_pixrefer.hip b/voicepuppet_amd/csrc/plan_pixrefer.hip
--- a/voicepuppet_amd/csrc/plan_pixrefer.hip
+++ b/voicepuppet_amd/csrc/plan_pixrefer.hip
@@ -79,6 +79,7 @@
   IgemmPlan fwd_half;
   size_t pk_fwd_half = 0;
   bool has_fwd_half = false;
+  IgemmPlan fwd_sub[2];
   WgradPlan wg;
   size_t desc0 = 0, desc1 = 0;
   bool tapgemm = false;
@@ -107,12 +108,17 @@
   PackDesc* d_descs = nullptr;
   unsigned* sp_cnt = nullptr;
   size_t sp_cnt_n = 0;
+  bool has_subs = false;
+  std::string sub_why;
 };
 
 struct Lane { hipStream_t s; char* scratch; double* bn_partial; };
 enum { LANE_CALLER = 0, LANE_SIDE = 1, LANE_BRANCH = 2, LANE_BRANCH2 = 3 };
+enum { D_EARLY_SIDE_BEHIND = 2, D_EARLY_SIDE_FRONT = 3, D_EARLY_BRANCH2 = 4, D_EARLY_DEFAULT = D_EARLY_BRANCH2 };
 
 struct Sub { int sample0, nb; bool alt, gpass; };
+
+struct FwdSub { int sample0, nb, group0, ng; const IgemmPlan* plan; };
 
 }
 
@@ -131,6 +137,10 @@
   bool pool_fuse_ok[2];
   bool pool_bwd_fused;
   bool pool_dz_stale[2];
+  int d_early;
+  int d_fork_layer;
+  bool d_early_last;
+  hipEvent_t ev_dfork, ev_djoin;
   double *comp_partial, *perc_partial;
   Lane lane[4];
   hipEvent_t ev_b2join;
@@ -452,6 +462,38 @@
     }
     if (training && L.has_pair && L.bwd_pair.a.kern == CK_SMALLP) n.sp_cnt_n += smallp_counters(L.bwd_pair.a);
   }
+}
+
+static void plan_fwd_subs(Net& n, int bf16) {
+  n.has_subs = false;
+  n.sub_why.clear();
+  char why[256];
+  const int gn = n.batch / n.groups;
+  for (Layer& L : n.l) {
+    for (int k = 0; k < 2 && n.sub_why.empty(); ++k) {
+      IgemmPlan& s = L.fwd_sub[k];
+      s = L.fwd;
+      const int ng = k ? 1 : n.groups - 1;
+      s.a.N = ng * gn;
+      s.partial_bytes = s.a.splitk > 1 ? (size_t)s.a.nclass * s.a.splitk * s.a.N * s.a.Hg * s.a.Wg * s.a.CoutPad * sizeof(float) : 0;
+      const IgemmArgs v = launch_view(s, s.form);
+      const Tens& to = n.t[L.out];
+      const bool s2_rows = L.fwd.a.kern == CK_S2C64 && (size_t)n.groups * conv_s2c64_grid(L.fwd.a) * 2 * to.C <= (size_t)1024 * 2 * 512 && n.groups <= 32;
+      BnArgs bs;
+      memset(&bs, 0, sizeof(bs));
+      bs.Pg = gn * to.H * to.W;
+      if (L.fwd.a.kern == CK_SMALLP) snprintf(why, sizeof(why), "%s runs on the few-pixel kernel", L.scope.c_str());
+      else if (pick_conv_kernel(v, bf16) != L.fwd.a.kern || !conv_kernel_ok(v, bf16))
+        snprintf(why, sizeof(why), "%s: kernel %s of the %d-sample launch does not take %d samples", L.scope.c_str(), conv_kernel_name(L.fwd.a.kern), n.batch, s.a.N);
+      else if (L.fwd_stats && epi_stat_chunks(s, s.a.N, ng) != epi_stat_chunks(L.fwd, n.batch, n.groups))
+        snprintf(why, sizeof(why), "%s: the statistics rows of %d samples are not those of the %d-sample launch", L.scope.c_str(), s.a.N, n.batch);
+      else if (L.has_bn && !L.fwd_stats && !s2_rows && bn_small(bs))
+        snprintf(why, sizeof(why), "%s: the batch-norm over %d pixels per group is one launch (bn_small_fwd)", L.scope.c_str(), bs.Pg);
+      else continue;
+      n.sub_why = why;
+    }
+  }
+  n.has_subs = n.sub_why.empty();
 }
 
 static void carve_net(Net& n, Arena& ar, int es, bool training) {
@@ -558,6 +600,11 @@
   if (d->training) {
     build_discriminator(h->D, d->batch, d->height, d->ndf);
     plan_net(h->D, h->bf16, true, true, d->batch, &smax);
+    plan_fwd_subs(h->D, h->bf16);
+    {
+      const int knob = d_real_early_knob();
+      h->d_early = !h->D.has_subs ? 0 : (knob == 1 ? D_EARLY_DEFAULT : knob);
+    }
     build_vgg(h->V, d->batch, d->height);
     for (Layer& L : h->V.l) L.g.N = 2 * d->batch;
     plan_net(h->V, h->bf16, true, false, d->batch, &smax, true);
@@ -622,20 +669,22 @@
   return VP_OK;
 }
 
-static int run_bn_stats(vp_pixrefer* h, Net& n, Layer& L, int fused_chunks, const Lane& ln) {
+static int run_bn_stats(vp_pixrefer* h, Net& n, Layer& L, int fused_chunks, const Lane& ln, const FwdSub& fs) {
   hipStream_t st = ln.s;
   Tens& t = n.t[L.out];
   BnArgs b;
   memset(&b, 0, sizeof(b));
-  b.y = t.y; b.C = t.C; b.G = n.groups; b.Pg = (n.batch / n.groups) * t.H * t.W;
-  b.nchunk = bn_nchunk(b.Pg, b.C, b.G, h->bf16);
-  b.partial = ln.bn_partial;
+  b.y = at_sample(t, t.y, fs.sample0, h->es); b.C = t.C; b.G = fs.ng; b.Pg = (n.batch / n.groups) * t.H * t.W;
+  b.nchunk = fused_chunks > 0 ? fused_chunks : bn_nchunk(b.Pg, b.C, n.groups, h->bf16);
+  b.partial = ln.bn_partial + (size_t)fs.group0 * b.nchunk * 2 * t.C;
   b.gamma = n.params + L.gamma_off; b.beta = n.params + L.beta_off;
-  b.aff_a = t.bn.a; b.aff_b = t.bn.b; b.mu = t.bn.mu; b.rstd = t.bn.rstd;
+  const size_t g0 = (size_t)fs.group0 * t.C;
+  b.aff_a = t.bn.a + g0; b.aff_b = t.bn.b + g0; b.mu = t.bn.mu + g0; b.rstd = t.bn.rstd + g0;
   b.eps = 1e-5f;
-  if (fused_chunks > 0) { b.nchunk = fused_chunks; VP_HIP_CHECK(launch_bn_finalize(b, st)); return VP_OK; }
+  if (fused_chunks > 0) { VP_HIP_CHECK(launch_bn_finalize(b, st)); return VP_OK; }
   if (bn_small(b)) {
-    VP_HIP_CHECK(launch_bn_small_fwd(b, t.xa[ACT_LRELU], t.xa[ACT_RELU], h->bf16, st));
+    VP_HIP_CHECK(launch_bn_small_fwd(b, t.xa[ACT_LRELU] ? at_sample(t, t.xa[ACT_LRELU], fs.sample0, h->es) : nullptr,
+                                     t.xa[ACT_RELU] ? at_sample(t, t.xa[ACT_RELU], fs.sample0, h->es) : nullptr, h->bf16, st));
     return 1;
   }
   VP_HIP_CHECK(launch_bn_stats(b, h->bf16, st));
@@ -708,14 +757,17 @@
   t.bn_bwd_done = true;
 }
 
-static int run_layer_fwd(vp_pixrefer* h, Net& n, Layer& L, const Lane& ln, void* pool_out = nullptr) {
+static int run_layer_fwd(vp_pixrefer* h, Net& n, Layer& L, const Lane& ln, void* pool_out = nullptr, const FwdSub* sub = nullptr) {
   hipStream_t st = ln.s;
-  IgemmArgs a = L.fwd.a;
+  const FwdSub fs = sub ? *sub : FwdSub{0, n.batch, 0, n.groups, &L.fwd};
+  const int s0 = fs.sample0, es = h->es;
+  IgemmArgs a = fs.plan->a;
   a.pool_out = pool_out;
-  fill_src(n, L, a.x, n.batch / n.groups, 0, h->es);
-  a.Wp = n.packed + L.pk_fwd * h->es;
+  fill_src(n, L, a.x, n.batch / n.groups, s0, es);
+  a.Wp = n.packed + L.pk_fwd * es;
   Tens& to = n.t[L.out];
-  a.Y = L.tapgemm ? L.tap_S : to.y;
+  float* const tap_S = L.tapgemm ? L.tap_S + (size_t)s0 * L.g.Hin * L.g.Win * 16 : nullptr;
+  a.Y = L.tapgemm ? (void*)tap_S : (to.is_f32 ? to.y : at_sample(to, to.y, s0, es));
   a.bias = L.has_bn || L.tapgemm ? nullptr : n.params + L.b_off;
   a.partial = (float*)ln.scratch;
   a.zeros = h->zeros;
@@ -744,43 +796,47 @@
     a.bn_part = ln.bn_partial; a.bn_tpg = 1 << 30; a.bn_nchunk = stat_chunks;
     fused_stats = true;
   } else if (L.has_bn && a.kern == CK_S2C64) {
-    const int grid = conv_s2c64_grid(a);
+    const int grid = conv_s2c64_grid(L.fwd.a);
     if ((size_t)n.groups * grid * 2 * to.C <= (size_t)1024 * 2 * 512 && n.groups <= 32) {
       stat_chunks = grid;
-      a.bn_part = ln.bn_partial; a.bn_tpg = (n.batch / n.groups) * conv_s2c64_tiles_per_image(a); a.bn_nchunk = grid;
+      a.bn_tpg = (n.batch / n.groups) * conv_s2c64_tiles_per_image(a); a.bn_nchunk = grid;
+      a.tile0 = fs.group0 * a.bn_tpg;
       fused_stats = true;
     }
   } else if (L.fwd_stats) {
     stat_chunks = epi_stat_chunks(L.fwd, n.batch, n.groups);
-    a.bn_part = ln.bn_partial; a.bn_tpg = stat_chunks / a.nclass; a.bn_nchunk = stat_chunks;
+    a.bn_tpg = stat_chunks / a.nclass; a.bn_nchunk = stat_chunks;
     fused_stats = true;
   }
+  if (fused_stats && !a.bn_part) a.bn_part = ln.bn_partial + (size_t)fs.group0 * stat_chunks * 2 * to.C;
   bool acts_fused = false;
+  void* const xa_lrelu = to.need_act[ACT_LRELU] ? at_sample(to, to.xa[ACT_LRELU], s0, es) : nullptr;
+  void* const xa_relu = to.need_act[ACT_RELU] ? at_sample(to, to.xa[ACT_RELU], s0, es) : nullptr;
   if (first_layer_acts_fused(h, n, L)) {
-    a.xa_lrelu = to.need_act[ACT_LRELU] ? to.xa[ACT_LRELU] : nullptr;
-    a.xa_relu = to.need_act[ACT_RELU] ? to.xa[ACT_RELU] : nullptr;
+    a.xa_lrelu = xa_lrelu;
+    a.xa_relu = xa_relu;
     if (!h->store_first_raw) a.Y = nullptr;
     acts_fused = true;
   }
   profile_tag((L.scope + ":fwd").c_str());
-  VP_HIP_CHECK(launch_igemm(a, h->bf16, L.fwd.cfg, st));
+  VP_HIP_CHECK(launch_igemm(a, h->bf16, fs.plan->cfg, st));
   if (L.tapgemm) {
     TapArgs ta;
     memset(&ta, 0, sizeof(ta));
-    ta.S = L.tap_S; ta.bias = n.params + L.b_off; ta.y = (float*)to.y;
-    ta.N = L.g.N; ta.Hin = L.g.Hin; ta.Win = L.g.Win; ta.Hout = L.g.Hout; ta.Wout = L.g.Wout; ta.ks = L.g.ks; ta.pad = L.g.pad;
+    ta.S = tap_S; ta.bias = n.params + L.b_off; ta.y = (float*)to.y + (size_t)s0 * L.g.Hout * L.g.Wout;
+    ta.N = fs.nb; ta.Hin = L.g.Hin; ta.Win = L.g.Win; ta.Hout = L.g.Hout; ta.Wout = L.g.Wout; ta.ks = L.g.ks; ta.pad = L.g.pad;
     VP_HIP_CHECK(launch_tap_gather(ta, st));
   }
   bool acts_done = acts_fused;
   if (L.has_bn) {
-    const int rc = run_bn_stats(h, n, L, fused_stats ? stat_chunks : 0, ln);
+    const int rc = run_bn_stats(h, n, L, fused_stats ? stat_chunks : 0, ln, fs);
     if (rc < 0) return rc;
     acts_done = rc == 1;
   }
   if (!acts_done && (to.need_act[ACT_LRELU] || to.need_act[ACT_RELU])) {
-    VP_HIP_CHECK(launch_act_apply(to.y, L.has_bn ? to.bn.a : nullptr, L.has_bn ? to.bn.b : nullptr, to.C,
-                                  (n.batch / n.groups) * to.H * to.W, (size_t)to.N * to.H * to.W,
-                                  to.xa[ACT_LRELU], to.xa[ACT_RELU], h->bf16, st));
+    const size_t g0 = (size_t)fs.group0 * to.C;
+    VP_HIP_CHECK(launch_act_apply(at_sample(to, to.y, s0, es), L.has_bn ? to.bn.a + g0 : nullptr, L.has_bn ? to.bn.b + g0 : nullptr, to.C,
+                                  (n.batch / n.groups) * to.H * to.W, (size_t)fs.nb * to.H * to.W, xa_lrelu, xa_relu, h->bf16, st));
   }
   return VP_OK;
 }
@@ -1242,6 +1298,15 @@
       };
       plan_ok(L.fwd, "fwd");
       if (L.has_fwd_half) plan_ok(L.fwd_half, "fwd_half");
+      for (int k = 0; k < 2 && n == &h->D && n->has_subs; ++k) {
+        const IgemmPlan& s = L.fwd_sub[k];
+        plan_ok(s, k ? "fwd_sub (fake group)" : "fwd_sub (real groups)");
+        if (s.a.kern != L.fwd.a.kern || s.cfg != L.fwd.cfg || s.a.splitk != L.fwd.a.splitk || s.pack.dst_off != L.pk_fwd || s.a.N != (k ? 1 : 2) * d->batch)
+          fail("%s fwd_sub %d: not the 3N plan's kernel / tile / K split / packed block", L.scope.c_str(), k);
+        const int rows = !L.has_bn ? 0 : (L.fwd_stats ? epi_stat_chunks(L.fwd, n->batch, n->groups) : (s.a.kern == CK_S2C64 ? conv_s2c64_grid(L.fwd.a) : bn_nchunk(d->batch * n->t[L.out].H * n->t[L.out].W, n->t[L.out].C, n->groups, h->bf16)));
+        if ((size_t)n->groups * rows * 2 * n->t[L.out].C > (size_t)1024 * 2 * 512 && (L.fwd_stats || s.a.kern != CK_S2C64))
+          fail("%s fwd_sub %d: %d groups x %d statistics rows exceed a lane's partial table", L.scope.c_str(), k, n->groups, rows);
+      }
       if (d->training && L.has_pair) plan_ok(L.bwd_pair, "bwd_pair");
       if (d->training)
         for (int s2 = 0; s2 < L.nsrc; ++s2) if (L.need_bwd[s2]) { plan_ok(L.bwd[s2], "bwd"); if (n == &h->D || n == &h->V) plan_ok(L.bwd_alt[s2], "bwd_alt"); }
@@ -1276,6 +1341,11 @@
       region_of(tp.dz, tp.elems() / 2 * es, (tp.name + ".dz (pooled-source read)").c_str());
       region_of(h->vpool_code[k], tp.elems() / 2, (tp.name + " codes (pooled-source read)").c_str());
     }
+  }
+  if (rc == VP_OK) {
+    if (d->training && !h->d_early && !h->D.has_subs) set_err("discriminator forward not split: %s", h->D.sub_why.c_str());
+    else if (d->training && !h->d_early) set_err("discriminator forward not split: vp_tune(\"d_real_early\", %d)", d_real_early_knob());
+    else set_err("%s", "");
   }
   delete h;
   return rc;
@@ -1340,11 +1410,14 @@
   VP_HIP_CHECK(hipStreamSynchronize(st));
   h->overlap = false; h->forked = false;
   h->bst_on = 1; h->vgg_fork_layer = 3;
+  h->d_fork_layer = h->G.i_me2;
   h->ov_on = true; h->store_first_raw = false; h->dfork_point = d->d_backward_fork ? d->d_backward_fork - 1 : 2; h->dsplit_on = d->d_beside_vgg != 1;
   if (d->training && d->streams != 1) {
     { const int rc = pool_streams(false, &h->lane[LANE_SIDE].s, &h->lane[LANE_BRANCH].s, &h->lane[LANE_BRANCH2].s); if (rc) { delete h; return rc; } }
     VP_HIP_CHECK(hipEventCreateWithFlags(&h->ev_fork, hipEventDisableTiming));
     VP_HIP_CHECK(hipEventCreateWithFlags(&h->ev_join, hipEventDisableTiming));
+    VP_HIP_CHECK(hipEventCreateWithFlags(&h->ev_dfork, hipEventDisableTiming));
+    VP_HIP_CHECK(hipEventCreateWithFlags(&h->ev_djoin, hipEventDisableTiming));
     h->use_b2 = d->streams != 3;
     VP_HIP_CHECK(hipEventCreateWithFlags(&h->ev_b2join, hipEventDisableTiming));
     VP_HIP_CHECK(hipEventCreateWithFlags(&h->ev_bfork, hipEventDisableTiming));
@@ -1362,7 +1435,7 @@
   if (h->marks_made) for (int i = 0; i < 64; ++i) (void)hipEventDestroy(h->mark[i]);
   if (h->overlap) {
     for (int k = LANE_SIDE; k <= LANE_BRANCH2; ++k) if (h->lane[k].s) (void)hipStreamSynchronize(h->lane[k].s);
-    for (hipEvent_t ev : {h->ev_fork, h->ev_join, h->ev_bfork, h->ev_bjoin, h->ev_b2join, h->ev_upd_b, h->ev_upd_m}) (void)hipEventDestroy(ev);
+    for (hipEvent_t ev : {h->ev_fork, h->ev_join, h->ev_dfork, h->ev_djoin, h->ev_bfork, h->ev_bjoin, h->ev_b2join, h->ev_upd_b, h->ev_upd_m}) (void)hipEventDestroy(ev);
   }
   delete h;
 }
@@ -1423,13 +1496,31 @@
   bool split_vgg = d.training && h->overlap && h->ov_on;
   if (split_vgg) for (Layer& L : h->V.l) split_vgg = split_vgg && L.has_fwd_half;
   bool vgg_real_pending = split_vgg;
+  int d_early = d.training && h->overlap && h->ov_on && !profile_enabled() ? h->d_early : 0;
+  if (d_early == D_EARLY_BRANCH2 && !h->use_b2) d_early = D_EARLY_SIDE_BEHIND;
+  if (d_early == D_EARLY_BRANCH2 && !h->lane[LANE_BRANCH2].s && (rc = pool_streams(true, nullptr, nullptr, &h->lane[LANE_BRANCH2].s))) return rc;
+  h->d_early_last = d_early != 0;
+  auto d_real_groups = [&](const Lane& ln) -> int {
+    if ((rc = after(h->ev_dfork, st, ln.s))) return rc;
+    for (Layer& L : h->D.l) {
+      const FwdSub real{0, 2 * N, 0, 2, &L.fwd_sub[0]};
+      if ((rc = run_layer_fwd(h, h->D, L, ln, nullptr, &real))) return rc;
+    }
+    VP_HIP_CHECK(hipEventRecord(h->ev_djoin, ln.s));
+    return VP_OK;
+  };
   auto vgg_real_half = [&]() -> int {
     vgg_real_pending = false;
+    if (d_early == D_EARLY_SIDE_FRONT && (rc = d_real_groups(side))) return rc;
     if ((rc = after(h->ev_fork, st, side.s))) return rc;
     if ((rc = vgg_forward(h, 0, side, false))) return rc;
     VP_HIP_CHECK(hipEventRecord(h->ev_join, side.s));
+    if (d_early == D_EARLY_SIDE_BEHIND && (rc = d_real_groups(side))) return rc;
     return VP_OK;
   };
+  bool d_real_pending = d_early == D_EARLY_BRANCH2;
+  if (d_real_pending && h->d_fork_layer <= 0) { d_real_pending = false; if ((rc = d_real_groups(h->lane[LANE_BRANCH2]))) return rc; }
+  if (d_early && d_early != D_EARLY_BRANCH2 && !split_vgg && (rc = d_real_groups(side))) return rc;
   if (vgg_real_pending && h->vgg_fork_layer <= 0 && (rc = vgg_real_half())) return rc;
 
   const bool split_enc = d.training && h->overlap && h->ov_on;
@@ -1443,11 +1534,13 @@
     if (split_enc && L.fg) continue;
     if (split_enc && i == h->G.i_me2) VP_HIP_CHECK(hipStreamWaitEvent(st, h->ev_bjoin, 0));
     if (vgg_real_pending && i >= h->vgg_fork_layer && (rc = vgg_real_half())) return rc;
+    if (d_real_pending && i >= h->d_fork_layer) { d_real_pending = false; if ((rc = d_real_groups(h->lane[LANE_BRANCH2]))) return rc; }
     if (g_phase_detail) phase_mark(h, st, 8 + i);
     if ((rc = run_layer_fwd(h, h->G, L, me))) return rc;
   }
 
   if (vgg_real_pending && (rc = vgg_real_half())) return rc;
+  if (d_real_pending && (rc = d_real_groups(h->lane[LANE_BRANCH2]))) return rc;
   CompositeArgs ca;
   memset(&ca, 0, sizeof(ca));
   ca.y4 = h->y4; ca.targets = targets; ca.masks = masks; ca.o4 = h->o4; ca.outputs = h->outputs; ca.outputs_fg = h->outputs_fg;
@@ -1459,7 +1552,15 @@
   const bool split_d = h->overlap && h->ov_on && h->dsplit_on;
   const Lane& ld = split_d ? branch : me;
   if (split_d && (rc = after(h->ev_bfork, st, branch.s))) return rc;
-  for (Layer& L : h->D.l) if ((rc = run_layer_fwd(h, h->D, L, ld))) return rc;
+  if (d_early) {
+    for (Layer& L : h->D.l) {
+      const FwdSub fake{2 * N, N, 2, 1, &L.fwd_sub[1]};
+      if ((rc = run_layer_fwd(h, h->D, L, ld, nullptr, &fake))) return rc;
+    }
+    VP_HIP_CHECK(hipStreamWaitEvent(ld.s, h->ev_djoin, 0));
+  } else {
+    for (Layer& L : h->D.l) if ((rc = run_layer_fwd(h, h->D, L, ld))) return rc;
+  }
   const int hd = H / 8 - 2;
   GanLossArgs ga;
   memset(&ga, 0, sizeof(ga));
@@ -1623,6 +1724,7 @@
   if (k == "d_beside_vgg") { h->dsplit_on = value != 0; return VP_OK; }
   if (k == "store_first_raw") { h->store_first_raw = value != 0; return VP_OK; }
   if (k == "bwd_sums_in_epilogue") { h->bst_on = value < 0 ? 0 : (value > 2 ? 2 : value); return VP_OK; }
+  if (k == "d_real_fork") { h->d_fork_layer = value < 0 ? 0 : value; return VP_OK; }
   if (k == "vgg_real_fork") { h->vgg_fork_layer = value < 0 ? 0 : value; return VP_OK; }
   set_err("vp_pixrefer_set_option: unknown key %s", key);
   return VP_ERR_ARG;
@@ -1633,6 +1735,7 @@
   if (std::string(key) == "bwd_sums_launches") return h->bst_count;
   if (std::string(key) == "pool_codes_written") return h->pool_codes_written ? 1 : 0;
   if (std::string(key) == "pool_bwd_fused") return h->pool_bwd_fused ? 1 : 0;
+  if (std::string(key) == "d_real_early") return h->d_early_last ? 1 : 0;
   return -1;
 }
 
```

Result: no change. 4543 frames/s, median of 6 (+0.9%).
